# vandenheuvel/rust-lp

Hardware: AMD Instinct MI355X
Metric: simplex iterations/sec (higher is better)
Workload: dtype f64; 1 GPU; dense10k: synthetic dense LP 10000x10000 f64 (+10000 slack columns), SteepestDescent, dense tableau with blocked f64-MFMA updates; m=10000, n=10000, seed=20250002, engine=tableau, update_block=64, parallelism=single GPU, solves=1

## Files before the change

include/relp_engine.h:

```cpp
#ifndef RELP_ENGINE_H
#define RELP_ENGINE_H

#include <stdint.h>

#ifdef __cplusplus
extern "C" {
#endif

typedef struct relp_engine relp_engine_t;

typedef enum {
    RELP_OK = 0,
    RELP_E_ARG = -1,
    RELP_E_HIP = -2,
    RELP_E_ZERO_PIVOT = -3,
    RELP_E_SINGULAR = -4,
    RELP_E_STATE = -5,
    RELP_E_UNSUPPORTED = -6,
    RELP_E_ALLOC = -7
} relp_status_t;

typedef enum {
    RELP_RUNNING = 0,
    RELP_OPTIMAL = 1,
    RELP_UNBOUNDED = 2,
    RELP_INFEASIBLE = 3,
    RELP_PHASE_ONE_DONE = 4,
    RELP_NO_ROW_PHASE_ONE = 5
} relp_outcome_t;

typedef enum {
    RELP_RULE_FIRST_PROFITABLE = 0,
    RELP_RULE_FIRST_PROFITABLE_WITH_MEMORY = 1,
    RELP_RULE_STEEPEST_DESCENT = 2
} relp_pivot_rule_t;

typedef enum { RELP_FORMAT_CSC = 0, RELP_FORMAT_DENSE = 1 } relp_format_t;
typedef enum { RELP_MEM_HOST = 0, RELP_MEM_DEVICE = 1 } relp_memory_t;

typedef struct {
    int32_t nr_normal;
    int32_t nr_eq, nr_range, nr_le, nr_ge;
    int32_t format;
    int32_t matrix_memory;
    const int64_t *col_ptr;
    const int32_t *row_idx;
    const double  *values;
    const double  *dense;
    int64_t        dense_ld;
    const double  *b;
    const double  *ranges;
    const double  *cost;
    const double  *upper_bound;
} relp_matrix_data_t;

typedef struct {
    int32_t device;
    int32_t phase_one_rule;
    int32_t phase_two_rule;
    double  tol_cost;
    double  tol_pivot;
    double  tol_zero;
    double  tol_tie;
    double  tol_feas;
    int32_t poll_interval;
    int32_t trace_capacity;
    int32_t shard_rank, shard_count;
    int32_t update_block;
    int32_t engine;
    int32_t ratio_rule;
    int32_t artificial_removal;
    int32_t pivot_rescue;
    int32_t auto_reinversion;
} relp_config_t;

typedef enum { RELP_RATIO_REFERENCE = 0, RELP_RATIO_LARGEST_PIVOT = 1 } relp_ratio_rule_t;
typedef enum { RELP_ARTIFICIAL_REFERENCE = 0, RELP_ARTIFICIAL_TEXTBOOK = 1 } relp_artificial_removal_t;

typedef enum {
    RELP_ENGINE_REVISED = 0,
    RELP_ENGINE_TABLEAU = 1,
    RELP_ENGINE_LU = 2,
    RELP_ENGINE_AUTO = 3
} relp_engine_kind_t;

void relp_default_config(relp_config_t *cfg);
void relp_robust_config(relp_config_t *cfg);
int32_t relp_engine_kind(const relp_engine_t *h);
relp_status_t relp_robust_stats(const relp_engine_t *h, int64_t *out4);
const char *relp_last_error(const relp_engine_t *h);
const char *relp_version(void);

relp_status_t relp_engine_create(const relp_matrix_data_t *md, const relp_config_t *cfg, relp_engine_t **out);
void          relp_engine_destroy(relp_engine_t *h);
relp_status_t relp_set_stream(relp_engine_t *h, void *hip_stream);

relp_status_t relp_select_primal_pivot_column(relp_engine_t *h, int32_t rule, int32_t *found,
                                              int32_t *column, double *relative_cost);
relp_status_t relp_relative_costs(relp_engine_t *h, double *out_n);
relp_status_t relp_generate_column(relp_engine_t *h, int32_t column, double *out_m);
relp_status_t relp_generate_element(relp_engine_t *h, int32_t row, int32_t column, double *out);
relp_status_t relp_select_primal_pivot_row(relp_engine_t *h, int32_t *found, int32_t *row);
relp_status_t relp_select_primal_pivot_row_of(relp_engine_t *h, const double *column_m, int32_t *found, int32_t *row);
relp_status_t relp_bring_into_basis(relp_engine_t *h, int32_t column, int32_t row, double relative_cost,
                                    int32_t *leaving_column);

relp_status_t relp_run(relp_engine_t *h, int64_t max_iters, int64_t *iterations_done, int32_t *outcome);
relp_status_t relp_solve_relaxation(relp_engine_t *h, int64_t max_iters, int32_t *outcome);
relp_status_t relp_from_basis(relp_engine_t *h, const int32_t *basis_columns_m);
relp_status_t relp_set_reinversion_interval(relp_engine_t *h, int64_t pivots);
int64_t       relp_reinversions(const relp_engine_t *h);
relp_status_t relp_flush(relp_engine_t *h);
relp_status_t relp_tab_flush_stats(relp_engine_t *h, int64_t *out2);
int32_t       relp_tab_load_batch(const relp_engine_t *h);
int32_t       relp_update_block(const relp_engine_t *h);
relp_status_t relp_lu_stats(const relp_engine_t *h, int64_t *out8);
relp_status_t relp_lu_lookahead_stats(const relp_engine_t *h, int64_t *out4);
relp_status_t relp_lu_kernel_layout(const relp_engine_t *h, int32_t *out4);
relp_status_t relp_lu_set_device_factorisation(relp_engine_t *h, int32_t on);
relp_status_t relp_lu_device_factorisation_stats(const relp_engine_t *h, int64_t *out6);
relp_status_t relp_lu_factor_residual(relp_engine_t *h, double *out);

relp_status_t relp_lu_phase_cycles(relp_engine_t *h, int64_t *out16);

relp_status_t relp_basis_inverse_row(relp_engine_t *h, int32_t row, double *out_m);
relp_status_t relp_should_refactor(relp_engine_t *h, int32_t *out);
relp_status_t relp_generate_column_of(relp_engine_t *h, const int32_t *row_idx, const double *values, int32_t nnz, double *out_m);
relp_status_t relp_cost_difference_of(relp_engine_t *h, const int32_t *row_idx, const double *values, int32_t nnz, double *out);
relp_status_t relp_lu_change_basis(relp_engine_t *h, int32_t pivot_row_index);
relp_status_t relp_lu_set_factors(relp_engine_t *h, const int64_t *l_col_ptr, const int32_t *l_row_idx, const double *l_values,
                                  const int64_t *u_col_ptr, const int32_t *u_row_idx, const double *u_values);
relp_status_t relp_lu_updates(relp_engine_t *h, int32_t *count);
relp_status_t relp_lu_get_update(relp_engine_t *h, int32_t k, int32_t *pivot, int32_t *idx, double *values, int32_t cap, int32_t *nnz);
relp_status_t relp_lu_get_upper(relp_engine_t *h, int64_t *col_ptr_m1, int32_t *row_idx, double *values, int64_t cap, int64_t *nnz);

int32_t relp_nr_rows(const relp_engine_t *h);
int32_t relp_nr_columns(const relp_engine_t *h);
int32_t relp_phase(const relp_engine_t *h);
int32_t relp_nr_artificial(const relp_engine_t *h);
relp_status_t relp_get_objective(relp_engine_t *h, double *out);
relp_status_t relp_get_b(relp_engine_t *h, double *out_m);
relp_status_t relp_get_minus_pi(relp_engine_t *h, double *out_m);
relp_status_t relp_get_basis_indices(relp_engine_t *h, int32_t *out_m);
relp_status_t relp_get_basis_inverse(relp_engine_t *h, double *out_mm);
relp_status_t relp_current_bfs(relp_engine_t *h, int32_t *cols, double *vals, int32_t cap, int32_t *count);
relp_status_t relp_get_iterations(relp_engine_t *h, int64_t *out);
relp_status_t relp_get_degenerate_pivots(relp_engine_t *h, int64_t *out);
relp_status_t relp_get_trace(relp_engine_t *h, int32_t *phase, int32_t *entering, int32_t *row,
                             int32_t *leaving, int64_t cap, int64_t *count);
relp_status_t relp_check_basis(relp_engine_t *h, double *max_identity_error, double *max_basic_cost,
                               double *min_b);

typedef enum {
    RELP_K_PRICE = 0, RELP_K_SELECT_COLUMN = 1, RELP_K_BUILD_COLUMN = 2, RELP_K_FTRAN = 3,
    RELP_K_RATIO = 4, RELP_K_UPDATE_VECTORS = 5, RELP_K_UPDATE_INVERSE = 6,
    RELP_K_APPLY_W = 7,
    RELP_K_UPDATE_W = 8,
    RELP_K_FLUSH = 9,
    RELP_K_FT_RUN = 10,
    RELP_K_COUNT = 11
} relp_kernel_id_t;
relp_status_t relp_profile_enable(relp_engine_t *h, int32_t enable, int64_t max_launches, int32_t sample_every);
relp_status_t relp_profile_read(relp_engine_t *h, int32_t kernel_id, int64_t *launches, double *total_ms);

relp_status_t relp_synth_fill_dense(double *device_a, int64_t ld, int32_t m, int32_t n, uint64_t seed,
                                    int64_t first_column, void *hip_stream);
relp_status_t relp_device_alloc(void **out, int64_t bytes);
relp_status_t relp_device_free(void *p);

relp_status_t relp_shard_ranges(const relp_engine_t *h, int32_t *col_lo, int32_t *col_hi,
                                int32_t *row_lo, int32_t *row_hi, int32_t *row_slice_stride);
void          relp_shard_column_range(int32_t nr_normal, int32_t rank, int32_t count, int32_t *lo, int32_t *hi);
int64_t       relp_shard_candidate_len(const relp_engine_t *h);
int64_t       relp_shard_rho_len(const relp_engine_t *h);
relp_status_t relp_shard_price(relp_engine_t *h, double *dev_candidate);
relp_status_t relp_shard_select_column(relp_engine_t *h, const double *dev_candidates, int32_t count);
relp_status_t relp_shard_ftran(relp_engine_t *h, double *dev_alpha_slice);
relp_status_t relp_shard_ratio(relp_engine_t *h, const double *dev_alpha_slices, int32_t count, double *dev_rho);
relp_status_t relp_shard_update(relp_engine_t *h, const double *dev_rho);
relp_status_t relp_shard_plan(const relp_matrix_data_t *md, const relp_config_t *cfg, int32_t *col_lo, int32_t *col_hi);
relp_status_t relp_shard_pivot(relp_engine_t *h);
relp_status_t relp_shard_flush_begin(relp_engine_t *h, double **dev_snapshot, int64_t *len_doubles);
relp_status_t relp_shard_flush_end(relp_engine_t *h);
relp_status_t relp_poll(relp_engine_t *h, int32_t *outcome, int64_t *iterations);

typedef int (*relp_allgather_fn)(void *ctx, const void *dev_send, void *dev_recv, int64_t bytes_per_rank, void *hip_stream);
typedef int (*relp_allreduce_sum_fn)(void *ctx, double *dev_buf, int64_t count, void *hip_stream);
relp_status_t relp_shard_set_collectives(relp_engine_t *h, relp_allgather_fn allgather, relp_allreduce_sum_fn allreduce_sum,
                                         void *ctx);
relp_status_t relp_shard_run(relp_engine_t *h, int64_t max_iters, int64_t *done, int32_t *outcome);
relp_status_t relp_shard_inject_failure(relp_engine_t *h, int64_t after_pivots);
#define RELP_RCCL_ID_BYTES 128
relp_status_t relp_rccl_unique_id(uint8_t id[RELP_RCCL_ID_BYTES]);
relp_status_t relp_rccl_attach(relp_engine_t *h, const uint8_t id[RELP_RCCL_ID_BYTES]);

#ifdef __cplusplus
}
#endif
#endif
```

rust-lp_amd/csrc/relp_abi.cpp:

```cpp
#include <cstring>
#include <new>

#include "relp_engine.hpp"

using relp::Engine;

struct relp_engine { Engine impl; };

#define H(h) ((h)->impl)

extern "C" {

void relp_default_config(relp_config_t* cfg) {
    std::memset(cfg, 0, sizeof(*cfg));
    cfg->device = -1;
    cfg->phase_one_rule = RELP_RULE_FIRST_PROFITABLE_WITH_MEMORY;
    cfg->phase_two_rule = RELP_RULE_STEEPEST_DESCENT;
    cfg->tol_cost = 1e-7; cfg->tol_pivot = 1e-5; cfg->tol_zero = 1e-11; cfg->tol_tie = 1e-9; cfg->tol_feas = 1e-7;
    cfg->poll_interval = 64;
    cfg->trace_capacity = 0;
    cfg->shard_rank = 0; cfg->shard_count = 1;
    cfg->update_block = -1;
    cfg->engine = RELP_ENGINE_REVISED;
}

void relp_robust_config(relp_config_t* cfg) {
    relp_default_config(cfg);
    cfg->ratio_rule = RELP_RATIO_LARGEST_PIVOT;
    cfg->artificial_removal = RELP_ARTIFICIAL_TEXTBOOK;
    cfg->pivot_rescue = 1;
    cfg->auto_reinversion = 1;
    cfg->engine = RELP_ENGINE_AUTO;
}
int32_t relp_engine_kind(const relp_engine_t* h) { return h ? H(h).engine_kind() : -1; }
relp_status_t relp_robust_stats(const relp_engine_t* h, int64_t* out4) { return (h && out4) ? H(h).robust_stats(out4) : RELP_E_ARG; }

const char* relp_last_error(const relp_engine_t* h) { return h ? H(h).last_error() : "null handle"; }
const char* relp_version(void) { return "relp-mi355x 0.2 (gfx950; engines: explicit inverse, dense tableau, sparse LU + Forrest-Tomlin)"; }

relp_status_t relp_engine_create(const relp_matrix_data_t* md, const relp_config_t* cfg, relp_engine_t** out) {
    if (!md || !cfg || !out) return RELP_E_ARG;
    relp_engine_t* h = new (std::nothrow) relp_engine_t();
    if (!h) return RELP_E_ALLOC;
    relp_status_t st = H(h).create(*md, *cfg);
    *out = h;
    return st;
}

void relp_engine_destroy(relp_engine_t* h) { delete h; }
relp_status_t relp_set_stream(relp_engine_t* h, void* s) { return h ? H(h).set_stream((hipStream_t)s) : RELP_E_ARG; }

relp_status_t relp_select_primal_pivot_column(relp_engine_t* h, int32_t rule, int32_t* found, int32_t* column, double* cost) {
    return h ? H(h).select_primal_pivot_column(rule, found, column, cost) : RELP_E_ARG;
}
relp_status_t relp_relative_costs(relp_engine_t* h, double* out) { return (h && out) ? H(h).relative_costs(out) : RELP_E_ARG; }
relp_status_t relp_generate_column(relp_engine_t* h, int32_t column, double* out) { return h ? H(h).generate_column(column, out) : RELP_E_ARG; }
relp_status_t relp_generate_element(relp_engine_t* h, int32_t row, int32_t column, double* out) {
    return h ? H(h).generate_element(row, column, out) : RELP_E_ARG;
}
relp_status_t relp_select_primal_pivot_row(relp_engine_t* h, int32_t* found, int32_t* row) {
    return h ? H(h).select_primal_pivot_row(found, row) : RELP_E_ARG;
}
relp_status_t relp_select_primal_pivot_row_of(relp_engine_t* h, const double* column, int32_t* found, int32_t* row) {
    return (h && column) ? H(h).select_primal_pivot_row_of(column, found, row) : RELP_E_ARG;
}
relp_status_t relp_bring_into_basis(relp_engine_t* h, int32_t column, int32_t row, double cost, int32_t* leaving) {
    return h ? H(h).bring_into_basis(column, row, cost, leaving) : RELP_E_ARG;
}

relp_status_t relp_run(relp_engine_t* h, int64_t max_iters, int64_t* done, int32_t* outcome) {
    return h ? H(h).run(max_iters, done, outcome) : RELP_E_ARG;
}
relp_status_t relp_solve_relaxation(relp_engine_t* h, int64_t max_iters, int32_t* outcome) {
    return h ? H(h).solve_relaxation(max_iters, outcome) : RELP_E_ARG;
}
relp_status_t relp_from_basis(relp_engine_t* h, const int32_t* basis) { return (h && basis) ? H(h).from_basis(basis) : RELP_E_ARG; }

relp_status_t relp_flush(relp_engine_t* h) { return h ? H(h).flush() : RELP_E_ARG; }
relp_status_t relp_set_reinversion_interval(relp_engine_t* h, int64_t pivots) { return h ? H(h).set_reinversion_interval(pivots) : RELP_E_ARG; }
int64_t relp_reinversions(const relp_engine_t* h) { return h ? H(h).reinversions() : -1; }
int32_t relp_update_block(const relp_engine_t* h) { return h ? H(h).update_block() : -1; }
int32_t relp_tab_load_batch(const relp_engine_t* h) { return h ? H(h).tab_load_batch_size() : -1; }
relp_status_t relp_lu_stats(const relp_engine_t* h, int64_t* out8) { return (h && out8) ? H(h).lu_stats(out8) : RELP_E_ARG; }
relp_status_t relp_lu_lookahead_stats(const relp_engine_t* h, int64_t* out4) { return (h && out4) ? H(h).lu_lookahead_stats(out4) : RELP_E_ARG; }
relp_status_t relp_lu_kernel_layout(const relp_engine_t* h, int32_t* out4) { return (h && out4) ? H(h).lu_kernel_layout(out4) : RELP_E_ARG; }
relp_status_t relp_lu_set_device_factorisation(relp_engine_t* h, int32_t on) { return h ? H(h).lu_set_device_factorisation(on != 0) : RELP_E_ARG; }
relp_status_t relp_lu_factor_residual(relp_engine_t* h, double* out) { return (h && out) ? H(h).lu_factor_residual(out) : RELP_E_ARG; }
relp_status_t relp_lu_device_factorisation_stats(const relp_engine_t* h, int64_t* out6) { return (h && out6) ? H(h).luf_stats(out6) : RELP_E_ARG; }
relp_status_t relp_shard_inject_failure(relp_engine_t* h, int64_t after_pivots) { if (!h) return RELP_E_ARG; H(h).shard_inject_failure(after_pivots); return RELP_OK; }
relp_status_t relp_lu_phase_cycles(relp_engine_t* h, int64_t* out16) { return (h && out16) ? H(h).lu_phase_cycles(out16) : RELP_E_ARG; }
relp_status_t relp_basis_inverse_row(relp_engine_t* h, int32_t row, double* out_m) { return (h && out_m) ? H(h).basis_inverse_row(row, out_m) : RELP_E_ARG; }
relp_status_t relp_should_refactor(relp_engine_t* h, int32_t* out) { return (h && out) ? H(h).should_refactor(out) : RELP_E_ARG; }
relp_status_t relp_generate_column_of(relp_engine_t* h, const int32_t* idx, const double* val, int32_t nnz, double* out_m) {
    return h ? H(h).generate_column_of(idx, val, nnz, out_m) : RELP_E_ARG;
}
relp_status_t relp_cost_difference_of(relp_engine_t* h, const int32_t* idx, const double* val, int32_t nnz, double* out) {
    return h ? H(h).cost_difference_of(idx, val, nnz, out) : RELP_E_ARG;
}
relp_status_t relp_lu_change_basis(relp_engine_t* h, int32_t row) { return h ? H(h).lu_change_basis(row) : RELP_E_ARG; }
relp_status_t relp_lu_set_factors(relp_engine_t* h, const int64_t* l_ptr, const int32_t* l_idx, const double* l_val,
                                  const int64_t* u_ptr, const int32_t* u_idx, const double* u_val) {
    return h ? H(h).lu_set_factors(l_ptr, l_idx, l_val, u_ptr, u_idx, u_val) : RELP_E_ARG;
}
relp_status_t relp_lu_updates(relp_engine_t* h, int32_t* count) { return (h && count) ? H(h).lu_updates(count) : RELP_E_ARG; }
relp_status_t relp_lu_get_update(relp_engine_t* h, int32_t k, int32_t* pivot, int32_t* idx, double* val, int32_t cap, int32_t* nnz) {
    return h ? H(h).lu_get_update(k, pivot, idx, val, cap, nnz) : RELP_E_ARG;
}
relp_status_t relp_lu_get_upper(relp_engine_t* h, int64_t* col_ptr, int32_t* row_idx, double* values, int64_t cap, int64_t* nnz) {
    return h ? H(h).lu_get_upper(col_ptr, row_idx, values, cap, nnz) : RELP_E_ARG;
}
relp_status_t relp_shard_flush_begin(relp_engine_t* h, double** snap, int64_t* len) {
    return h ? H(h).shard_flush_begin(snap, len) : RELP_E_ARG;
}
relp_status_t relp_shard_flush_end(relp_engine_t* h) { return h ? H(h).shard_flush_end() : RELP_E_ARG; }
relp_status_t relp_shard_set_collectives(relp_engine_t* h, relp_allgather_fn ag, relp_allreduce_sum_fn ar, void* ctx) {
    return h ? H(h).shard_set_collectives(ag, ar, ctx) : RELP_E_ARG;
}
relp_status_t relp_shard_run(relp_engine_t* h, int64_t max_iters, int64_t* done, int32_t* outcome) {
    return h ? H(h).shard_run(max_iters, done, outcome) : RELP_E_ARG;
}
relp_status_t relp_rccl_attach(relp_engine_t* h, const uint8_t* id) { return (h && id) ? H(h).rccl_attach(id) : RELP_E_ARG; }

int32_t relp_nr_rows(const relp_engine_t* h) { return h ? H(h).nr_rows() : -1; }
int32_t relp_nr_columns(const relp_engine_t* h) { return h ? H(h).nr_columns() : -1; }
int32_t relp_phase(const relp_engine_t* h) { return h ? H(h).phase() : -1; }
int32_t relp_nr_artificial(const relp_engine_t* h) { return h ? H(h).nr_artificial() : -1; }
relp_status_t relp_get_objective(relp_engine_t* h, double* out) { return (h && out) ? H(h).get_objective(out) : RELP_E_ARG; }
relp_status_t relp_get_b(relp_engine_t* h, double* out) { return (h && out) ? H(h).get_vector(0, out) : RELP_E_ARG; }
relp_status_t relp_get_minus_pi(relp_engine_t* h, double* out) { return (h && out) ? H(h).get_vector(1, out) : RELP_E_ARG; }
relp_status_t relp_get_basis_indices(relp_engine_t* h, int32_t* out) { return (h && out) ? H(h).get_basis_indices(out) : RELP_E_ARG; }
relp_status_t relp_get_basis_inverse(relp_engine_t* h, double* out) { return (h && out) ? H(h).get_basis_inverse(out) : RELP_E_ARG; }
relp_status_t relp_current_bfs(relp_engine_t* h, int32_t* cols, double* vals, int32_t cap, int32_t* count) {
    return h ? H(h).current_bfs(cols, vals, cap, count) : RELP_E_ARG;
}
relp_status_t relp_get_iterations(relp_engine_t* h, int64_t* out) { return (h && out) ? H(h).get_iterations(out) : RELP_E_ARG; }
relp_status_t relp_get_degenerate_pivots(relp_engine_t* h, int64_t* out) { return (h && out) ? H(h).get_degenerate_pivots(out) : RELP_E_ARG; }
relp_status_t relp_tab_flush_stats(relp_engine_t* h, int64_t* out2) { return (h && out2) ? H(h).tab_flush_stats(out2) : RELP_E_ARG; }
relp_status_t relp_get_trace(relp_engine_t* h, int32_t* phase, int32_t* entering, int32_t* row, int32_t* leaving,
                             int64_t cap, int64_t* count) {
    return h ? H(h).get_trace(phase, entering, row, leaving, cap, count) : RELP_E_ARG;
}
relp_status_t relp_check_basis(relp_engine_t* h, double* e1, double* e2, double* mb) { return h ? H(h).check_basis(e1, e2, mb) : RELP_E_ARG; }

relp_status_t relp_profile_enable(relp_engine_t* h, int32_t enable, int64_t max_launches, int32_t sample_every) {
    return h ? H(h).profile_enable(enable != 0, max_launches, sample_every) : RELP_E_ARG;
}
relp_status_t relp_profile_read(relp_engine_t* h, int32_t kid, int64_t* launches, double* total_ms) {
    return h ? H(h).profile_read(kid, launches, total_ms) : RELP_E_ARG;
}

relp_status_t relp_synth_fill_dense(double* device_a, int64_t ld, int32_t m, int32_t n, uint64_t seed,
                                    int64_t first_column, void* hip_stream) {
    if (!device_a || ld < m || m < 0 || n < 0) return RELP_E_ARG;
    relp::launch_fill_dense(device_a, ld, m, n, seed, first_column, (hipStream_t)hip_stream);
    if (hipStreamSynchronize((hipStream_t)hip_stream) != hipSuccess) return RELP_E_HIP;
    return hipGetLastError() == hipSuccess ? RELP_OK : RELP_E_HIP;
}
relp_status_t relp_device_alloc(void** out, int64_t bytes) {
    if (!out || bytes < 0) return RELP_E_ARG;
    return hipMalloc(out, (size_t)(bytes ? bytes : 1)) == hipSuccess ? RELP_OK : RELP_E_ALLOC;
}
relp_status_t relp_device_free(void* p) { return hipFree(p) == hipSuccess ? RELP_OK : RELP_E_HIP; }

relp_status_t relp_shard_ranges(const relp_engine_t* h, int32_t* col_lo, int32_t* col_hi, int32_t* row_lo,
                                int32_t* row_hi, int32_t* stride) {
    if (!h) return RELP_E_ARG;
    H(h).shard_ranges(col_lo, col_hi, row_lo, row_hi, stride);
    return RELP_OK;
}
void relp_shard_column_range(int32_t nr_normal, int32_t rank, int32_t count, int32_t* lo, int32_t* hi) {
    relp::shard_column_range(nr_normal, rank, count, lo, hi);
}
int64_t relp_shard_candidate_len(const relp_engine_t* h) { return h ? H(h).candidate_len() : -1; }
int64_t relp_shard_rho_len(const relp_engine_t* h) { return h ? H(h).rho_len() : -1; }
relp_status_t relp_shard_price(relp_engine_t* h, double* c) { return (h && c) ? H(h).shard_price(c) : RELP_E_ARG; }
relp_status_t relp_shard_select_column(relp_engine_t* h, const double* c, int32_t count) {
    return (h && c) ? H(h).shard_select_column(c, count) : RELP_E_ARG;
}
relp_status_t relp_shard_ftran(relp_engine_t* h, double* a) { return (h && a) ? H(h).shard_ftran(a) : RELP_E_ARG; }
relp_status_t relp_shard_ratio(relp_engine_t* h, const double* a, int32_t count, double* rho) {
    return (h && a && rho) ? H(h).shard_ratio(a, count, rho) : RELP_E_ARG;
}
relp_status_t relp_shard_update(relp_engine_t* h, const double* rho) { return (h && rho) ? H(h).shard_update(rho) : RELP_E_ARG; }
relp_status_t relp_shard_pivot(relp_engine_t* h) { return h ? H(h).shard_pivot() : RELP_E_ARG; }
relp_status_t relp_shard_plan(const relp_matrix_data_t* md, const relp_config_t* cfg, int32_t* col_lo, int32_t* col_hi) {
    if (!md || !cfg) return RELP_E_ARG;
    relp::Layout layout;
    const relp_status_t st = layout.plan(*md, *cfg, nullptr);
    if (st) return st;
    if (col_lo) *col_lo = layout.col_lo;
    if (col_hi) *col_hi = layout.col_hi;
    return RELP_OK;
}
relp_status_t relp_poll(relp_engine_t* h, int32_t* outcome, int64_t* iterations) { return h ? H(h).poll(outcome, iterations) : RELP_E_ARG; }

}
```

rust-lp_amd/csrc/relp_device_common.h:

```cpp
#pragma once
#include <algorithm>
#include "relp_kernels.h"

#include <math.h>

namespace relp {

static constexpr int kThreads = 256;
static constexpr int kVecPerBlock = 8;
static constexpr int kSingleBlock = 1024;

__device__ __forceinline__ double wave_sum(double v) {
#pragma unroll
    for (int off = 32; off > 0; off >>= 1) v += __shfl_down(v, off, 64);
    return v;
}

__device__ __forceinline__ void block_multi_dot(const double* __restrict__ M, int64_t ld, int len,
                                                int v0, int v_hi, const double* __restrict__ x,
                                                double* s_partial ,
                                                double& result) {
    const int t = threadIdx.x;
    double acc[kVecPerBlock];
    const double* base[kVecPerBlock];
#pragma unroll
    for (int v = 0; v < kVecPerBlock; ++v) {
        acc[v] = 0.0;
        int vi = v0 + v;
        if (vi >= v_hi) vi = v_hi - 1;
        base[v] = M + (int64_t)vi * ld;
    }
    const int len2 = len & ~1;
    for (int k = 2 * t; k < len2; k += 2 * kThreads) {
        const double2 xv = *reinterpret_cast<const double2*>(x + k);
#pragma unroll
        for (int v = 0; v < kVecPerBlock; ++v) {
            const double2 a = *reinterpret_cast<const double2*>(base[v] + k);
            acc[v] = fma(a.x, xv.x, acc[v]);
            acc[v] = fma(a.y, xv.y, acc[v]);
        }
    }
    if ((len & 1) && t == 0) {
        const double xl = x[len - 1];
#pragma unroll
        for (int v = 0; v < kVecPerBlock; ++v) acc[v] = fma(base[v][len - 1], xl, acc[v]);
    }
    const int lane = t & 63, wave = t >> 6;
#pragma unroll
    for (int v = 0; v < kVecPerBlock; ++v) {
        const double w = wave_sum(acc[v]);
        if (lane == 0) s_partial[wave * kVecPerBlock + v] = w;
    }
    __syncthreads();
    if (t < kVecPerBlock) {
        result = (s_partial[0 * kVecPerBlock + t] + s_partial[1 * kVecPerBlock + t]) +
                 (s_partial[2 * kVecPerBlock + t] + s_partial[3 * kVecPerBlock + t]);
    }
}

__device__ __forceinline__ double select_key(int rule, int n, const PivotRecord* rec, int j, double d_j) {
    if (rule == 2) return d_j;
    const int last = (rule == 1 && rec) ? rec->last_selected : -1;
    if (last >= 0) return (double)(j >= last ? j - last : j - last + n);
    return (double)j;
}

template <int BS>
__device__ __forceinline__ void block_min_key(double& key, int& kj) {
    __shared__ double s_k[BS / 64];
    __shared__ int s_j[BS / 64];
#pragma unroll
    for (int off = 32; off > 0; off >>= 1) {
        const double ok = __shfl_down(key, off, 64);
        const int oj = __shfl_down(kj, off, 64);
        if (ok < key || (ok == key && oj < kj)) { key = ok; kj = oj; }
    }
    const int lane = threadIdx.x & 63, wave = threadIdx.x >> 6;
    if (lane == 0) { s_k[wave] = key; s_j[wave] = kj; }
    __syncthreads();
    key = s_k[0]; kj = s_j[0];
#pragma unroll
    for (int w = 1; w < BS / 64; ++w)
        if (s_k[w] < key || (s_k[w] == key && s_j[w] < kj)) { key = s_k[w]; kj = s_j[w]; }
}

__device__ __forceinline__ void block_partial_min(double key, int kj, SelectPartials sp, int slot) {
    block_min_key<kThreads>(key, kj);
    if (threadIdx.x == 0) { sp.k1[slot] = key; sp.j[slot] = kj; }
}

__device__ __forceinline__ void price_virtual_body(const ColumnTable& ct, const double* __restrict__ minus_pi,
                                                   double* __restrict__ d, int cost_mode, const SelectPartials& sp,
                                                   const PivotRecord* rec, int block) {
    const int t = block * kThreads + threadIdx.x;
    int j = -1;
    double val = 0.0;
    if (t < ct.nr_artificial) {
        j = t;
        val = (cost_mode == 1 ? 1.0 : 0.0) + minus_pi[ct.column_to_row[t]];
    } else {
        const int v = t - ct.nr_artificial;
        if (v < ct.nr_virtual) {
            const int r0 = ct.vrow0[v];
            double s = r0 >= 0 ? (double)ct.vsign[v] * minus_pi[r0] : 0.0;
            const int r1 = ct.vrow1[v];
            if (r1 >= 0) s += minus_pi[r1];
            j = ct.nr_artificial + ct.nr_normal + v;
            val = s;
        }
    }
    if (j >= 0) d[j] = val;
    if (!sp.k1) return;
    double key = INFINITY;
    int kj = 0x7fffffff;
    if (j >= 0 && !sp.in_basis[j] && val < -sp.tol_cost) { key = select_key(sp.rule, sp.n, rec, j, val); kj = j; }
    block_partial_min(key, kj, sp, sp.offset + block);
}

template <int BS>
__device__ __forceinline__ void tab_select_entering(const TableauView& tv, const SelectPartials& sp, int count, double& k1,
                                                    int& bj) {
    constexpr int kListMax = 32, kGroups = BS / kThreads;
    __shared__ int s_list[kListMax];
    __shared__ int s_cnt;
    __shared__ int s_low[BS / 64];
    for (int t = threadIdx.x + BS; t < count; t += BS) {
        const double key = sp.k1[t];
        const int j = sp.j[t];
        if (key < k1 || (key == k1 && j < bj)) { k1 = key; bj = j; }
    }
    if (threadIdx.x == 0) s_cnt = 0;
    block_min_key<BS>(k1, bj);
    if (!(bj != 0x7fffffff && sp.rule == 2 && sp.tol_tie > 0.0)) return;
    const double bound = k1 + sp.tol_tie * fmax(1.0, fabs(k1));
    for (int t = threadIdx.x; t < count; t += BS) {
        if (!(sp.k1[t] <= bound)) continue;
        const int pos = atomicAdd(&s_cnt, 1);
        if (pos < kListMax) s_list[pos] = t;
    }
    __syncthreads();
    const int listed = s_cnt;
    const int grp = threadIdx.x / kThreads, u = threadIdx.x % kThreads;
    int lowest = 0x7fffffff;
    auto scan_slot = [&](int t) {
        const int c = tv.c_lo + t * kThreads + u;
        const int j = c - tv.col_off;
        if (c < tv.c_hi && j >= 0 && j < tv.n) {
            const double v = tv.d[c];
            if (!sp.in_basis[j] && v < -sp.tol_cost && v <= bound && j < lowest) lowest = j;
        }
    };
    if (listed <= kListMax) {
        for (int i = grp; i < listed; i += kGroups) scan_slot(s_list[i]);
    } else {
        for (int t = grp; t < count; t += kGroups)
            if (sp.k1[t] <= bound) scan_slot(t);
    }
#pragma unroll
    for (int off = 32; off > 0; off >>= 1) lowest = min(lowest, __shfl_down(lowest, off, 64));
    if ((threadIdx.x & 63) == 0) s_low[threadIdx.x >> 6] = lowest;
    __syncthreads();
    bj = s_low[0];
#pragma unroll
    for (int w = 1; w < BS / 64; ++w) bj = min(bj, s_low[w]);
}

__device__ __forceinline__ int candidate_winner(const double* key, const double* idx, int64_t stride, int count, int rule,
                                                double tol_tie) {
    int win = -1; double k1 = INFINITY; double kj = 0.0;
    for (int g = 0; g < count; ++g) {
        const double a = key[g * stride], j = idx[g * stride];
        if (a < k1 || (a == k1 && win >= 0 && j < kj)) { k1 = a; kj = j; win = g; }
    }
    if (win >= 0 && rule == 2 && tol_tie > 0.0) {
        const double bound = k1 + tol_tie * fmax(1.0, fabs(k1));
        for (int g = 0; g < count; ++g)
            if (key[g * stride] <= bound && idx[g * stride] < kj) { kj = idx[g * stride]; win = g; }
    }
    return win;
}

static constexpr int kMaxRanks = 64;
__device__ __forceinline__ int candidate_winner_staged(const double* __restrict__ msgs, int count, int64_t msg_len, int rule,
                                                       double tol_tie, int* q, double* d_q) {
    __shared__ double s_key[kMaxRanks], s_idx[kMaxRanks], s_dq[kMaxRanks];
    __shared__ int s_win;
    for (int g = threadIdx.x; g < count && g < kMaxRanks; g += blockDim.x) {
        s_key[g] = msgs[g * msg_len + 0]; s_idx[g] = msgs[g * msg_len + 1]; s_dq[g] = msgs[g * msg_len + 2];
    }
    __syncthreads();
    if (threadIdx.x == 0) s_win = candidate_winner(s_key, s_idx, 1, count, rule, tol_tie);
    __syncthreads();
    const int win = s_win;
    if (win >= 0) { *q = (int)s_idx[win]; *d_q = s_dq[win]; }
    return win;
}

__device__ __forceinline__ void record_candidate(PivotRecord* rec, int rule, int win, int q, double d_q) {
    if (win < 0) {
        rec->outcome = DEV_NO_CANDIDATE;
        if (rule == 1) rec->last_selected = -1;
    } else {
        rec->q = q;
        rec->d_q = d_q;
        if (rule == 1) rec->last_selected = q;
    }
}

__device__ __forceinline__ double pivot_b(double a, double b_i, double br, bool is_r) {
    return is_r ? br : (a != 0.0 ? fma(-a, br, b_i) : b_i);
}

__device__ __forceinline__ void pivot_bookkeeping(int phase, long long iterations, double minus_objective, double d_q, double br,
                                                  int q, int r, int leaving, uint8_t* in_basis, int32_t* trace, int64_t trace_cap,
                                                  PivotRecord* rec) {
    rec->minus_objective = fma(-d_q, br, minus_objective);
    if (leaving < kWrappedArtificialBase) in_basis[leaving] = 0;
    in_basis[q] = 1;
    if (trace && iterations < trace_cap) {
        trace[0 * trace_cap + iterations] = phase;
        trace[1 * trace_cap + iterations] = q;
        trace[2 * trace_cap + iterations] = r;
        trace[3 * trace_cap + iterations] = leaving;
    }
    if (br == 0.0) rec->degenerate += 1;
    rec->iterations = iterations + 1;
}

static constexpr int kMaxEta = 128;

typedef unsigned long long tie_key_t;
static constexpr tie_key_t kNoTieKey = ~0ull;
__device__ __forceinline__ tie_key_t tie_key(double a, int leave, int ratio_rule) {
    const unsigned size = ratio_rule ? 0x7fffffffu - __float_as_uint((float)a) : 0u;
    return ((tie_key_t)size << 32) | (unsigned)leave;
}
__device__ __forceinline__ int tie_key_leaving(tie_key_t k) { return (int)(unsigned)(k & 0xffffffffull); }

template <int BS>
__device__ __forceinline__ void tie_reduce(tie_key_t& key, int& row, tie_key_t* s_k, int* s_r, bool wide) {
    const int lane = threadIdx.x & 63, wave = threadIdx.x >> 6;
    if (wide) {
#pragma unroll
        for (int off = 32; off > 0; off >>= 1) {
            const tie_key_t ok = __shfl_down(key, off, 64);
            const int orow = __shfl_down(row, off, 64);
            if (ok < key) { key = ok; row = orow; }
        }
    } else {
        int lv = (int)(unsigned)key;
        if (key == kNoTieKey) lv = 0x7fffffff;
#pragma unroll
        for (int off = 32; off > 0; off >>= 1) {
            const int ol = __shfl_down(lv, off, 64);
            const int orow = __shfl_down(row, off, 64);
            if (ol < lv) { lv = ol; row = orow; }
        }
        key = (unsigned)lv;
    }
    if (lane == 0) { s_k[wave] = key; s_r[wave] = row; }
    __syncthreads();
    key = s_k[0]; row = s_r[0];
#pragma unroll
    for (int w = 1; w < BS / 64; ++w)
        if (s_k[w] < key) { key = s_k[w]; row = s_r[w]; }
}

template <int BS>
__device__ __forceinline__ void ratio_commit_row(int r, int leaving, const double* alpha, const double* b, const DeferredUpdate& du,
                                                 int p, PivotRecord* rec, int guard_m = 0, double guard_rel = 0.0) {
    if (guard_m > 0) {
        __shared__ double s_gm[BS / 64];
        double mx = 0.0;
        for (int i = threadIdx.x; i < guard_m; i += BS) mx = fmax(mx, fabs(alpha[i]));
#pragma unroll
        for (int off = 32; off > 0; off >>= 1) mx = fmax(mx, __shfl_down(mx, off, 64));
        __syncthreads();
        if ((threadIdx.x & 63) == 0) s_gm[threadIdx.x >> 6] = mx;
        __syncthreads();
        double amax = s_gm[0];
#pragma unroll
        for (int w = 1; w < BS / 64; ++w) amax = fmax(amax, s_gm[w]);
        if (alpha[r] < guard_rel * amax) {
            if (threadIdx.x == 0) rec->outcome = DEV_NO_ROW;
            return;
        }
    }
    const bool deferred = du.kmax > 0;
    double a_r = 0.0, b_r = 0.0;
    int jt = 0;
    if (threadIdx.x == 0) {
        a_r = alpha[r];
        b_r = b[r];
        if (deferred) jt = du.pos_of_row[r];
    }
    if (deferred)
        for (int j = threadIdx.x; j < p; j += BS) du.wr[j] = du.W[(int64_t)j * du.ld + r];
    if (threadIdx.x == 0) {
        rec->r = r;
        rec->leaving = leaving;
        rec->alpha_r = a_r;
        rec->b_r = b_r;
        if (deferred) {
            rec->n_eta_old = p;
            if (jt < 0) { jt = p; du.S[p] = r; du.pos_of_row[r] = p; rec->n_eta = p + 1; }
            rec->eta_target = jt;
        }
    }
}

template <int BS, int ITEMS>
__device__ __forceinline__ void ratio_body(const double* alpha, const double* b, const int32_t* basis_indices, int m,
                                           const Tolerances& tol, const DeferredUpdate& du, int p, PivotRecord* rec) {
    __shared__ double s_min[BS / 64];
    __shared__ double s_bcast;
    const int lane = threadIdx.x & 63, wave = threadIdx.x >> 6;

    constexpr int kItems = ITEMS;
    const bool cached = m <= kItems * BS;
    double ratio_r[kItems], alpha_r[kItems];
    int leave_r[kItems];
    double mn = INFINITY;
    if (cached) {
#pragma unroll
        for (int k = 0; k < kItems; ++k) {
            const int i = threadIdx.x + k * BS;
            const bool in = i < m;
            const double a = in ? alpha[i] : 0.0;
            double bi = in ? b[i] : 0.0;
            leave_r[k] = in ? basis_indices[i] : 0x7fffffff;
            alpha_r[k] = a;
            if (bi <= tol.zero) bi = 0.0;
            ratio_r[k] = (in && a > tol.pivot) ? bi / a : INFINITY;
            mn = fmin(mn, ratio_r[k]);
        }
    } else {
#pragma unroll 4
        for (int i = threadIdx.x; i < m; i += BS) {
            const double a = alpha[i];
            double bi = b[i];
            if (bi <= tol.zero) bi = 0.0;
            const double ratio = (a > tol.pivot) ? bi / a : INFINITY;
            mn = fmin(mn, ratio);
        }
    }
#pragma unroll
    for (int off = 32; off > 0; off >>= 1) mn = fmin(mn, __shfl_down(mn, off, 64));
    if (lane == 0) s_min[wave] = mn;
    __syncthreads();
    if (threadIdx.x == 0) {
        double g = s_min[0];
        for (int w = 1; w < BS / 64; ++w) g = fmin(g, s_min[w]);
        s_bcast = g;
    }
    __syncthreads();
    const double gmin = s_bcast;
    if (gmin == INFINITY) {
        if (threadIdx.x == 0) rec->outcome = DEV_NO_ROW;
        return;
    }
    const double bound = gmin + tol.tie * fmax(1.0, fabs(gmin));
    tie_key_t best_key = kNoTieKey;
    int best_row = -1;
    if (cached) {
#pragma unroll
        for (int k = 0; k < kItems; ++k) {
            if (ratio_r[k] <= bound) {
                const tie_key_t key = tie_key(alpha_r[k], leave_r[k], tol.ratio_rule);
                if (key < best_key) { best_key = key; best_row = threadIdx.x + k * BS; }
            }
        }
    } else {
#pragma unroll 4
        for (int i = threadIdx.x; i < m; i += BS) {
            const double a = alpha[i];
            double bi = b[i];
            const int lv = basis_indices[i];
            if (bi <= tol.zero) bi = 0.0;
            if (a > tol.pivot && bi / a <= bound) {
                const tie_key_t key = tie_key(a, lv, tol.ratio_rule);
                if (key < best_key) { best_key = key; best_row = i; }
            }
        }
    }
    __shared__ tie_key_t s_cl[BS / 64];
    __shared__ int s_cr[BS / 64];
    tie_reduce<BS>(best_key, best_row, s_cl, s_cr, tol.ratio_rule != 0);
    ratio_commit_row<BS>(best_row, tie_key_leaving(best_key), alpha, b, du, p, rec, tol.pivot_guard ? m : 0, tol.guard_rel);
}

__device__ __forceinline__ double row_ratio(double a, double bi, const Tolerances& tol) {
    if (bi <= tol.zero) bi = 0.0;
    return a > tol.pivot ? bi / a : INFINITY;
}

template <int BS>
__device__ __forceinline__ void ratio_blocks_pick(const double* alpha, const double* b, const int32_t* basis_indices, int m,
                                                  const Tolerances& tol, const double* rmin, int nblk, int* row_out, int* leave_out,
                                                  double first = INFINITY, bool have_first = false, int rpb = kThreads) {
    __shared__ double s_min[BS / 64];
    __shared__ double s_bcast;
    constexpr int kListMax = 64;
    __shared__ int s_list[kListMax];
    __shared__ int s_cnt;
    __shared__ tie_key_t s_cl[BS / 64];
    __shared__ int s_cr[BS / 64];
    const int lane = threadIdx.x & 63, wave = threadIdx.x >> 6;
    double mn = have_first ? first : INFINITY;
    for (int t = threadIdx.x + (have_first ? BS : 0); t < nblk; t += BS) mn = fmin(mn, rmin[t]);
#pragma unroll
    for (int off = 32; off > 0; off >>= 1) mn = fmin(mn, __shfl_down(mn, off, 64));
    if (lane == 0) s_min[wave] = mn;
    if (threadIdx.x == 0) s_cnt = 0;
    __syncthreads();
    if (threadIdx.x == 0) {
        double g = s_min[0];
        for (int w = 1; w < BS / 64; ++w) g = fmin(g, s_min[w]);
        s_bcast = g;
    }
    __syncthreads();
    const double gmin = s_bcast;
    if (gmin == INFINITY) { *row_out = -1; *leave_out = 0x7fffffff; return; }
    const double bound = gmin + tol.tie * fmax(1.0, fabs(gmin));
    for (int t = threadIdx.x; t < nblk; t += BS) {
        if (!(rmin[t] <= bound)) continue;
        const int pos = atomicAdd(&s_cnt, 1);
        if (pos < kListMax) s_list[pos] = t;
    }
    __syncthreads();
    const int listed = s_cnt;
    const bool use_list = listed <= kListMax;
    const int total = (use_list ? listed : nblk) * rpb;
    tie_key_t best_key = kNoTieKey;
    int best_row = -1;
    for (int idx = threadIdx.x; idx < total; idx += BS) {
        const int t = use_list ? s_list[idx / rpb] : idx / rpb;
        const int i = t * rpb + idx % rpb;
        if (i >= m) continue;
        const double a = alpha[i];
        double bi = b[i];
        int lv = basis_indices[i];
        asm volatile("" : "+v"(lv));
        if (bi <= tol.zero) bi = 0.0;
        if (a > tol.pivot && bi / a <= bound) {
            const tie_key_t key = tie_key(a, lv, tol.ratio_rule);
            if (key < best_key) { best_key = key; best_row = i; }
        }
    }
    tie_reduce<BS>(best_key, best_row, s_cl, s_cr, tol.ratio_rule != 0);
    *row_out = best_row; *leave_out = tie_key_leaving(best_key);
}

template <int BS>
__device__ __forceinline__ void ratio_blocks_body(const double* alpha, const double* b, const int32_t* basis_indices, int m,
                                                  const Tolerances& tol, const DeferredUpdate& du, const double* rmin, int nblk,
                                                  int p, PivotRecord* rec, double first = INFINITY, bool have_first = false,
                                                  int rpb = kThreads) {
    int r, leaving;
    ratio_blocks_pick<BS>(alpha, b, basis_indices, m, tol, rmin, nblk, &r, &leaving, first, have_first, rpb);
    if (r < 0) {
        if (threadIdx.x == 0) rec->outcome = DEV_NO_ROW;
        return;
    }
    ratio_commit_row<BS>(r, leaving, alpha, b, du, p, rec, tol.pivot_guard ? m : 0, tol.guard_rel);
}

static inline int cdiv(int64_t a, int64_t b) { return (int)((a + b - 1) / b); }
static inline int element_blocks(int64_t total) { return (int)std::min<int64_t>((total + 255) / 256, int64_t(1) << 22); }

}
```

rust-lp_amd/csrc/relp_engine.cpp:

```cpp
#include "relp_engine_internal.hpp"

#include <algorithm>
#include <chrono>
#include <cmath>
#include <cstdio>
#include <cstdlib>
#include <cstring>
#include <limits>

namespace relp {

bool Engine::hip_ok(hipError_t e, const char* what) {
    if (e == hipSuccess) return true;
    err_ = std::string(what) + ": " + hipGetErrorString(e);
    return false;
}

void Engine::free_all() {
    luf_release();
    auto fr = [](auto*& p) { if (p) { (void)hipFree(p); p = nullptr; } };
    if (owns_A_) fr(dA_);
    dA_ = nullptr;
    fr(dBinv_); fr(d_minus_pi_); fr(d_b_); fr(d_alpha_); fr(d_aq_); fr(d_rho_); fr(d_d_); fr(d_w_); fr(d_cost_);
    fr(d_basis_); fr(d_column_to_row_); fr(d_bound_row_); fr(d_vrow0_); fr(d_vrow1_); fr(d_vsign_); fr(d_trace_);
    fr(d_in_basis_); fr(d_rec_);
    fr(d_part_k1_); fr(d_part_j_);
    fr(d_fcols_); fr(d_fcount_); fr(d_fmask_); fr(d_fstats_); fr(d_R0c_);
    fr(dT0_); fr(dR0_); fr(d_b_alt_); fr(d_basis_alt_); fr(d_shadow_); fr(d_shadow_meta_);
    if (h_lu_buf_) { (void)hipHostFree(h_lu_buf_); h_lu_buf_ = nullptr; h_lu_cap_ = 0; }
    if (h_basis_) { (void)hipHostFree(h_basis_); h_basis_ = nullptr; }
    if (h_mirror_) { (void)hipHostFree(h_mirror_); h_mirror_ = nullptr; d_mirror_ = nullptr; }
    fr(d_cost_store_); fr(d_idcol_); fr(d_rmin_);
    fr(d_msg_cand_); fr(d_msg_cands_); fr(d_msg_slice_); fr(d_msg_slices_); fr(d_msg_rho_); fr(d_msg_status_); fr(d_msg_statuses_);
    fr(d_v_); fr(d_W_); fr(d_wr_); fr(d_R_); fr(d_S_); fr(d_pos_of_row_);
    fr(d_cptr_); fr(d_cidx_); fr(d_cval_); fr(d_lu_buf_); fr(d_lu_buf_alt_); fr(d_lu_scratch_); fr(d_ft_buf_); fr(d_pe_buf_);
    if (h_ft_hdr_) { (void)hipHostFree(h_ft_hdr_); h_ft_hdr_ = nullptr; }
    if (h_rec_) { (void)hipHostFree(h_rec_); h_rec_ = nullptr; }
    for (auto e : prof_ev_) (void)hipEventDestroy(e);
    prof_ev_.clear();
    if (owns_stream_ && stream_) { (void)hipStreamDestroy(stream_); }
    stream_ = nullptr;
}

Engine::~Engine() { rccl_release(); free_all(); }

ColumnTable Engine::table() const {
    ColumnTable ct;
    ct.nr_artificial = lay_.nr_artificial;
    ct.nr_normal = lay_.nr_normal;
    ct.nr_virtual = lay_.nr_virtual;
    ct.nr_constraints = lay_.mc;
    ct.column_to_row = d_column_to_row_;
    ct.bound_row = d_bound_row_;
    ct.vrow0 = d_vrow0_;
    ct.vrow1 = d_vrow1_;
    ct.vsign = d_vsign_;
    ct.cost = d_cost_;
    return ct;
}

Tolerances Engine::tolerances() const { return Tolerances{cfg_.tol_cost, cfg_.tol_pivot, cfg_.tol_zero, cfg_.tol_tie, cfg_.ratio_rule, (pivot_guard_on_ && guard_rel_ > 0.0) ? 1 : 0, guard_rel_}; }

TableauView Engine::tview() const {
    TableauView tv;
    tv.T0 = dT0_ - (int64_t)lay_.sc_lo * ld_t_; tv.ld_t = ld_t_;
    tv.R0 = dR0_ - (int64_t)lay_.sc_lo; tv.ld_r = ld_r_;
    tv.d = d_d_; tv.m = lay_.m; tv.n_store = n_store_;
    tv.col_off = phase_ == 1 ? 0 : tab_na_;
    tv.n = nr_columns();
    tv.c_lo = lay_.sc_lo; tv.c_hi = lay_.sc_hi;
    return tv;
}

FlushList Engine::flush_list() const {
    FlushList fl;
    fl.cols = d_fcols_; fl.count = d_fcount_; fl.mask = d_fmask_; fl.R0c = d_R0c_; fl.ld = ld_r_; fl.stats = d_fstats_;
    return fl;
}

SelectPartials Engine::tab_partials(int rule) const {
    SelectPartials sp;
    sp.k1 = d_part_k1_; sp.j = d_part_j_; sp.in_basis = d_in_basis_; sp.tol_cost = cfg_.tol_cost; sp.rule = rule;
    sp.n = nr_columns(); sp.offset = 0; sp.nb_struct = 0; sp.tol_tie = cfg_.tol_tie; sp.p_lo = 0; sp.cols_per_slot = 8;
    return sp;
}

DeferredUpdate Engine::deferred() const {
    DeferredUpdate du;
    du.W = d_W_; du.ld = ld_b_; du.kmax = block_; du.S = d_S_; du.pos_of_row = d_pos_of_row_; du.wr = d_wr_; du.R = d_R_;
    du.batch = load_batch_; du.w_split = w_split_;
    return du;
}

relp_status_t Engine::download_rec() {
    HIP_TRY(hipMemcpyAsync(h_rec_, d_rec_, sizeof(PivotRecord), hipMemcpyDeviceToHost, stream_));
    HIP_TRY(hipStreamSynchronize(stream_));
    return RELP_OK;
}

relp_status_t Engine::upload_rec() {
    HIP_TRY(hipMemcpyAsync(d_rec_, h_rec_, sizeof(PivotRecord), hipMemcpyHostToDevice, stream_));
    HIP_TRY(hipStreamSynchronize(stream_));
    return RELP_OK;
}

relp_status_t Engine::set_stream(hipStream_t s) {
    if (stream_) HIP_TRY(hipStreamSynchronize(stream_));
    if (owns_stream_ && stream_) HIP_TRY(hipStreamDestroy(stream_));
    stream_ = s;
    owns_stream_ = false;
    return RELP_OK;
}

relp_status_t Engine::create(const relp_matrix_data_t& md, const relp_config_t& cfg) {
    (void)hipGetLastError();
    cfg_ = cfg;
    if (cfg_.shard_count < 1) cfg_.shard_count = 1;
    if (cfg_.poll_interval < 1) cfg_.poll_interval = 64;
    if (const relp_status_t lst = lay_.build(md, cfg_, &err_)) return lst;
    if (cfg_.device >= 0) HIP_TRY(hipSetDevice(cfg_.device));
    phase_ = 1;
    n_alloc_ = lay_.nr_columns();

    HIP_TRY(hipStreamCreateWithFlags(&stream_, hipStreamNonBlocking));
    owns_stream_ = true;
    const int32_t n_local = lay_.col_hi - lay_.col_lo;
    lu_ = lay_.engine == RELP_ENGINE_LU;
    tableau_ = lay_.engine == RELP_ENGINE_TABLEAU;
    if (lu_) {
        if (cfg_.shard_count > 1) return fail(RELP_E_UNSUPPORTED, "the LU engine is not sharded");
        relp_status_t lst = lu_load_matrix(md);
        if (lst) return lst;
    } else if (md.format == RELP_FORMAT_DENSE) {
        if (lay_.nr_normal > 0 && lay_.mc > 0 && !md.dense) return fail(RELP_E_ARG, "dense matrix missing");
        const int64_t src_ld = md.dense_ld > 0 ? md.dense_ld : lay_.mc;
        if (src_ld < lay_.mc) return fail(RELP_E_ARG, "dense_ld < nr_constraints");
        if (md.matrix_memory == RELP_MEM_DEVICE && (src_ld % 2) == 0) {
            dA_ = const_cast<double*>(md.dense); ld_a_ = src_ld; owns_A_ = false;
        } else {
            ld_a_ = round_up(std::max<int64_t>(lay_.mc, 1), 2);
            HIP_TRY(dev_alloc(&dA_, ld_a_ * std::max(n_local, 1)));
            owns_A_ = true;
            if (n_local > 0 && lay_.mc > 0)
                HIP_TRY(hipMemcpy2D(dA_, ld_a_ * sizeof(double), md.dense, src_ld * sizeof(double), lay_.mc * sizeof(double),
                                    n_local, md.matrix_memory == RELP_MEM_DEVICE ? hipMemcpyDeviceToDevice : hipMemcpyHostToDevice));
        }
    } else if (md.format == RELP_FORMAT_CSC) {
        if (md.matrix_memory != RELP_MEM_HOST) return fail(RELP_E_UNSUPPORTED, "CSC input must be in host memory");
        if (!md.col_ptr) return fail(RELP_E_ARG, "col_ptr missing");
        ld_a_ = round_up(std::max<int64_t>(lay_.mc, 1), 2);
        const int64_t e0 = n_local > 0 ? md.col_ptr[lay_.col_lo] : 0, e1 = n_local > 0 ? md.col_ptr[lay_.col_hi] : 0;
        for (int64_t p = e0; p < e1; ++p)
            if (md.row_idx[p] < 0 || md.row_idx[p] >= lay_.mc) return fail(RELP_E_ARG, "row index out of range");
        const int64_t cells = ld_a_ * std::max(n_local, 1);
        HIP_TRY(dev_alloc(&dA_, cells));
        owns_A_ = true;
        HIP_TRY(hipMemset(dA_, 0, (size_t)cells * sizeof(double)));
        if (e1 > e0) {
            int64_t* t_ptr = nullptr; int32_t* t_idx = nullptr; double* t_val = nullptr;
            auto drop = [&]() { if (t_ptr) (void)hipFree(t_ptr); if (t_idx) (void)hipFree(t_idx); if (t_val) (void)hipFree(t_val); };
            if (hipMalloc(reinterpret_cast<void**>(&t_ptr), sizeof(int64_t) * (size_t)(n_local + 1)) != hipSuccess ||
                hipMalloc(reinterpret_cast<void**>(&t_idx), sizeof(int32_t) * (size_t)(e1 - e0)) != hipSuccess ||
                hipMalloc(reinterpret_cast<void**>(&t_val), sizeof(double) * (size_t)(e1 - e0)) != hipSuccess) {
                drop();
                return fail(RELP_E_ALLOC, "staging the CSC arrays");
            }
            hipError_t err = hipMemcpy(t_ptr, md.col_ptr + lay_.col_lo, sizeof(int64_t) * (size_t)(n_local + 1), hipMemcpyHostToDevice);
            if (err == hipSuccess) err = hipMemcpy(t_idx, md.row_idx + e0, sizeof(int32_t) * (size_t)(e1 - e0), hipMemcpyHostToDevice);
            if (err == hipSuccess) err = hipMemcpy(t_val, md.values + e0, sizeof(double) * (size_t)(e1 - e0), hipMemcpyHostToDevice);
            if (err == hipSuccess) {
                launch_csc_to_dense(t_ptr, t_idx, t_val, n_local, dA_, ld_a_, nullptr);
                err = hipDeviceSynchronize();
            }
            drop();
            if (err != hipSuccess) return fail(RELP_E_HIP, "dense copy of the CSC input");
        }
    } else {
        return fail(RELP_E_ARG, "unknown matrix format");
    }

    ld_b_ = round_up(lay_.m, 16);
    const int64_t rows_local = std::max(lay_.row_hi - lay_.row_lo, 1);
    HIP_TRY(dev_alloc(&dBinv_, (tableau_ || lu_) ? 16 : rows_local * ld_b_));
    HIP_TRY(dev_alloc(&d_minus_pi_, ld_b_));
    HIP_TRY(dev_alloc(&d_b_, ld_b_));
    HIP_TRY(dev_alloc(&d_alpha_, ld_b_));
    HIP_TRY(dev_alloc(&d_aq_, ld_b_));
    HIP_TRY(dev_alloc(&d_rho_, ld_b_));
    HIP_TRY(dev_alloc(&d_w_, ld_b_));
    HIP_TRY(dev_alloc(&d_d_, n_alloc_));
    HIP_TRY(dev_alloc(&d_cost_, lay_.nr_normal));
    HIP_TRY(dev_alloc(&d_basis_, lay_.m));
    HIP_TRY(dev_alloc(&d_column_to_row_, lay_.nr_artificial));
    HIP_TRY(dev_alloc(&d_bound_row_, lay_.nr_normal));
    HIP_TRY(dev_alloc(&d_vrow0_, lay_.nr_virtual));
    HIP_TRY(dev_alloc(&d_vrow1_, lay_.nr_virtual));
    HIP_TRY(dev_alloc(&d_vsign_, lay_.nr_virtual));
    HIP_TRY(dev_alloc(&d_in_basis_, n_alloc_));
    HIP_TRY(dev_alloc(&d_rec_, 1));
    {
        const int64_t slots = price_structural_blocks(lay_.col_lo, lay_.col_hi) + (lay_.nr_artificial + lay_.nr_virtual + 255) / 256 + 8 +
                              tab_scan_blocks(n_alloc_) + price_csc_blocks(0, lay_.nr_normal);
        HIP_TRY(dev_alloc(&d_part_k1_, slots));
        HIP_TRY(dev_alloc(&d_part_j_, slots));
    }
    block_ = cfg_.update_block < 0 ? (lay_.m >= 4096 ? 64 : 0) : std::min(cfg_.update_block, 128);
    if (lu_) {
        block_ = cfg_.update_block < 0 ? 128 : std::max(1, std::min(cfg_.update_block, 128));
        HIP_TRY(dev_alloc(&d_lu_scratch_, ld_b_));
        {
            const char* la = std::getenv("RELP_LU_LOOKAHEAD");
            const char* fl = std::getenv("RELP_FUSE_LANES");
            const char* df = std::getenv("RELP_LU_DEVICE_FACTOR");
            luf_enabled_ = df && std::atoi(df) != 0;
            luf_download_ = df && std::atoi(df) == 2;
            lu_lookahead_env_ = la ? std::atoi(la) : 8;
            lu_lookahead_set_ = la != nullptr;
            lu_fuse_lanes_env_ = fl ? std::atoi(fl) : 256;
        }
        relp_status_t fst = ft_plan_and_alloc();
        if (fst) return fst;
    }
    if (tableau_) {
        if (block_ == 0) block_ = 64;
        if (cfg_.update_block < 0 && lay_.m >= 4096 && n_alloc_ >= 40000) block_ = 96;
        n_store_ = n_alloc_;
        tab_na_ = lay_.nr_artificial;
        const int64_t n_owned = std::max(lay_.sc_hi - lay_.sc_lo, 1);
        ld_t_ = round_up(lay_.m, 2);
        ld_r_ = round_up(n_owned, 2);
        HIP_TRY(dev_alloc(&dT0_, ld_t_ * n_owned));
        HIP_TRY(dev_alloc(&dR0_, ld_r_ * (block_ + 1)));
        {
            const char* e = std::getenv("RELP_TAB_FLUSH_ALL");
            flush_all_ = e && std::atoi(e) != 0;
            HIP_TRY(dev_alloc(&d_fstats_, 2));
            if (!flush_all_) {
                HIP_TRY(dev_alloc(&d_fcols_, n_owned));
                HIP_TRY(dev_alloc(&d_fcount_, 1));
                HIP_TRY(dev_alloc(&d_fmask_, (n_owned + 63) / 64));
                HIP_TRY(dev_alloc(&d_R0c_, ld_r_ * block_));
            }
        }
        {
            const char* e = std::getenv("RELP_TAB_LOAD_BATCH");
            load_batch_ = tab_load_batch(e ? std::atoi(e) : 0);
            const char* w = std::getenv("RELP_TAB_W_SPLIT");
            w_split_ = w && std::atoi(w) >= 1 ? std::min(std::atoi(w), 16) : kTabSplitDefault;
        }
        {
            const char* e = std::getenv("RELP_FUSED_UPDATE");
            fused_update_ = !(e && std::atoi(e) == 0);
            if (cfg_.pivot_rescue && cfg_.shard_count == 1) fused_update_ = false;
            if (fused_update_) {
                HIP_TRY(dev_alloc(&d_b_alt_, ld_b_));
                HIP_TRY(dev_alloc(&d_basis_alt_, lay_.m));
                HIP_TRY(dev_alloc(&d_shadow_, std::max(block_, 1) + 1));
                HIP_TRY(hipMalloc(reinterpret_cast<void**>(&d_shadow_meta_), 2 * sizeof(int32_t)));
                const int32_t none[2] = {-1, 0};
                HIP_TRY(hipMemcpy(d_shadow_meta_, none, sizeof none, hipMemcpyHostToDevice));
            }
        }
        HIP_TRY(dev_alloc(&d_cost_store_, n_store_));
        HIP_TRY(dev_alloc(&d_idcol_, lay_.m));
    }
    if (block_ > 0 && ft_) {
        HIP_TRY(dev_alloc(&d_v_, ld_b_));
    } else if (block_ > 0) {
        HIP_TRY(dev_alloc(&d_v_, ld_b_));
        HIP_TRY(dev_alloc(&d_W_, ld_b_ * block_));
        if (!tableau_) HIP_TRY(dev_alloc(&d_R_, ld_b_ * block_));
        HIP_TRY(dev_alloc(&d_wr_, block_));
        HIP_TRY(dev_alloc(&d_S_, block_));
        HIP_TRY(dev_alloc(&d_pos_of_row_, lay_.m));
        HIP_TRY(hipMemset(d_pos_of_row_, 0xFF, sizeof(int32_t) * lay_.m));
    }
    HIP_TRY(dev_alloc(&d_rmin_, lay_.m / 8 + 2));
    HIP_TRY(hipHostMalloc(reinterpret_cast<void**>(&h_rec_), sizeof(PivotRecord), hipHostMallocDefault));
    trace_cap_ = std::max(cfg_.trace_capacity, 0);
    if (trace_cap_ > 0) HIP_TRY(dev_alloc(&d_trace_, 4 * trace_cap_));

    auto up = [&](void* dst, const void* src, size_t bytes) -> hipError_t {
        return bytes ? hipMemcpy(dst, src, bytes, hipMemcpyHostToDevice) : hipSuccess;
    };
    HIP_TRY(up(d_cost_, lay_.cost.data(), sizeof(double) * lay_.nr_normal));
    HIP_TRY(up(d_bound_row_, lay_.bound_row.data(), sizeof(int32_t) * lay_.nr_normal));
    HIP_TRY(up(d_vrow0_, lay_.vrow0.data(), sizeof(int32_t) * lay_.nr_virtual));
    HIP_TRY(up(d_vrow1_, lay_.vrow1.data(), sizeof(int32_t) * lay_.nr_virtual));
    HIP_TRY(up(d_vsign_, lay_.vsign.data(), sizeof(int32_t) * lay_.nr_virtual));
    HIP_TRY(up(d_column_to_row_, lay_.column_to_row.data(), sizeof(int32_t) * lay_.nr_artificial));
    HIP_TRY(up(d_basis_, lay_.basis.data(), sizeof(int32_t) * lay_.m));
    HIP_TRY(up(d_b_, lay_.rhs.data(), sizeof(double) * lay_.m));
    HIP_TRY(up(d_minus_pi_, lay_.minus_pi.data(), sizeof(double) * lay_.m));
    std::vector<uint8_t> flags(n_alloc_, 0);
    for (int32_t r = 0; r < lay_.m; ++r) flags[lay_.basis[r]] = 1;
    HIP_TRY(up(d_in_basis_, flags.data(), flags.size()));
    if (lay_.row_hi > lay_.row_lo && !tableau_ && !lu_) launch_set_identity(dBinv_, ld_b_, lay_.row_lo, lay_.row_hi, stream_);
    if (tableau_) {
        idcol_h_ = lay_.basis;
        HIP_TRY(up(d_idcol_, idcol_h_.data(), sizeof(int32_t) * lay_.m));
        const double* A = dA_ - (int64_t)lay_.col_lo * ld_a_;
        launch_tab_build(tview(), A, ld_a_, table(), stream_);
        cost_store_h_.assign(n_store_, 0.0);
        for (int32_t k = 0; k < lay_.nr_artificial; ++k) cost_store_h_[k] = 1.0;
        std::vector<double> w(ld_b_, 0.0);
        for (int32_t k = 0; k < lay_.nr_artificial; ++k) w[lay_.column_to_row[k]] = 1.0;
        HIP_TRY(up(d_cost_store_, cost_store_h_.data(), sizeof(double) * n_store_));
        HIP_TRY(up(d_w_, w.data(), sizeof(double) * ld_b_));
        launch_tab_price_init(tview(), d_w_, d_cost_store_, stream_);
    }
    {
        bool sparse_input = false;
        if (md.format == RELP_FORMAT_CSC && md.col_ptr && lay_.nr_normal > 0 && lay_.mc > 0)
            sparse_input = (double)md.col_ptr[lay_.nr_normal] <= 0.10 * (double)lay_.nr_normal * (double)lay_.mc;
        reinvert_interval_ = (!lu_ && cfg_.shard_count == 1 && lay_.m <= 4096 && sparse_input) ? 1000 : 0;
        if (cfg_.auto_reinversion && !lu_ && cfg_.shard_count == 1) reinvert_interval_ = 256;
    }
    std::memset(h_rec_, 0, sizeof(PivotRecord));
    h_rec_->outcome = DEV_RUNNING;
    h_rec_->minus_objective = -lay_.phase1_objective;
    h_rec_->last_selected = -1;
    h_rec_->phase = 1;
    relp_status_t st = upload_rec();
    if (st) return st;
    HIP_TRY(hipDeviceSynchronize());
    if (hipGetLastError() != hipSuccess) return fail(RELP_E_HIP, "a kernel launch of the set-up failed");
    if (lu_ && (st = lu_refactor())) return st;
    return RELP_OK;
}

relp_status_t Engine::profile_enable(bool enable, int64_t max_launches, int32_t sample_every) {
    prof_stride_ = sample_every > 0 ? sample_every : 1;
    prof_tick_ = 0;
    HIP_TRY(hipStreamSynchronize(stream_));
    for (auto e : prof_ev_) (void)hipEventDestroy(e);
    prof_ev_.clear(); prof_kid_.clear(); prof_open_ = false;
    prof_on_ = enable;
    if (enable) {
        prof_ev_.resize((size_t)max_launches * 2);
        for (auto& e : prof_ev_) HIP_TRY(hipEventCreate(&e));
        prof_kid_.reserve((size_t)max_launches);
    }
    return RELP_OK;
}

void Engine::prof_begin(int kid, hipStream_t on) {
    prof_open_ = false;
    if (!prof_on_ || (prof_kid_.size() + 1) * 2 > prof_ev_.size()) return;
    if (kid != RELP_K_FLUSH && (prof_tick_ % prof_stride_) != 0) return;
    (void)hipEventRecord(prof_ev_[2 * prof_kid_.size()], on ? on : stream_);
    prof_kid_.push_back(kid);
    prof_open_ = true;
}

void Engine::prof_end(hipStream_t on) {
    if (!prof_open_) return;
    (void)hipEventRecord(prof_ev_[2 * (prof_kid_.size() - 1) + 1], on ? on : stream_);
    prof_open_ = false;
}

relp_status_t Engine::profile_read(int kernel_id, int64_t* launches, double* total_ms) {
    HIP_TRY(hipStreamSynchronize(stream_));
    int64_t n = 0; double ms = 0.0;
    for (size_t k = 0; k < prof_kid_.size(); ++k) {
        if (prof_kid_[k] != kernel_id) continue;
        float t = 0.f;
        if (hipEventElapsedTime(&t, prof_ev_[2 * k], prof_ev_[2 * k + 1]) == hipSuccess) { ms += t; ++n; }
    }
    if (launches) *launches = n;
    if (total_ms) *total_ms = ms;
    return RELP_OK;
}

void Engine::enqueue_price(int cost_mode, const double* vec, const PivotRecord* rec, int32_t p_lo, int32_t p_hi) {
    const ColumnTable ct = table();
    if (lu_) {
        launch_price_csc(csc(), ct, vec, d_d_, 0, lay_.nr_normal, cost_mode, SelectPartials{}, rec, stream_);
        launch_price_virtual(ct, vec, d_d_, cost_mode, rec, stream_);
        return;
    }
    const double* A = dA_ - (int64_t)lay_.col_lo * ld_a_;
    launch_price_structural(A, ld_a_, ct, vec, d_d_, p_lo, p_hi, cost_mode, rec, stream_);
    if (p_lo > 0 || p_hi < lay_.nr_normal) launch_price_mask_unowned(ct, d_d_, p_lo, p_hi, rec, stream_);
    launch_price_virtual(ct, vec, d_d_, cost_mode, rec, stream_);
}

void Engine::enqueue_iteration_tableau(int rule) {
    const TableauView tv = tview();
    const DeferredUpdate du = deferred();
    const SelectPartials sp = tab_partials(rule);
    if (fused_update_ && in_loop_) {
        prof_begin(RELP_K_FTRAN);
        launch_tab_select_column_rmin(tv, du, sp, tab_scan_blocks(lay_.sc_hi - lay_.sc_lo), d_alpha_, d_b_, tolerances(), d_rmin_,
                                      d_rec_, stream_, d_shadow_, d_shadow_meta_);
        prof_end();
        prof_begin(RELP_K_PRICE);
        launch_tab_ratio_update_all(tv, du, sp, lay_.m, d_alpha_, d_b_, d_b_alt_, d_basis_, d_basis_alt_, d_in_basis_, d_trace_,
                                    trace_cap_, tolerances(), d_rmin_, d_shadow_, d_shadow_meta_, d_rec_, stream_);
        prof_end();
        std::swap(d_b_, d_b_alt_);
        std::swap(d_basis_, d_basis_alt_);
        shadow_pending_ = true;
        if (++since_flush_ >= block_) enqueue_flush();
        return;
    }
    tab_settle();
    prof_begin(RELP_K_FTRAN);
    launch_tab_select_column_rmin(tv, du, sp, tab_scan_blocks(lay_.sc_hi - lay_.sc_lo), d_alpha_, d_b_, tolerances(), d_rmin_,
                                  d_rec_, stream_);
    prof_end();
    prof_begin(RELP_K_RATIO);
    launch_ratio_blocks(d_alpha_, d_b_, d_basis_, lay_.m, tolerances(), du, d_rmin_, d_rec_, stream_);
    prof_end();
    prof_begin(RELP_K_PRICE);
    launch_tab_update_all(tv, du, sp, lay_.m, d_alpha_, d_b_, d_basis_, d_in_basis_, d_trace_, trace_cap_, d_rec_, stream_);
    prof_end();
    if (++since_flush_ >= block_) enqueue_flush();
}

void Engine::enqueue_iteration(int rule) {
    struct Tick { int64_t& t; ~Tick() { ++t; } } tick{prof_tick_};
    if (tableau_) { enqueue_iteration_tableau(rule); return; }
    if (lu_) { enqueue_iteration_lu(rule); return; }
    const ColumnTable ct = table();
    const double* A = dA_ - (int64_t)lay_.col_lo * ld_a_;
    double* Binv = dBinv_ - (int64_t)lay_.row_lo * ld_b_;
    const int n = nr_columns();
    SelectPartials sp;
    sp.k1 = d_part_k1_; sp.j = d_part_j_; sp.in_basis = d_in_basis_; sp.tol_cost = cfg_.tol_cost; sp.rule = rule;
    const int nb_struct = price_structural_blocks(lay_.col_lo, lay_.col_hi);
    sp.n = n; sp.offset = 0; sp.nb_struct = nb_struct; sp.tol_tie = cfg_.tol_tie; sp.p_lo = lay_.col_lo; sp.cols_per_slot = 8;
    const int nb_virt = price_virtual_blocks(ct);
    prof_begin(RELP_K_PRICE);
    if (lay_.col_lo > 0 || lay_.col_hi < lay_.nr_normal) {
        launch_price_structural_sel(A, ld_a_, ct, d_minus_pi_, d_d_, lay_.col_lo, lay_.col_hi, phase_, sp, d_rec_, stream_);
        launch_price_mask_unowned(ct, d_d_, lay_.col_lo, lay_.col_hi, d_rec_, stream_);
        SelectPartials spv = sp;
        spv.offset = nb_struct;
        launch_price_virtual_sel(ct, d_minus_pi_, d_d_, phase_, spv, d_rec_, stream_);
    } else {
        launch_price_all_sel(A, ld_a_, ct, d_minus_pi_, d_d_, lay_.col_lo, lay_.col_hi, phase_, sp, d_rec_, stream_);
    }
    prof_end();
    prof_begin(RELP_K_SELECT_COLUMN);
    launch_select_partials(sp, nb_struct + nb_virt, d_d_, A, ld_a_, ct, lay_.m, d_aq_, d_rec_, stream_);
    prof_end();
    if (block_ == 0) {
        prof_begin(RELP_K_FTRAN);
        launch_ftran_rmin(Binv, ld_b_, lay_.m, d_aq_, d_alpha_, d_b_, tolerances(), d_rmin_, d_rec_, stream_);
        prof_end();
        prof_begin(RELP_K_RATIO);
        launch_ratio_rows(d_alpha_, d_b_, d_basis_, lay_.m, tolerances(), DeferredUpdate{}, d_rmin_, ftran_rows_per_block(), d_rec_,
                          stream_);
        prof_end();
        prof_begin(RELP_K_UPDATE_VECTORS);
        launch_compute_rho(Binv, ld_b_, lay_.m, lay_.row_lo, lay_.row_hi, d_rho_, d_rec_, stream_);
        prof_end();
        prof_begin(RELP_K_UPDATE_INVERSE);
        launch_update_inverse_vectors(Binv, ld_b_, lay_.m, d_alpha_, d_rho_, d_b_, d_minus_pi_, d_basis_, d_in_basis_, d_trace_,
                                      trace_cap_, d_rec_, stream_);
        prof_end();
        return;
    }
    const DeferredUpdate du = deferred();
    prof_begin(RELP_K_FTRAN);
    launch_ftran(Binv, ld_b_, lay_.m, lay_.row_lo, lay_.row_hi, d_aq_, d_v_, 0, d_rec_, stream_);
    prof_end();
    prof_begin(RELP_K_APPLY_W);
    launch_apply_w_rmin(du, lay_.m, d_v_, d_alpha_, d_b_, tolerances(), d_rmin_, d_rec_, stream_);
    prof_end();
    prof_begin(RELP_K_RATIO);
    launch_ratio_rows(d_alpha_, d_b_, d_basis_, lay_.m, tolerances(), du, d_rmin_, 256, d_rec_, stream_);
    prof_end();
    prof_begin(RELP_K_UPDATE_W);
    launch_update_w(du, lay_.m, d_alpha_, d_rec_, stream_);
    launch_rho_deferred(du, Binv, ld_b_, lay_.m, lay_.row_lo, lay_.row_hi, d_rho_, d_rec_, stream_);
    prof_end();
    prof_begin(RELP_K_UPDATE_VECTORS);
    launch_update_vectors(lay_.m, d_alpha_, d_rho_, d_b_, d_minus_pi_, d_basis_, d_in_basis_, d_trace_, trace_cap_, d_rec_,
                          stream_);
    prof_end();
    if (++since_flush_ >= block_) enqueue_flush();
}

void Engine::tab_settle() {
    if (shadow_pending_) {
        launch_tab_apply_shadow(deferred(), d_shadow_, d_shadow_meta_, stream_);
        shadow_pending_ = false;
    }
}

void Engine::enqueue_flush() {
    if (block_ == 0) return;
    if (lu_) {
        if (since_flush_ == 0 && !ft_need_refactor_) return;
        prof_begin(RELP_K_FLUSH);
        const relp_status_t st = lu_refactor();
        prof_end();
        if (st && !lu_status_) lu_status_ = st;
        return;
    }
    if (tableau_) {
        tab_settle();
        const DeferredUpdate dut = deferred();
        prof_begin(RELP_K_FLUSH);
        launch_tab_flush(tview(), dut, d_rec_, flush_list(), stream_);
        launch_flush_reset(dut, d_rec_, stream_);
        prof_end();
        since_flush_ = 0;
        if (++flushes_since_reprice_ >= kRepriceEveryFlushes) {
            flushes_since_reprice_ = 0;
            const TableauView tv = tview();
            const int rule = phase_ == 1 ? cfg_.phase_one_rule : cfg_.phase_two_rule;
            launch_tab_basis_costs(tv, d_basis_, d_cost_store_, d_w_, stream_);
            launch_tab_price_init(tv, d_w_, d_cost_store_, stream_);
            launch_tab_scan(tv, tab_partials(rule), d_rec_, stream_);
        }
        return;
    }
    const DeferredUpdate du = deferred();
    double* Binv = dBinv_ - (int64_t)lay_.row_lo * ld_b_;
    prof_begin(RELP_K_FLUSH);
    launch_flush_snapshot(du, Binv, ld_b_, lay_.row_lo, lay_.row_hi, d_rec_, stream_);
    launch_flush_apply(du, Binv, ld_b_, lay_.m, lay_.row_lo, lay_.row_hi, d_rec_, stream_);
    launch_flush_reset(du, d_rec_, stream_);
    prof_end();
    since_flush_ = 0;
}

relp_status_t Engine::flush() {
    tab_settle();
    if (cfg_.shard_count > 1 && block_ > 0 && !tableau_) {
        if (!coll_allreduce_) return fail(RELP_E_STATE, "sharded flush needs relp_shard_flush_begin/end (or the collective hooks)");
        if (since_flush_ == 0) return RELP_OK;
        double* snap = nullptr; int64_t len = 0;
        relp_status_t st = shard_flush_begin(&snap, &len);
        if (st) return st;
        if (len > 0) {
            if (coll_allreduce_(coll_ctx_, snap, len, stream_)) return fail(RELP_E_HIP, "all-reduce of the flush snapshot failed");
            if ((st = shard_flush_end())) return st;
        }
        since_flush_ = 0;
        return RELP_OK;
    }
    enqueue_flush();
    return RELP_OK;
}

relp_status_t Engine::select_primal_pivot_column(int rule, int32_t* found, int32_t* column, double* cost) {
    relp_status_t st = download_rec();
    if (st) return st;
// ... 954 lines not shown
```

rust-lp_amd/csrc/relp_engine.hpp:

```cpp
#pragma once
#include <hip/hip_runtime.h>

#include <cstdint>
#include <chrono>
#include <condition_variable>
#include <functional>
#include <mutex>
#include <string>
#include <thread>
#include <vector>

#include "../../include/relp_engine.h"
#include "relp_kernels.h"
#include "relp_layout.hpp"
#include "relp_lu.hpp"

namespace relp {

class Engine {
  public:
    Engine() = default;
    ~Engine();

    relp_status_t create(const relp_matrix_data_t& md, const relp_config_t& cfg);
    relp_status_t set_stream(hipStream_t s);

    relp_status_t select_primal_pivot_column(int rule, int32_t* found, int32_t* column, double* cost);
    relp_status_t relative_costs(double* out_n);
    relp_status_t generate_column(int32_t column, double* out_m);
    relp_status_t generate_element(int32_t row, int32_t column, double* out);
    relp_status_t select_primal_pivot_row(int32_t* found, int32_t* row);
    relp_status_t select_primal_pivot_row_of(const double* column, int32_t* found, int32_t* row);
    relp_status_t bring_into_basis(int32_t column, int32_t row, double cost, int32_t* leaving);

    relp_status_t run(int64_t max_iters, int64_t* done, int32_t* outcome);
    int32_t engine_kind() const { return lay_.engine; }
    relp_status_t robust_stats(int64_t* out4) const;
    relp_status_t solve_relaxation(int64_t max_iters, int32_t* outcome);
    relp_status_t from_basis(const int32_t* basis_columns);
    relp_status_t set_reinversion_interval(int64_t pivots);
    int64_t reinversions() const { return reinversions_; }
    relp_status_t flush();
    int32_t update_block() const { return block_; }
    relp_status_t lu_stats(int64_t* out8) const;
    relp_status_t lu_lookahead_stats(int64_t* out4) const;
    relp_status_t lu_kernel_layout(int32_t* out4) const;
    relp_status_t luf_stats(int64_t* out6) const;
    relp_status_t lu_set_device_factorisation(bool on);
    relp_status_t lu_factor_residual(double* out);
    relp_status_t lu_basis_columns(std::vector<std::vector<std::pair<int32_t, double>>>& cols);
    relp_status_t lu_basis_flat(std::vector<int64_t>& ptr, std::vector<int32_t>& idx, std::vector<double>& val);
    relp_status_t lu_phase_cycles(int64_t* out16);
    relp_status_t lu_download_basis();
    relp_status_t lu_factor_downloaded_basis();
    relp_status_t lu_refactor_lookahead(int rule, int64_t budget, bool have_basis);
    relp_status_t ft_read_report(bool* have_basis);
    void lu_refactor_clock(std::chrono::steady_clock::time_point tb, std::chrono::steady_clock::time_point t0,
                           std::chrono::steady_clock::time_point t1, std::chrono::steady_clock::time_point t2);
    relp_status_t basis_inverse_row(int32_t row, double* out_m);
    relp_status_t should_refactor(int32_t* out);
    relp_status_t generate_column_of(const int32_t* idx, const double* val, int32_t nnz, double* out_m);
    relp_status_t cost_difference_of(const int32_t* idx, const double* val, int32_t nnz, double* out);
    relp_status_t lu_change_basis(int32_t row);
    relp_status_t lu_updates(int32_t* count);
    relp_status_t lu_get_update(int32_t k, int32_t* pivot, int32_t* idx, double* val, int32_t cap, int32_t* nnz);
    relp_status_t lu_get_upper(int64_t* col_ptr, int32_t* row_idx, double* values, int64_t cap, int64_t* nnz);
    relp_status_t lu_set_factors(const int64_t* l_ptr, const int32_t* l_idx, const double* l_val, const int64_t* u_ptr,
                                 const int32_t* u_idx, const double* u_val);
    relp_status_t shard_flush_begin(double** dev_snapshot, int64_t* len);
    relp_status_t shard_flush_end();

    int32_t nr_rows() const { return lay_.m; }
    int32_t nr_columns() const { return lay_.nr_columns(); }
    int32_t phase() const { return phase_; }
    int32_t nr_artificial() const { return lay_.nr_artificial; }
    relp_status_t get_objective(double* out);
    relp_status_t get_vector(int which, double* out);
    relp_status_t get_basis_indices(int32_t* out);
    relp_status_t get_basis_inverse(double* out);
    relp_status_t current_bfs(int32_t* cols, double* vals, int32_t cap, int32_t* count);
    relp_status_t get_iterations(int64_t* out);
    relp_status_t get_degenerate_pivots(int64_t* out);
    relp_status_t tab_flush_stats(int64_t* out2);
    int32_t tab_load_batch_size() const { return tableau_ ? load_batch_ : 0; }
    relp_status_t get_trace(int32_t* phase, int32_t* entering, int32_t* row, int32_t* leaving, int64_t cap,
                            int64_t* count);
    relp_status_t check_basis(double* max_identity_error, double* max_basic_cost, double* min_b);

    relp_status_t profile_enable(bool enable, int64_t max_launches, int32_t sample_every);
    relp_status_t profile_read(int kernel_id, int64_t* launches, double* total_ms);

    void shard_ranges(int32_t* col_lo, int32_t* col_hi, int32_t* row_lo, int32_t* row_hi, int32_t* stride) const;
    int64_t candidate_len() const { return lay_.candidate_len; }
    int64_t rho_len() const { return ld_b_; }
    relp_status_t shard_price(double* dev_candidate);
    relp_status_t shard_select_column(const double* dev_candidates, int32_t count);
    relp_status_t shard_ftran(double* dev_alpha_slice);
    relp_status_t shard_ratio(const double* dev_alpha_slices, int32_t count, double* dev_rho);
    relp_status_t shard_update(const double* dev_rho);
    relp_status_t shard_pivot();
    relp_status_t shard_set_collectives(relp_allgather_fn ag, relp_allreduce_sum_fn ar, void* ctx);
    relp_status_t shard_run(int64_t max_iters, int64_t* done, int32_t* outcome);
    void shard_inject_failure(int64_t after_pivots) { inject_failure_after_ = after_pivots; }
    relp_status_t rccl_attach(const uint8_t* id);
    relp_status_t poll(int32_t* outcome, int64_t* iterations);

    const char* last_error() const { return err_.c_str(); }

  private:
    Layout lay_;
    relp_config_t cfg_{};
    int32_t phase_ = 1;

    double* dA_ = nullptr; int64_t ld_a_ = 0; bool owns_A_ = false;
    double* dBinv_ = nullptr; int64_t ld_b_ = 0;
    double *d_minus_pi_ = nullptr, *d_b_ = nullptr, *d_alpha_ = nullptr, *d_aq_ = nullptr, *d_rho_ = nullptr,
           *d_d_ = nullptr, *d_w_ = nullptr, *d_cost_ = nullptr;
    int32_t *d_basis_ = nullptr, *d_column_to_row_ = nullptr, *d_bound_row_ = nullptr, *d_vrow0_ = nullptr,
            *d_vrow1_ = nullptr, *d_vsign_ = nullptr, *d_trace_ = nullptr;
    uint8_t* d_in_basis_ = nullptr;
    PivotRecord* d_rec_ = nullptr;
    PivotRecord* h_rec_ = nullptr;
    hipStream_t stream_ = nullptr; bool owns_stream_ = false;
    int64_t trace_cap_ = 0;
    int32_t block_ = 0;
    int64_t since_flush_ = 0;
    double* d_v_ = nullptr;
    double *d_W_ = nullptr, *d_wr_ = nullptr, *d_R_ = nullptr;
    int32_t *d_S_ = nullptr, *d_pos_of_row_ = nullptr;
    double* d_part_k1_ = nullptr;
    int32_t* d_part_j_ = nullptr;
    bool tableau_ = false;
    double* dT0_ = nullptr; int64_t ld_t_ = 0;
    double* dR0_ = nullptr; int64_t ld_r_ = 0;
    bool flush_all_ = false;
    int32_t *d_fcols_ = nullptr, *d_fcount_ = nullptr;
    unsigned long long *d_fmask_ = nullptr, *d_fstats_ = nullptr;
    double* d_R0c_ = nullptr;
    FlushList flush_list() const;
    int32_t load_batch_ = 0, w_split_ = 0;
    double* d_cost_store_ = nullptr;
    int32_t* d_idcol_ = nullptr;
    bool fused_update_ = false, shadow_pending_ = false;
    double *d_b_alt_ = nullptr, *d_shadow_ = nullptr;
    int32_t *d_basis_alt_ = nullptr, *d_shadow_meta_ = nullptr;
    double* d_rmin_ = nullptr;
    int32_t n_store_ = 0;
    int32_t tab_na_ = 0;
    bool tab_partials_valid_ = false;
    static constexpr int kRepriceEveryFlushes = 8;
    int32_t flushes_since_reprice_ = 0;
    std::vector<int32_t> idcol_h_;
    std::vector<double> cost_store_h_;
    bool in_loop_ = false;
    void tab_settle();
    struct LoopScope {
        Engine& e;
        explicit LoopScope(Engine& en) : e(en) { e.in_loop_ = true; }
        ~LoopScope() { e.in_loop_ = false; e.tab_settle(); }
    };
    struct SettledScope {
        Engine& e; bool was;
        explicit SettledScope(Engine& en) : e(en), was(en.in_loop_) { e.in_loop_ = false; e.tab_settle(); }
        ~SettledScope() { e.in_loop_ = was; }
    };
    TableauView tview() const;
    double* d_aq_big() { return dR0_ + (int64_t)block_ * ld_r_; }
    SelectPartials tab_partials(int rule) const;
    void enqueue_iteration_tableau(int rule);
    relp_status_t tableau_reprice();
    bool lu_ = false;
    std::vector<int64_t> hc_ptr_; std::vector<int32_t> hc_idx_; std::vector<double> hc_val_;
    int64_t* d_cptr_ = nullptr; int32_t* d_cidx_ = nullptr; double* d_cval_ = nullptr;
    LUFactors hlu_;
    char* d_lu_buf_ = nullptr; int64_t lu_cap_ = 0;
    std::vector<std::vector<std::pair<int32_t, double>>> basis_cols_;
    std::vector<int64_t> basis_ptr_; std::vector<int32_t> basis_idx_; std::vector<double> basis_val_;
    struct HostPool {
        struct Slot { std::thread th; std::mutex mu; std::condition_variable cv; std::function<void()> job; bool busy = false, stop = false; };
        Slot slot[2];
        void run(int i, std::function<void()> f) {
            Slot& s = slot[i];
            if (!s.th.joinable())
                s.th = std::thread([&s] {
                    std::unique_lock<std::mutex> lk(s.mu);
                    for (;;) {
                        s.cv.wait(lk, [&s] { return s.busy || s.stop; });
                        if (s.stop) return;
                        lk.unlock(); s.job(); lk.lock();
                        s.busy = false;
                        s.cv.notify_all();
                    }
                });
            { std::lock_guard<std::mutex> lk(s.mu); s.job = std::move(f); s.busy = true; }
            s.cv.notify_all();
        }
        void wait() {
            for (Slot& s : slot) { std::unique_lock<std::mutex> lk(s.mu); s.cv.wait(lk, [&s] { return !s.busy; }); }
        }
        ~HostPool() {
            for (Slot& s : slot) {
                if (!s.th.joinable()) continue;
                { std::lock_guard<std::mutex> lk(s.mu); s.stop = true; }
                s.cv.notify_all();
                s.th.join();
            }
        }
    } host_pool_;
    char* h_lu_buf_ = nullptr; size_t h_lu_cap_ = 0;
    char* d_lu_buf_alt_ = nullptr; int64_t lu_cap_alt_ = 0;
    int32_t* h_basis_ = nullptr; int32_t m_alloc_rows_ = 0;
    FtMirror* h_mirror_ = nullptr; FtMirror* d_mirror_ = nullptr;
    double* d_lu_scratch_ = nullptr;
    DeviceLU dlu_{};
    relp_status_t lu_status_ = RELP_OK;
    int64_t lu_refactors_ = 0;
    int64_t lu_lookahead_installs_ = 0, lu_replayed_changes_ = 0;
    int32_t lu_lookahead_env_ = 8, lu_fuse_lanes_env_ = 256;
    bool lu_lookahead_set_ = false;
    int32_t lu_pipeline_cap_ = 0;
    double refactor_us_[3] = {0.0, 0.0, 0.0};
    int64_t reinvert_interval_ = 0, since_reinvert_ = 0, reinversions_ = 0;
    DeviceCSC csc() const { return DeviceCSC{d_cptr_, d_cidx_, d_cval_}; }
    auto csc_column() const {
        return [this](int32_t p, auto&& put) { for (int64_t e = hc_ptr_[p]; e < hc_ptr_[p + 1]; ++e) put(hc_idx_[e], hc_val_[e]); };
    }
    relp_status_t lu_load_matrix(const relp_matrix_data_t& md);
    relp_status_t lu_refactor();
    relp_status_t lu_upload_factors();
    relp_status_t reinvert();
    relp_status_t retabulate();
    bool retab_done_ = false;
    relp_status_t build_basis_columns(const std::vector<int32_t>& basis, std::vector<std::vector<std::pair<int32_t, double>>>* cols);
    void enqueue_iteration_lu(int rule);
    bool ft_ = false;
    FtState fts_{};
    char* d_ft_buf_ = nullptr;
    int32_t* h_ft_hdr_ = nullptr;
    int32_t ft_tcap_ = 0, ft_eta_cap_ = 0;
    struct LufState;
    LufState* luf_ = nullptr;
    bool luf_enabled_ = false;
    int64_t luf_runs_ = 0, luf_fallbacks_ = 0, luf_lds_retries_ = 0; double luf_kernel_us_ = 0.0; int32_t luf_last_bump_ = 0, luf_last_peeled_ = 0;
    relp_status_t luf_prepare();
    relp_status_t lu_factor_on_device(int32_t* device_status);
    relp_status_t luf_download_factors();
    relp_status_t lu_host_factors();
    bool luf_is_resident() const;
    bool luf_download_ = false;
    void luf_release();
    void luf_mark_dirty();
    bool hyper_forced_ = false; int32_t hyper_probe_in_[4] = {0, 0, 0, 0};
    bool ft_big_ = false; int32_t ft_rhs_cap_ = 0;
    bool ft_grid_price_ = false;
    int32_t ft_tier_ = 0;
    int64_t ft_zero_bytes_ = 0, ft_ones_bytes_ = 0;
    bool ft_need_refactor_ = false;
    relp_status_t ft_plan_and_alloc();
    relp_status_t ft_reset();
    relp_status_t ft_read_hdr();
    FtProblem ft_problem(int rule) const;
    void ft_enqueue_pivots(const FtState& go, int rule, int64_t left);
    char* d_pe_buf_ = nullptr; PriceEll pe_{};
    relp_status_t ft_build_price_ell();
    relp_status_t run_ft(int64_t max_iters, int64_t* done, int32_t* outcome);
    DeferredUpdate deferred() const;
    void enqueue_flush();
    int32_t n_alloc_ = 0;

    relp_allgather_fn coll_allgather_ = nullptr;
    relp_allreduce_sum_fn coll_allreduce_ = nullptr;
    void* coll_ctx_ = nullptr;
    void* rccl_comm_ = nullptr;
    double* d_msg_cand_ = nullptr;
    double* d_msg_cands_ = nullptr;
    double* d_msg_slice_ = nullptr;
    double* d_msg_slices_ = nullptr;
    double* d_msg_rho_ = nullptr;
    relp_status_t shard_iteration();
    relp_status_t shard_iteration_comm_only(int from_step);
    int coll_step_ = 0;
    int64_t shadow_flush_ = 0;
    relp_status_t shard_agree_on_status(relp_status_t local);
    double* d_msg_status_ = nullptr;
    double* d_msg_statuses_ = nullptr;
    int64_t inject_failure_after_ = -1;
    bool coll_broken_ = false;
    relp_status_t remove_artificial_basis_variables_sharded(std::vector<int32_t>& rows_to_remove);
    void rccl_release();

    bool prof_on_ = false;
    std::vector<hipEvent_t> prof_ev_;
    std::vector<int> prof_kid_;
    bool prof_open_ = false;
    int32_t prof_stride_ = 1;
    int64_t prof_tick_ = 0;

    std::string err_;

    ColumnTable table() const;
    Tolerances tolerances() const;
    bool hip_ok(hipError_t e, const char* what);
    relp_status_t fail(relp_status_t code, const std::string& msg) { err_ = msg; return code; }
    relp_status_t download_rec();
    relp_status_t upload_rec();
    void prof_begin(int kid, hipStream_t on = nullptr);
    void prof_end(hipStream_t on = nullptr);
    void enqueue_price(int cost_mode, const double* vec, const PivotRecord* rec, int32_t p_lo, int32_t p_hi);
    void enqueue_iteration(int rule);
    relp_status_t finish_phase_one(int32_t* outcome);
    relp_status_t remove_artificial_basis_variables(std::vector<int32_t>& rows_to_remove);
    relp_status_t switch_to_phase_two(const std::vector<int32_t>& rows_to_remove);
    std::vector<int32_t> stuck_artificials_;
    relp_status_t run_loop(int64_t max_iters, int64_t* done, int32_t* outcome);
    relp_status_t rescue_unbar_all();
    void auto_reinversion_adapt(const std::vector<double>& before, const std::vector<double>& after);
    std::vector<int32_t> barred_;
    double guard_rel_ = 0.0;
    bool pivot_guard_on_ = false;
    bool hold_phase_end_ = false;
    int64_t rescue_small_pivots_ = 0, rescue_barred_ = 0, rescue_confirmations_ = 0;
    double last_reinvert_drift_ = -1.0;
    relp_status_t remove_rows(const std::vector<int32_t>& rows);
    void free_all();
};

}
```

rust-lp_amd/csrc/relp_kernels.h:

```cpp
#pragma once
#include <hip/hip_runtime.h>
#include <stdint.h>

#include "relp_layout.hpp"

namespace relp {

enum DeviceOutcome : int32_t { DEV_RUNNING = 0, DEV_NO_CANDIDATE = 1, DEV_NO_ROW = 2 };

struct PivotRecord {
    int32_t outcome;
    int32_t q;
    double  d_q;
    int32_t r;
    int32_t leaving;
    double  alpha_r;
    double  b_r;
    double  minus_objective;
    long long iterations;
    int32_t last_selected;
    int32_t phase;
    int32_t owner_has_row;
    int32_t pad_;
    double  key1;
    int32_t n_eta;
    int32_t eta_target;
    int32_t n_eta_old;
    int32_t degenerate;
    int32_t p_now;
    int32_t pad2_;
};

struct DeferredUpdate {
    double*  W;
    int64_t  ld;
    int32_t  kmax;
    int32_t* S;
    int32_t* pos_of_row;
    double*  wr;
    double*  R;
    int32_t  batch;
    int32_t  w_split;
};

struct ColumnTable {
    int32_t nr_artificial;
    int32_t nr_normal;
    int32_t nr_virtual;
    int32_t nr_constraints;
    const int32_t* column_to_row;
    const int32_t* bound_row;
    const int32_t* vrow0;
    const int32_t* vrow1;
    const int32_t* vsign;
    const double*  cost;
};

struct Tolerances { double cost, pivot, zero, tie; int32_t ratio_rule, pivot_guard; double guard_rel; };

struct SelectPartials {
    double*        k1;
    int32_t*       j;
    const uint8_t* in_basis;
    double         tol_cost;
    int32_t        rule;
    int32_t        n;
    int32_t        offset;
    int32_t        nb_struct;
    double         tol_tie;
    int32_t        p_lo;
    int32_t        cols_per_slot;
};

struct LuRow { int32_t k, e0, e1, pad_; double diag; };
struct DeviceSchedule {
    const LuRow* rows;
    const int32_t* idx; const double* val;
    const int32_t* level_ptr;
    int32_t n_levels; int32_t nnz;
    const int32_t* seg; int32_t n_seg; int32_t pad_;
};
struct DeviceLU {
    int32_t m; int32_t pad_;
    const int32_t* rowperm;
    const int32_t* colperm;
    DeviceSchedule Lf, Uf, Ub, Lb;
};
static constexpr int kEllLg = 13;
static constexpr int kEllLgWide = 24;
static constexpr int kEllPadHeaders = 4;
struct EllPass { int32_t lane0, lanes, info, level; };
struct EllSchedule {
    const EllPass*  passes;
    const int32_t*  lvl_pass;
    double*         rdiag;
    double*         sval;
    const double*   oval;
    const int32_t*  rovf;
    const uint16_t* sidx;
    const uint16_t* oidx;
    const int32_t*  via_ptr;
    const int32_t*  via_pos;
    int32_t n_passes, n_levels, m, n_lanes, n_ovf;
    int32_t bytes;
    int32_t rhs_base;
    int32_t n_triv;
    const int32_t* triv;
    const int32_t* reach;
    const int32_t* rhs_src;
    int32_t n_rhs, pad_;
    const int32_t* rhs_pos;
    const uint32_t* triv_bits;
};

struct DeviceCSC { const int64_t* col_ptr; const int32_t* row_idx; const double* values; };

static constexpr int kFtThreads = 512;
static constexpr int kFtWaves = kFtThreads / 64;
static constexpr int kFtMaxSlots = 64;
static constexpr int kFtMaxRows = 1 << 20;
static constexpr int kFtLdsBudget = 156 * 1024;
static constexpr int kFtBitmapBytes = 40 * 1024;
static inline __host__ __device__ int ft_bitmap_shift(int m, int rhs_cap) {
    int s = 0;
    while (((((long long)m + 1 + rhs_cap) >> s) + 64 + (((long long)m) >> s) + 64) / 8 > kFtBitmapBytes) ++s;
    return s;
}
struct FtPivotInfo {
    int32_t u_e0, u_e1;
    int32_t via_u0, via_u1;
    int32_t via_t0, via_t1;
    int32_t lev_ub, pad_;
};
struct FtState {
    int32_t  m, tcap, ldt, eta_cap;
    int32_t* hdr;
    int32_t* slot_pivot;
    int32_t* slot_prev;
    int32_t* slot_live;
    int32_t* tslot;
    double*  TC;
    int32_t* eta_off;
    int32_t* eta_idx; double* eta_val;
    int32_t* spk_off;
    int32_t* spk_idx; double* spk_val;
    const int32_t* inv_rowperm;
    const int32_t* inv_colperm;
    const int32_t* task_uf;
    const int32_t* task_ub;
    EllSchedule ell[4];
    const int32_t* lev_ub;
    const struct FtPivotInfo* pinfo;
    int32_t* journal;
    double*  spike;
    double*  sp_work;
    int32_t  hyper;
    int32_t  pad2_;
    double*  x_work;
    unsigned long long* chunk_mask;
    int32_t* nz_idx; double* nz_val;
    int32_t* rho_idx;
    int32_t* nzc;
    uint32_t* bits_save;
    int32_t  big;
    int32_t  rhs_cap;
    int32_t  stage[4];
    int32_t  stage_bytes;
    int32_t  lds_bytes;
    int32_t  max_updates;
    int32_t  pad_;
    long long* prof;
};
static constexpr int kPriceSlots = 8;
static constexpr int kPriceLongSlots = 24;
static constexpr int kPriceLongFlag = 0x8000;
static constexpr uint32_t kPriceLongFlag32 = 0x80000000u;
struct PriceEll {
    const uint16_t* idx; const double* val;
    const uint16_t* lidx; const double* lval;
    const uint32_t* idx32; const uint32_t* lidx32;
    const int32_t* long_cols;
    const int32_t* very_long;
    const uint16_t* long_of;
    int32_t n_long, n_very_long;
};
struct FtMirror {
    PivotRecord rec;
    int32_t hdr[4];
    int32_t walked[4], whole[4];
    int32_t sweeps[4];
    int32_t basis[1];
};
struct FtProblem {
    DeviceCSC csc; ColumnTable ct; PriceEll pe;
    double *minus_pi, *b, *alpha, *rho, *d;
    int32_t* basis; uint8_t* in_basis; int32_t* trace; int64_t trace_cap;
    PivotRecord* rec;
    FtMirror* mirror;
    Tolerances tol;
    int32_t rule, n, phase;
    int32_t external_price;
};

void launch_price_structural(const double* A, int64_t ld_a, const ColumnTable& ct, const double* minus_pi,
                             double* d, int32_t p_lo, int32_t p_hi, int32_t cost_mode, const PivotRecord* rec,
                             hipStream_t s);
void launch_price_mask_unowned(const ColumnTable& ct, double* d, int32_t p_lo, int32_t p_hi,
                               const PivotRecord* rec, hipStream_t s);
void launch_price_structural_sel(const double* A, int64_t ld_a, const ColumnTable& ct, const double* minus_pi,
                                 double* d, int32_t p_lo, int32_t p_hi, int32_t cost_mode, SelectPartials sp,
                                 const PivotRecord* rec, hipStream_t s);
void launch_price_virtual_sel(const ColumnTable& ct, const double* minus_pi, double* d, int32_t cost_mode,
                              SelectPartials sp, const PivotRecord* rec, hipStream_t s);
void launch_price_all_sel(const double* A, int64_t ld_a, const ColumnTable& ct, const double* minus_pi, double* d,
                          int32_t p_lo, int32_t p_hi, int32_t cost_mode, SelectPartials sp, const PivotRecord* rec,
                          hipStream_t s);
int32_t price_structural_blocks(int32_t p_lo, int32_t p_hi);
int32_t price_virtual_blocks(const ColumnTable& ct);
void launch_select_partials(SelectPartials sp, int32_t count, const double* d, const double* A, int64_t ld_a,
                            const ColumnTable& ct, int32_t m, double* aq, PivotRecord* rec, hipStream_t s);
void launch_price_virtual(const ColumnTable& ct, const double* minus_pi, double* d, int32_t cost_mode,
                          const PivotRecord* rec, hipStream_t s);
void launch_select_column(const double* d, const uint8_t* in_basis, int32_t n, int32_t rule, double tol_cost,
                          double tol_tie, PivotRecord* rec, hipStream_t s);
void launch_build_column(const double* A, int64_t ld_a, const ColumnTable& ct, int32_t m, double* aq,
                         const PivotRecord* rec, hipStream_t s);
void launch_ftran(const double* Binv, int64_t ld_b, int32_t m, int32_t row_lo, int32_t row_hi,
                  const double* aq, double* out, int32_t out_offset, const PivotRecord* rec, hipStream_t s);
void launch_ratio(const double* alpha, const double* b, const int32_t* basis_indices, int32_t m,
                  Tolerances tol, PivotRecord* rec, hipStream_t s);
void launch_compute_rho(const double* Binv, int64_t ld_b, int32_t m, int32_t row_lo, int32_t row_hi,
                        double* rho, PivotRecord* rec, hipStream_t s);
void launch_update_vectors(int32_t m, const double* alpha, const double* rho, double* b, double* minus_pi,
                           int32_t* basis_indices, uint8_t* in_basis, int32_t* trace, int64_t trace_cap,
                           PivotRecord* rec, hipStream_t s);
void launch_update_inverse(double* Binv, int64_t ld_b, int32_t m, int32_t row_lo, int32_t row_hi,
                           const double* alpha, const double* rho, const PivotRecord* rec, hipStream_t s);
void launch_update_inverse_vectors(double* Binv, int64_t ld_b, int32_t m, const double* alpha, const double* rho, double* b,
                                   double* minus_pi, int32_t* basis_indices, uint8_t* in_basis, int32_t* trace,
                                   int64_t trace_cap, PivotRecord* rec, hipStream_t s);

void launch_weighted_column_sums(const double* Binv, int64_t ld_b, int32_t m, const double* w,
                                 double* minus_pi, hipStream_t s);
void launch_set_identity(double* Binv_local, int64_t ld_b, int32_t row_lo, int32_t row_hi, hipStream_t s);
void launch_fill_dense(double* A, int64_t ld, int32_t m, int32_t n, uint64_t seed, int64_t first_column,
                       hipStream_t s);
void launch_csc_to_dense(const int64_t* col_ptr, const int32_t* row_idx, const double* values, int32_t n_cols, double* A,
                         int64_t ld, hipStream_t s);

void launch_apply_w(const DeferredUpdate& du, int32_t m, const double* v, double* alpha, const PivotRecord* rec,
                    hipStream_t s);
int32_t ftran_rows_per_block();
void launch_ftran_rmin(const double* Binv, int64_t ld_b, int32_t m, const double* aq, double* out, const double* b,
                       Tolerances tol, double* rmin, const PivotRecord* rec, hipStream_t s);
void launch_apply_w_rmin(const DeferredUpdate& du, int32_t m, const double* v, double* alpha, const double* b, Tolerances tol,
                         double* rmin, const PivotRecord* rec, hipStream_t s);
void launch_ratio_rows(const double* alpha, const double* b, const int32_t* basis_indices, int32_t m, Tolerances tol,
                       const DeferredUpdate& du, const double* rmin, int32_t rows_per_block, PivotRecord* rec, hipStream_t s);
void launch_eta_prepare(const DeferredUpdate& du, PivotRecord* rec, hipStream_t s);
void launch_update_w(const DeferredUpdate& du, int32_t m, const double* alpha, const PivotRecord* rec, hipStream_t s);
void launch_rho_deferred(const DeferredUpdate& du, const double* Binv, int64_t ld_b, int32_t m, int32_t row_lo,
                         int32_t row_hi, double* rho, PivotRecord* rec, hipStream_t s);
void launch_flush_snapshot(const DeferredUpdate& du, const double* Binv, int64_t ld_b, int32_t row_lo, int32_t row_hi,
                           const PivotRecord* rec, hipStream_t s);
void launch_flush_apply(const DeferredUpdate& du, double* Binv, int64_t ld_b, int32_t m, int32_t row_lo,
                        int32_t row_hi, const PivotRecord* rec, hipStream_t s);
void launch_flush_reset(const DeferredUpdate& du, PivotRecord* rec, hipStream_t s);

struct TableauView {
    double*  T0;      int64_t ld_t;
    double*  R0;      int64_t ld_r;
    double*  d;
    int32_t  m;
    int32_t  n_store;
    int32_t  col_off;
    int32_t  n;
    int32_t  c_lo, c_hi;
};
void launch_tab_build(const TableauView& tv, const double* A, int64_t ld_a, const ColumnTable& ct, hipStream_t s);
void launch_tab_price_init(const TableauView& tv, const double* w, const double* cost_store, hipStream_t s);
void launch_tab_basis_costs(const TableauView& tv, const int32_t* basis_indices, const double* cost_store, double* w,
                            hipStream_t s);
void launch_tab_scan(const TableauView& tv, SelectPartials sp, const PivotRecord* rec, hipStream_t s);
int32_t tab_scan_blocks(int32_t n_owned_columns);
bool launch_lu_ftran_cols(const DeviceLU& lu, const TableauView& tv, const double* A, int64_t ld_a, const ColumnTable& ct,
                          int32_t c_first, int32_t c_count, hipStream_t s);
void launch_tab_select(const TableauView& tv, SelectPartials sp, int32_t count, PivotRecord* rec, hipStream_t s);
void launch_tab_column(const TableauView& tv, const DeferredUpdate& du, double* alpha, const PivotRecord* rec,
                       hipStream_t s);
void launch_tab_row_update(const TableauView& tv, const DeferredUpdate& du, SelectPartials sp, PivotRecord* rec,
                           hipStream_t s);
void launch_tab_update_vectors(int32_t m, const double* alpha, double* b, int32_t* basis_indices, uint8_t* in_basis,
                               int32_t* trace, int64_t trace_cap, PivotRecord* rec, hipStream_t s);
void launch_tab_select_column_rmin(const TableauView& tv, const DeferredUpdate& du, SelectPartials sp, int32_t count,
                                   double* alpha, const double* b, Tolerances tol, double* rmin, PivotRecord* rec,
                                   hipStream_t s, const double* shadow = nullptr, int32_t* shadow_meta = nullptr);
void launch_ratio_blocks(const double* alpha, const double* b, const int32_t* basis_indices, int32_t m, Tolerances tol,
                         const DeferredUpdate& du, const double* rmin, PivotRecord* rec, hipStream_t s);
void launch_tab_select_column_msg(const TableauView& tv, const DeferredUpdate& du, SelectPartials sp, int32_t count,
                                  double* msg, const double* b, Tolerances tol, PivotRecord* rec, hipStream_t s,
                                  const double* shadow = nullptr, int32_t* shadow_meta = nullptr);
void launch_tab_select_candidate_ratio(const double* msgs, int32_t count, int64_t msg_len, int32_t m, double* alpha,
                                       const double* b, const int32_t* basis_indices, int32_t rule, Tolerances tol,
                                       const DeferredUpdate& du, int32_t forced_row, PivotRecord* rec, hipStream_t s);
void launch_tab_zero_level_scan(const TableauView& tv, const DeferredUpdate& du, SelectPartials sp, int32_t row,
                                int32_t nr_artificial, Tolerances tol, const PivotRecord* rec, hipStream_t s);
void launch_tab_update_all(const TableauView& tv, const DeferredUpdate& du, SelectPartials sp, int32_t m,
                           const double* alpha, double* b, int32_t* basis_indices, uint8_t* in_basis, int32_t* trace,
                           int64_t trace_cap, PivotRecord* rec, hipStream_t s);
struct FlushList {
    int32_t*            cols;
    int32_t*            count;
    unsigned long long* mask;
    double*             R0c;
    int64_t             ld;
    unsigned long long* stats;
};
static constexpr int32_t kTabLoadBatchDefault = 8;
static constexpr int32_t kTabSplitDefault = 2;
static constexpr int32_t kTabSplitCUs = 256;
int32_t tab_load_batch(int32_t wanted);
void launch_tab_flush(const TableauView& tv, const DeferredUpdate& du, const PivotRecord* rec, const FlushList& fl,
                      hipStream_t s);
void launch_tab_ratio_update_all(const TableauView& tv, const DeferredUpdate& du, SelectPartials sp, int32_t m,
                                 const double* alpha, const double* b_in, double* b_out, const int32_t* basis_in,
                                 int32_t* basis_out, uint8_t* in_basis, int32_t* trace, int64_t trace_cap, Tolerances tol,
                                 const double* rmin, double* shadow, int32_t* shadow_meta, PivotRecord* rec, hipStream_t s,
                                 const double* msgs = nullptr, int32_t count = 0, int64_t msg_len = 0, int32_t rule = 0);
void launch_tab_apply_shadow(const DeferredUpdate& du, double* shadow, int32_t* shadow_meta, hipStream_t s);
void launch_tab_gather_columns(const TableauView& tv, const int32_t* cols, double* out, hipStream_t s);
void launch_tab_row(const TableauView& tv, const DeferredUpdate& du, int32_t row, double* out, const PivotRecord* rec,
                    hipStream_t s);

void launch_price_csc(const DeviceCSC& csc, const ColumnTable& ct, const double* vec, double* d, int32_t p_lo,
                      int32_t p_hi, int32_t cost_mode, SelectPartials sp, const PivotRecord* rec, hipStream_t s);
void launch_price_csc_all(const DeviceCSC& csc, const ColumnTable& ct, const double* vec, double* d, int32_t nr_normal,
                          int32_t cost_mode, SelectPartials sp, int32_t nb_virtual, const PivotRecord* rec, hipStream_t s);
int32_t price_csc_blocks(int32_t p_lo, int32_t p_hi);
void launch_select_partials_csc(SelectPartials sp, int32_t count, const double* d, const DeviceCSC& csc,
                                const ColumnTable& ct, int32_t m, double* aq, PivotRecord* rec, hipStream_t s);
void launch_build_column_csc(const DeviceCSC& csc, const ColumnTable& ct, int32_t m, double* aq, const PivotRecord* rec,
                             hipStream_t s);
void launch_lu_ftran(const DeviceLU& lu, const double* aq, double* v, double* scratch, const PivotRecord* rec,
                     hipStream_t s);
void launch_lu_btran(const DeviceLU& lu, const DeferredUpdate& du, const double* rhs, int32_t row, double* rho,
// ... 23 lines not shown
```

rust-lp_amd/csrc/relp_kernels_tableau.hip:

```cpp
#include "relp_device_common.h"
#include <type_traits>

namespace relp {

typedef double double4_t __attribute__((ext_vector_type(4)));

template <int B, class Use>
__device__ __forceinline__ void for_pending(const double* base, int64_t stride, int64_t x, int n, Use&& use) {
    int j0 = 0;
    for (; j0 + B <= n; j0 += B) {
        double v[B];
#pragma unroll
        for (int t = 0; t < B; ++t) v[t] = base[(int64_t)(j0 + t) * stride + x];
#pragma unroll
        for (int t = 0; t < B; ++t) use(j0 + t, v[t]);
    }
    if (B > 1 && j0 < n) {
        double v[B];
#pragma unroll
        for (int t = 0; t < B; ++t) v[t] = j0 + t < n ? base[(int64_t)(j0 + t) * stride + x] : 0.0;
#pragma unroll
        for (int t = 0; t < B; ++t)
            if (j0 + t < n) use(j0 + t, v[t]);
    }
}

template <int B>
__device__ __forceinline__ void tab_update_w_row(const DeferredUpdate& du, int i, double u, const double* s_wr, int j0, int j1) {
    if (u == 0.0 || j1 <= j0) return;
    double* col = du.W + (int64_t)j0 * du.ld;
    for_pending<B>(col, du.ld, i, j1 - j0, [&](int j, double old) {
        const double w = s_wr[j0 + j];
        if (w != 0.0) col[(int64_t)j * du.ld + i] = fma(u, w, old);
    });
}

__global__ void k_tab_build(TableauView tv, const double* __restrict__ A, int64_t ld_a, ColumnTable ct) {
    const int64_t total = (int64_t)tv.m * (tv.c_hi - tv.c_lo);
    for (int64_t idx = (int64_t)blockIdx.x * blockDim.x + threadIdx.x; idx < total; idx += (int64_t)gridDim.x * blockDim.x) {
        const int c = tv.c_lo + (int)(idx / tv.m), i = (int)(idx % tv.m);
        double v = 0.0;
        if (c < ct.nr_artificial) {
            v = (i == ct.column_to_row[c]) ? 1.0 : 0.0;
        } else {
            const int p = c - ct.nr_artificial;
            if (p < ct.nr_normal) {
                if (i < ct.nr_constraints) v = A[(int64_t)p * ld_a + i];
                else v = (i == ct.bound_row[p]) ? 1.0 : 0.0;
            } else {
                const int vv = p - ct.nr_normal;
                if (i == ct.vrow0[vv]) v = (double)ct.vsign[vv];
                else if (i == ct.vrow1[vv]) v = 1.0;
            }
        }
        tv.T0[(int64_t)c * tv.ld_t + i] = v;
    }
}

__global__ __launch_bounds__(kThreads) void k_tab_price_init(TableauView tv, const double* __restrict__ w,
                                                             const double* __restrict__ cost_store) {
    __shared__ double s_partial[4 * kVecPerBlock];
    const int v0 = tv.c_lo + blockIdx.x * kVecPerBlock;
    double dot = 0.0;
    block_multi_dot(tv.T0, tv.ld_t, tv.m, v0, tv.c_hi, w, s_partial, dot);
    const int c = v0 + threadIdx.x;
    if (threadIdx.x < kVecPerBlock && c < tv.c_hi) tv.d[c] = cost_store[c] - dot;
}

__global__ void k_tab_basis_costs(const int32_t* __restrict__ basis_indices, const double* __restrict__ cost_store,
                                  int col_off, int n_store, int m, double* __restrict__ w) {
    const int i = blockIdx.x * blockDim.x + threadIdx.x;
    if (i >= m) return;
    const int j = basis_indices[i];
    const int c = j + col_off;
    w[i] = (j < kWrappedArtificialBase && c >= 0 && c < n_store) ? cost_store[c] : 0.0;
}

__global__ __launch_bounds__(kThreads) void k_tab_scan(TableauView tv, SelectPartials sp, const PivotRecord* rec) {
    if (rec->outcome != DEV_RUNNING) return;
    const int c = tv.c_lo + blockIdx.x * kThreads + threadIdx.x;
    const int j = c - tv.col_off;
    double key = INFINITY;
    int kj = 0x7fffffff;
    if (c < tv.c_hi && j >= 0 && j < tv.n) {
        const double v = tv.d[c];
        if (!sp.in_basis[j] && v < -sp.tol_cost) { key = select_key(sp.rule, sp.n, rec, j, v); kj = j; }
    }
    block_partial_min(key, kj, sp, blockIdx.x);
}

__global__ __launch_bounds__(kSingleBlock) void k_tab_select(TableauView tv, SelectPartials sp, int count,
                                                             PivotRecord* rec) {
    if (rec->outcome != DEV_RUNNING) return;
    double k1 = INFINITY;
    int bj = 0x7fffffff;
    if ((int)threadIdx.x < count) { k1 = sp.k1[threadIdx.x]; bj = sp.j[threadIdx.x]; }
    tab_select_entering<kSingleBlock>(tv, sp, count, k1, bj);
    if (threadIdx.x == 0) {
        if (bj == 0x7fffffff) {
            rec->outcome = DEV_NO_CANDIDATE;
            if (sp.rule == 1) rec->last_selected = -1;
        } else {
            rec->q = bj;
            rec->d_q = tv.d[bj + tv.col_off];
            rec->key1 = k1;
            if (sp.rule == 1) rec->last_selected = bj;
        }
    }
}

template <int B>
__global__ __launch_bounds__(kThreads) void k_tab_column(TableauView tv, DeferredUpdate du, double* __restrict__ alpha,
                                                         const PivotRecord* rec) {
    if (rec->outcome != DEV_RUNNING) return;
    __shared__ double s_vs[kMaxEta];
    const int p = rec->n_eta;
    const int cq = rec->q + tv.col_off;
    if ((int)threadIdx.x < p) s_vs[threadIdx.x] = tv.R0[(int64_t)threadIdx.x * tv.ld_r + cq];
    __syncthreads();
    const int i = blockIdx.x * kThreads + threadIdx.x;
    if (i >= tv.m) return;
    double a = tv.T0[(int64_t)cq * tv.ld_t + i];
    for_pending<B>(du.W, du.ld, i, p, [&](int j, double w) { a = fma(w, s_vs[j], a); });
    alpha[i] = a;
}

template <int B>
__device__ __forceinline__ void tab_row_update_core(const TableauView& tv, const DeferredUpdate& du, const SelectPartials& sp,
                                                    const PivotRecord& R, int block, const double* s_wr, int p_old, int jt, int r,
                                                    int q, int leaving, double d_q, double alpha_r) {
    const PivotRecord* rec = &R;
    const int c = tv.c_lo + block * kThreads + threadIdx.x;
    const double d_old = c < tv.c_hi ? tv.d[c] : 0.0;
    __syncthreads();
    double key = INFINITY;
    int kj = 0x7fffffff;
    if (c < tv.c_hi) {
        double base;
        if (jt < p_old) base = tv.R0[(int64_t)jt * tv.ld_r + c];
        else {
            base = tv.T0[(int64_t)c * tv.ld_t + r];
            tv.R0[(int64_t)jt * tv.ld_r + c] = base;
        }
        double row = base;
        for_pending<B>(tv.R0, tv.ld_r, c, p_old, [&](int j, double r0) { row = fma(s_wr[j], r0, row); });
        const double theta = d_q / alpha_r;
        const int j = c - tv.col_off;
        double dn = fma(-theta, row, d_old);
        if (j == q) dn = 0.0;
        tv.d[c] = dn;
        if (j >= 0 && j < tv.n) {
            const bool basic = (j == q) || (sp.in_basis[j] && j != leaving);
            if (!basic && dn < -sp.tol_cost) { key = select_key(sp.rule, sp.n, rec, j, dn); kj = j; }
        }
    }
    block_partial_min(key, kj, sp, block);
}

template <int B>
__device__ __forceinline__ void tab_row_update_body(const TableauView& tv, const DeferredUpdate& du,
                                                    const SelectPartials& sp, const PivotRecord& R, int block) {
    __shared__ double s_wr[kMaxEta];
    if ((int)threadIdx.x < du.kmax) s_wr[threadIdx.x] = du.wr[threadIdx.x];
    tab_row_update_core<B>(tv, du, sp, R, block, s_wr, R.n_eta_old, R.eta_target, R.r, R.q, R.leaving, R.d_q, R.alpha_r);
}

template <int B>
__global__ __launch_bounds__(kThreads) void k_tab_row_update(TableauView tv, DeferredUpdate du, SelectPartials sp,
                                                             PivotRecord* rec) {
    const PivotRecord R = *rec;
    if (R.outcome != DEV_RUNNING) return;
    tab_row_update_body<B>(tv, du, sp, R, blockIdx.x);
}

template <int B>
__device__ __forceinline__ void tab_update_w_vectors_body(const DeferredUpdate& du, int m, const double* __restrict__ alpha,
                                                          double* __restrict__ b, int32_t* __restrict__ basis_indices,
                                                          uint8_t* __restrict__ in_basis, int32_t* __restrict__ trace,
                                                          int64_t trace_cap, const PivotRecord& R, PivotRecord* rec,
                                                          int block) {
    __shared__ double s_wr2[kMaxEta];
    const int p_old = R.n_eta_old, jt = R.eta_target, r = R.r;
    if ((int)threadIdx.x < du.kmax) s_wr2[threadIdx.x] = du.wr[threadIdx.x];
    const int i = block * kThreads + threadIdx.x;
    const double a_i = i < m ? alpha[i] : 0.0;
    const double b_i = i < m ? b[i] : 0.0;
    __syncthreads();
    const double ar = R.alpha_r;
    const double br = R.b_r / ar;
    if (i < m) {
        const double a = a_i;
        const double u = (i == r) ? (1.0 / ar - 1.0) : (-a / ar);
        tab_update_w_row<B>(du, i, u, s_wr2, 0, p_old);
        double* tgt = du.W + (int64_t)jt * du.ld + i;
        if (jt < p_old) *tgt += u; else *tgt = u;
        b[i] = pivot_b(a, b_i, br, i == r);
    }
    if (i == 0) {
        basis_indices[r] = R.q;
        pivot_bookkeeping(R.phase, R.iterations, R.minus_objective, R.d_q, br, R.q, r, R.leaving, in_basis, trace, trace_cap, rec);
    }
}

template <int B>
__global__ __launch_bounds__(kThreads) void k_tab_update_all(TableauView tv, DeferredUpdate du, SelectPartials sp,
                                                             int nb_row, int m, const double* __restrict__ alpha,
                                                             double* __restrict__ b, int32_t* __restrict__ basis_indices,
                                                             uint8_t* __restrict__ in_basis, int32_t* __restrict__ trace,
                                                             int64_t trace_cap, PivotRecord* rec) {
    const PivotRecord R = *rec;
    if (R.outcome != DEV_RUNNING) return;
    if ((int)blockIdx.x < nb_row) tab_row_update_body<B>(tv, du, sp, R, blockIdx.x);
    else tab_update_w_vectors_body<B>(du, m, alpha, b, basis_indices, in_basis, trace, trace_cap, R, rec, blockIdx.x - nb_row);
}

template <int B>
__global__ __launch_bounds__(kThreads) void k_tab_ratio_update_all(TableauView tv, DeferredUpdate du, SelectPartials sp, int nb_row,
                                                                   int m, const double* alpha,
                                                                   const double* __restrict__ b_in, double* __restrict__ b_out,
                                                                   const int32_t* __restrict__ basis_in,
                                                                   int32_t* __restrict__ basis_out, uint8_t* in_basis,
                                                                   int32_t* __restrict__ trace, int64_t trace_cap, Tolerances tol,
                                                                   const double* rmin, int nblk,
                                                                   double* __restrict__ shadow, int32_t* __restrict__ shadow_meta,
                                                                   PivotRecord* rec, const double* __restrict__ msgs, int count,
                                                                   int64_t msg_len, int rule, int split) {
    const double first = (!msgs && (int)threadIdx.x < nblk) ? rmin[threadIdx.x] : INFINITY;
    PivotRecord R = *rec;
    const bool w_half = (int)blockIdx.x >= nb_row;
    const int part = w_half ? ((int)blockIdx.x - nb_row) / nblk : 0;
    const int wblock = (int)blockIdx.x - nb_row - part * nblk;
    const int i = wblock * kThreads + threadIdx.x;
    const bool lead = w_half && part == 0;
    const bool mine = lead && i < m;
    if (R.outcome != DEV_RUNNING) {
        if (mine) { b_out[i] = b_in[i]; basis_out[i] = basis_in[i]; }
        return;
    }
    if (msgs) {
        int q_win = 0;
        double d_win = 0.0;
        const int win = candidate_winner_staged(msgs, count, msg_len, rule, tol.tie, &q_win, &d_win);
        if (win < 0) {
            if (mine) { b_out[i] = b_in[i]; basis_out[i] = basis_in[i]; }
            if (lead && wblock == 0 && threadIdx.x == 0) record_candidate(rec, rule, -1, 0, 0.0);
            return;
        }
        R.q = q_win;
        R.d_q = d_win;
        if (rule == 1) R.last_selected = R.q;
        alpha = msgs + win * msg_len + 3;
        rmin = alpha + m;
    }
    int r, leaving;
    ratio_blocks_pick<kThreads>(alpha, b_in, basis_in, m, tol, rmin, nblk, &r, &leaving, first, !msgs);
    if (r < 0) {
        if (mine) { b_out[i] = b_in[i]; basis_out[i] = basis_in[i]; }
        if (lead && wblock == 0 && threadIdx.x == 0) rec->outcome = DEV_NO_ROW;
        return;
    }
    __shared__ double s_wr[kMaxEta];
    __shared__ double s_ab[2];
    __shared__ int s_jt;
    const int p_old = R.p_now;
    if ((int)threadIdx.x < p_old) s_wr[threadIdx.x] = du.W[(int64_t)threadIdx.x * du.ld + r];
    if (threadIdx.x == 0) {
        s_ab[0] = alpha[r]; s_ab[1] = b_in[r];
        const int slot = du.pos_of_row[r];
        s_jt = slot < 0 ? p_old : slot;
    }
    __syncthreads();
    const double alpha_r = s_ab[0], b_r = s_ab[1];
    const int jt = s_jt, q = R.q;
    if (!w_half) {
        tab_row_update_core<B>(tv, du, sp, R, blockIdx.x, s_wr, p_old, jt, r, q, leaving, R.d_q, alpha_r);
        return;
    }
    const double br = b_r / alpha_r;
    const int share = (p_old + split - 1) / split;
    const int j_lo = min(part * share, p_old), j_hi = min(j_lo + share, p_old);
    if (!lead) {
        if (i < m && i != r) {
            const double u = -alpha[i] / alpha_r;
            tab_update_w_row<B>(du, i, u, s_wr, j_lo, j_hi);
            if (jt >= j_lo && jt < j_hi) du.W[(int64_t)jt * du.ld + i] += u;
        }
        return;
    }
    if (i < m) {
        const double a = alpha[i], b_i = b_in[i];
        const double u = (i == r) ? (1.0 / alpha_r - 1.0) : (-a / alpha_r);
        if (i != r) {
            tab_update_w_row<B>(du, i, u, s_wr, j_lo, j_hi);
            double* tgt = du.W + (int64_t)jt * du.ld + i;
            if (jt >= p_old) *tgt = u;
            else if (jt < j_hi) *tgt += u;
        } else {
            for (int j = 0; j < p_old; ++j) {
                const double w = s_wr[j];
                shadow[j] = (u != 0.0 && w != 0.0) ? fma(u, w, w) : w;
            }
            if (jt < p_old) shadow[jt] += u; else shadow[jt] = u;
            shadow_meta[0] = r;
            shadow_meta[1] = jt < p_old ? p_old : p_old + 1;
        }
        b_out[i] = pivot_b(a, b_i, br, i == r);
        basis_out[i] = (i == r) ? q : basis_in[i];
    }
    if (i == 0) {
        if (msgs) record_candidate(rec, rule, 0, q, R.d_q);
        rec->r = r; rec->leaving = leaving; rec->alpha_r = alpha_r; rec->b_r = b_r;
        rec->n_eta_old = p_old; rec->eta_target = jt;
        if (jt >= p_old) { du.S[p_old] = r; du.pos_of_row[r] = p_old; rec->n_eta = p_old + 1; }
        pivot_bookkeeping(R.phase, R.iterations, R.minus_objective, R.d_q, br, q, r, leaving, in_basis, trace, trace_cap, rec);
    }
}

__global__ void k_tab_apply_shadow(DeferredUpdate du, double* __restrict__ shadow, int32_t* __restrict__ shadow_meta) {
    const int row = shadow_meta[0], len = shadow_meta[1];
    if (row < 0) return;
    for (int j = threadIdx.x; j < len; j += blockDim.x) du.W[(int64_t)j * du.ld + row] = shadow[j];
    __syncthreads();
    if (threadIdx.x == 0) shadow_meta[0] = -1;
}

template <int B>
__global__ __launch_bounds__(kThreads) void k_tab_select_column(TableauView tv, DeferredUpdate du, SelectPartials sp,
                                                                int count, double* alpha, double* msg,
                                                                const double* b, Tolerances tol,
                                                                double* rmin, PivotRecord* rec,
                                                                const double* shadow, int32_t* shadow_meta) {
    const int outcome = rec->outcome, p = rec->n_eta;
    if (shadow_meta) {
        const int srow = shadow_meta[0], slen = shadow_meta[1];
        if (srow >= 0 && srow / kThreads == (int)blockIdx.x) {
            if ((int)threadIdx.x < slen) du.W[(int64_t)threadIdx.x * du.ld + srow] = shadow[threadIdx.x];
            __syncthreads();
            if (threadIdx.x == 0) shadow_meta[0] = -1;
        }
        if (blockIdx.x == 0 && threadIdx.x == 0) rec->p_now = p;
    }
    double k1 = INFINITY;
    int bj = 0x7fffffff;
    if ((int)threadIdx.x < count) { k1 = sp.k1[threadIdx.x]; bj = sp.j[threadIdx.x]; }
    const int i = blockIdx.x * kThreads + threadIdx.x;
    const double b_i = (rmin && i < tv.m) ? b[i] : 0.0;
    if (outcome != DEV_RUNNING) return;
    __shared__ double s_vs[kMaxEta];
    __shared__ double s_min[kThreads / 64];
    tab_select_entering<kThreads>(tv, sp, count, k1, bj);
    if (bj == 0x7fffffff) {
        if (msg) {
            if (i < tv.m) alpha[i] = 0.0;
            if (i == 0) { msg[0] = INFINITY; msg[1] = 0.0; msg[2] = 0.0; }
        } else if (blockIdx.x == 0 && threadIdx.x == 0) {
            rec->outcome = DEV_NO_CANDIDATE;
            if (sp.rule == 1) rec->last_selected = -1;
        }
        return;
    }
    const int cq = bj + tv.col_off;
    if (blockIdx.x == 0 && threadIdx.x == 0) {
        if (msg) { msg[0] = k1; msg[1] = (double)bj; msg[2] = tv.d[cq]; }
        else {
            rec->q = bj;
            rec->d_q = tv.d[cq];
            rec->key1 = k1;
            if (sp.rule == 1) rec->last_selected = bj;
        }
    }
    if ((int)threadIdx.x < p) s_vs[threadIdx.x] = tv.R0[(int64_t)threadIdx.x * tv.ld_r + cq];
    const double t0 = i < tv.m ? tv.T0[(int64_t)cq * tv.ld_t + i] : 0.0;
    __syncthreads();
    double ratio = INFINITY;
    if (i < tv.m) {
        double a = t0;
        for_pending<B>(du.W, du.ld, i, p, [&](int j, double w) { a = fma(w, s_vs[j], a); });
        alpha[i] = a;
        const double bz = b_i <= tol.zero ? 0.0 : b_i;
        if (a > tol.pivot) ratio = bz / a;
    }
    if (!rmin) return;
#pragma unroll
    for (int off = 32; off > 0; off >>= 1) ratio = fmin(ratio, __shfl_down(ratio, off, 64));
    if ((threadIdx.x & 63) == 0) s_min[threadIdx.x >> 6] = ratio;
    __syncthreads();
    if (threadIdx.x == 0) rmin[blockIdx.x] = fmin(fmin(s_min[0], s_min[1]), fmin(s_min[2], s_min[3]));
}

__global__ __launch_bounds__(kSingleBlock) void k_ratio_blocks(const double* __restrict__ alpha, const double* __restrict__ b,
                                                               const int32_t* __restrict__ basis_indices, int m,
                                                               Tolerances tol, DeferredUpdate du,
                                                               const double* __restrict__ rmin, int nblk, PivotRecord* rec) {
    const int outcome = rec->outcome, p = rec->n_eta;
    const double first = (int)threadIdx.x < nblk ? rmin[threadIdx.x] : INFINITY;
    if (outcome != DEV_RUNNING) return;
    ratio_blocks_body<kSingleBlock>(alpha, b, basis_indices, m, tol, du, rmin, nblk, p, rec, first, true);
}

__global__ __launch_bounds__(kSingleBlock) void k_tab_select_candidate_ratio(const double* __restrict__ msgs, int count,
                                                                             int64_t msg_len, int m, double* __restrict__ alpha,
                                                                             const double* __restrict__ b,
                                                                             const int32_t* __restrict__ basis_indices,
                                                                             int rule, Tolerances tol, DeferredUpdate du,
                                                                             int forced_row, PivotRecord* rec) {
    const int outcome = rec->outcome, p = rec->n_eta;
    if (outcome != DEV_RUNNING) return;
    int q = 0;
    double d_q = 0.0;
    const int win = candidate_winner_staged(msgs, count, msg_len, rule, tol.tie, &q, &d_q);
    if (threadIdx.x == 0) record_candidate(rec, rule, win, q, d_q);
    if (win < 0) return;
    const double* __restrict__ col = msgs + win * msg_len + 3;
    const int nblk = (m + kThreads - 1) / kThreads;
    if (forced_row >= 0) {
        for (int i = threadIdx.x; i < m; i += kSingleBlock) alpha[i] = col[i];
        ratio_commit_row<kSingleBlock>(forced_row, basis_indices[forced_row], col, b, du, p, rec);
        return;
    }
    const double first = (int)threadIdx.x < nblk ? col[m + threadIdx.x] : INFINITY;
    constexpr int kCopy = 16;
    double cp[kCopy];
#pragma unroll
    for (int u = 0; u < kCopy; ++u) {
        const int i = threadIdx.x + u * kSingleBlock;
        cp[u] = i < m ? col[i] : 0.0;
    }
    ratio_blocks_body<kSingleBlock>(col, b, basis_indices, m, tol, du, col + m, nblk, p, rec, first, true);
#pragma unroll
    for (int u = 0; u < kCopy; ++u) {
        const int i = threadIdx.x + u * kSingleBlock;
        if (i < m) alpha[i] = cp[u];
    }
    for (int i = threadIdx.x + kCopy * kSingleBlock; i < m; i += kSingleBlock) alpha[i] = col[i];
}

__global__ void k_tab_update_vectors(int m, const double* __restrict__ alpha, double* __restrict__ b,
                                     int32_t* __restrict__ basis_indices, uint8_t* __restrict__ in_basis,
                                     int32_t* __restrict__ trace, int64_t trace_cap, PivotRecord* rec) {
    if (rec->outcome != DEV_RUNNING) return;
    const int i = blockIdx.x * blockDim.x + threadIdx.x;
    const int r = rec->r;
    const double br = rec->b_r / rec->alpha_r;
    if (i < m) b[i] = pivot_b(alpha[i], b[i], br, i == r);
    if (i == 0) {
        basis_indices[r] = rec->q;
        pivot_bookkeeping(rec->phase, rec->iterations, rec->minus_objective, rec->d_q, br, rec->q, r, rec->leaving, in_basis, trace,
                          trace_cap, rec);
    }
}

template <int MT, int NT>
__global__ __launch_bounds__(kThreads) void k_tab_flush(TableauView tv, DeferredUpdate du, const int32_t* p_dev,
                                                        unsigned long long* stats) {
    constexpr int kFlushMT = MT, kFlushNT = NT;
    const int p = *p_dev;
    if (p == 0) return;
    if (stats && blockIdx.x == 0 && blockIdx.y == 0 && threadIdx.x == 0) { stats[0] += 1; stats[1] += tv.c_hi - tv.c_lo; }
    const int lane = threadIdx.x & 63, wave = threadIdx.x >> 6;
    const int c_wave = tv.c_lo + blockIdx.x * (2 * 16 * MT) + (wave & 1) * (16 * MT);
    const int i_wave = blockIdx.y * (2 * 16 * NT) + (wave >> 1) * (16 * NT);
    if (c_wave >= tv.c_hi || i_wave >= tv.m) return;
    const int lm = lane & 15, lk = lane >> 4;
    double4_t acc[kFlushMT][kFlushNT];
#pragma unroll
    for (int a = 0; a < kFlushMT; ++a)
#pragma unroll
        for (int b = 0; b < kFlushNT; ++b)
#pragma unroll
            for (int g = 0; g < 4; ++g) {
                const int c = c_wave + a * 16 + lk + 4 * g;
                const int i = i_wave + b * 16 + lm;
                acc[a][b][g] = (c < tv.c_hi && i < tv.m) ? tv.T0[(int64_t)c * tv.ld_t + i] : 0.0;
            }
    double af[kFlushMT], bf[kFlushNT], afn[kFlushMT], bfn[kFlushNT];
    auto load_frags = [&](int k0, double* fa, double* fb) {
        const int k = k0 + lk;
        const bool kv = k < p;
#pragma unroll
        for (int a = 0; a < kFlushMT; ++a) {
            const int c = c_wave + a * 16 + lm;
            fa[a] = (kv && c < tv.c_hi) ? tv.R0[(int64_t)k * tv.ld_r + c] : 0.0;
        }
#pragma unroll
        for (int b = 0; b < kFlushNT; ++b) {
            const int i = i_wave + b * 16 + lm;
            fb[b] = (kv && i < tv.m) ? du.W[(int64_t)k * du.ld + i] : 0.0;
        }
    };
    load_frags(0, af, bf);
    for (int k0 = 0; k0 < p; k0 += 4) {
        load_frags(k0 + 4, afn, bfn);
#pragma unroll
        for (int a = 0; a < kFlushMT; ++a)
#pragma unroll
            for (int b = 0; b < kFlushNT; ++b)
                acc[a][b] = __builtin_amdgcn_mfma_f64_16x16x4f64(af[a], bf[b], acc[a][b], 0, 0, 0);
#pragma unroll
        for (int a = 0; a < kFlushMT; ++a) af[a] = afn[a];
#pragma unroll
        for (int b = 0; b < kFlushNT; ++b) bf[b] = bfn[b];
    }
#pragma unroll
    for (int a = 0; a < kFlushMT; ++a)
#pragma unroll
        for (int b = 0; b < kFlushNT; ++b)
#pragma unroll
            for (int g = 0; g < 4; ++g) {
                const int c = c_wave + a * 16 + lk + 4 * g;
                const int i = i_wave + b * 16 + lm;
                if (c < tv.c_hi && i < tv.m) tv.T0[(int64_t)c * tv.ld_t + i] = acc[a][b][g];
            }
}

template <int WC, int WR, int KC, bool kList>
__global__ __launch_bounds__(WC * WR * 64) void k_tab_flush_lds(TableauView tv, DeferredUpdate du, const int32_t* p_dev,
                                                                FlushList fl) {
    constexpr int MT = 4, NT = 2;
    constexpr int TC = WC * 16 * MT, TR = WR * 16 * NT, NTHR = WC * WR * 64;
    constexpr int RA = KC * TC / 2 / NTHR, RB = KC * TR / 2 / NTHR;
    static_assert(RA * NTHR * 2 == KC * TC && RB * NTHR * 2 == KC * TR, "staging must divide evenly");
    const int p = *p_dev;
    const int n_cols = kList ? *fl.count : tv.c_hi - tv.c_lo;
    if (p == 0) return;
    if (kList && (int)blockIdx.y * TC >= n_cols) return;
    if (!kList && fl.stats && blockIdx.x == 0 && blockIdx.y == 0 && threadIdx.x == 0) { fl.stats[0] += 1; fl.stats[1] += n_cols; }
    __shared__ __align__(16) double As[2][KC][TC];
    __shared__ __align__(16) double Bs[2][KC][TR];
    const int tid = threadIdx.x, lane = tid & 63, wave = tid >> 6;
    const int wc = wave % WC, wr = wave / WC;
    const int x_blk = blockIdx.y * TC, i_blk = blockIdx.x * TR;
    const int x_wave = x_blk + wc * 16 * MT, i_wave = i_blk + wr * 16 * NT;
    const bool active = x_wave < n_cols && i_wave < tv.m;
    const int lm = lane & 15, lk = lane >> 4;
    const double* a_src = kList ? fl.R0c : tv.R0 + tv.c_lo;
    const int64_t a_ld = kList ? fl.ld : tv.ld_r;
    const int col_lane = kList && active && x_wave + lane < n_cols ? fl.cols[x_wave + lane] : -1;
    auto column = [&](int a, int g) -> int {
        const int x = a * 16 + lk + 4 * g;
        if (kList) return __shfl(col_lane, x, 64);
        return x_wave + x < n_cols ? tv.c_lo + x_wave + x : -1;
    };
    double2 ra[RA], rb[RB];
    auto gload = [&](int kc) {
#pragma unroll
        for (int u = 0; u < RA; ++u) {
            const int idx = tid + NTHR * u, k = idx / (TC / 2), x = x_blk + 2 * (idx % (TC / 2));
            ra[u] = (kc + k < p && x < a_ld) ? *reinterpret_cast<const double2*>(a_src + (int64_t)(kc + k) * a_ld + x)
                                             : make_double2(0.0, 0.0);
        }
#pragma unroll
        for (int u = 0; u < RB; ++u) {
            const int idx = tid + NTHR * u, k = idx / (TR / 2), i = i_blk + 2 * (idx % (TR / 2));
            rb[u] = (kc + k < p && i < (int)du.ld) ? *reinterpret_cast<const double2*>(du.W + (int64_t)(kc + k) * du.ld + i)
                                                   : make_double2(0.0, 0.0);
        }
    };
    auto lstore = [&](int buf) {
#pragma unroll
        for (int u = 0; u < RA; ++u) {
            const int idx = tid + NTHR * u;
            *reinterpret_cast<double2*>(&As[buf][idx / (TC / 2)][2 * (idx % (TC / 2))]) = ra[u];
        }
#pragma unroll
        for (int u = 0; u < RB; ++u) {
            const int idx = tid + NTHR * u;
            *reinterpret_cast<double2*>(&Bs[buf][idx / (TR / 2)][2 * (idx % (TR / 2))]) = rb[u];
        }
    };
    gload(0);
    double4_t acc[MT][NT];
#pragma unroll
    for (int a = 0; a < MT; ++a)
#pragma unroll
        for (int b = 0; b < NT; ++b)
#pragma unroll
            for (int g = 0; g < 4; ++g) {
                const int c = column(a, g);
                const int i = i_wave + b * 16 + lm;
                acc[a][b][g] = (active && c >= 0 && i < tv.m) ? tv.T0[(int64_t)c * tv.ld_t + i] : 0.0;
            }
    lstore(0);
    __syncthreads();
    const int nchunks = (p + KC - 1) / KC;
    for (int ch = 0; ch < nchunks; ++ch) {
        const int buf = ch & 1;
        if (ch + 1 < nchunks) gload((ch + 1) * KC);
        if (active) {
            const int kmax = min(KC, p - ch * KC);
            for (int k0 = 0; k0 < kmax; k0 += 4) {
                double af[MT], bf[NT];
#pragma unroll
                for (int a = 0; a < MT; ++a) af[a] = As[buf][k0 + lk][wc * 16 * MT + a * 16 + lm];
#pragma unroll
                for (int b = 0; b < NT; ++b) bf[b] = Bs[buf][k0 + lk][wr * 16 * NT + b * 16 + lm];
#pragma unroll
                for (int a = 0; a < MT; ++a)
#pragma unroll
                    for (int b = 0; b < NT; ++b)
                        acc[a][b] = __builtin_amdgcn_mfma_f64_16x16x4f64(af[a], bf[b], acc[a][b], 0, 0, 0);
            }
        }
        if (ch + 1 < nchunks) lstore(buf ^ 1);
        __syncthreads();
    }
    if (!active) return;
#pragma unroll
    for (int a = 0; a < MT; ++a)
#pragma unroll
        for (int b = 0; b < NT; ++b)
#pragma unroll
            for (int g = 0; g < 4; ++g) {
                const int c = column(a, g);
                const int i = i_wave + b * 16 + lm;
                if (c >= 0 && i < tv.m) tv.T0[(int64_t)c * tv.ld_t + i] = acc[a][b][g];
            }
}

__global__ __launch_bounds__(kThreads) void k_tab_flush_mark(TableauView tv, FlushList fl, const int32_t* p_dev) {
    const int p = *p_dev;
    if (p == 0) return;
    __shared__ unsigned long long s_mask[kThreads / 64];
    const int lane = threadIdx.x & 63, wave = threadIdx.x >> 6;
    const int c = tv.c_lo + blockIdx.x * 64 + lane;
    bool nz = false;
    if (c < tv.c_hi) {
        for (int j0 = wave; j0 < p; j0 += 4 * 8) {
            double v[8];
#pragma unroll
            for (int u = 0; u < 8; ++u) v[u] = j0 + 4 * u < p ? tv.R0[(int64_t)(j0 + 4 * u) * tv.ld_r + c] : 0.0;
#pragma unroll
            for (int u = 0; u < 8; ++u) nz |= !(v[u] == 0.0);
        }
    }
    const unsigned long long m = __ballot(nz);
    if (lane == 0) s_mask[wave] = m;
    __syncthreads();
    if (threadIdx.x == 0) fl.mask[blockIdx.x] = s_mask[0] | s_mask[1] | s_mask[2] | s_mask[3];
}

__global__ __launch_bounds__(kThreads) void k_tab_flush_compact(TableauView tv, FlushList fl, const int32_t* p_dev, int nb) {
    const int p = *p_dev;
    if (p == 0) return;
    __shared__ int s_before[kThreads / 64];
    const int lane = threadIdx.x & 63, wave = threadIdx.x >> 6;
    int before = 0;
    for (int b = threadIdx.x; b < (int)blockIdx.x; b += kThreads) before += __popcll(fl.mask[b]);
#pragma unroll
    for (int off = 32; off > 0; off >>= 1) before += __shfl_down(before, off, 64);
    if (lane == 0) s_before[wave] = before;
    __syncthreads();
    before = s_before[0] + s_before[1] + s_before[2] + s_before[3];
    const unsigned long long mask = fl.mask[blockIdx.x];
    if ((mask >> lane) & 1ull) {
        const int c = tv.c_lo + blockIdx.x * 64 + lane;
        const int x = before + __popcll(mask & ((1ull << lane) - 1ull));
        if (wave == 0) fl.cols[x] = c;
        for (int j0 = wave; j0 < p; j0 += 4 * 8) {
            double v[8];
#pragma unroll
            for (int u = 0; u < 8; ++u) v[u] = j0 + 4 * u < p ? tv.R0[(int64_t)(j0 + 4 * u) * tv.ld_r + c] : 0.0;
#pragma unroll
            for (int u = 0; u < 8; ++u)
                if (j0 + 4 * u < p) fl.R0c[(int64_t)(j0 + 4 * u) * fl.ld + x] = v[u];
        }
    }
    if ((int)blockIdx.x == nb - 1 && threadIdx.x == 0) {
        const int count = before + __popcll(mask);
        *fl.count = count;
        fl.stats[0] += 1;
        fl.stats[1] += count;
    }
}

__global__ void k_tab_gather_columns(TableauView tv, const int32_t* __restrict__ cols, double* __restrict__ out) {
    const int64_t total = (int64_t)tv.m * tv.m;
    for (int64_t idx = (int64_t)blockIdx.x * blockDim.x + threadIdx.x; idx < total; idx += (int64_t)gridDim.x * blockDim.x) {
        const int k = (int)(idx / tv.m), i = (int)(idx % tv.m);
        out[(int64_t)i * tv.m + k] = tv.T0[(int64_t)cols[k] * tv.ld_t + i];
    }
}

template <int B>
__global__ __launch_bounds__(kThreads) void k_tab_row(TableauView tv, DeferredUpdate du, int row, double* __restrict__ out,
                                                      const PivotRecord* rec) {
    __shared__ double s_w[kMaxEta];
    const int p = rec->n_eta;
    if ((int)threadIdx.x < p) s_w[threadIdx.x] = du.W[(int64_t)threadIdx.x * du.ld + row];
    __syncthreads();
    const int c = tv.c_lo + blockIdx.x * kThreads + threadIdx.x;
    if (c >= tv.c_hi) return;
    double v = tv.T0[(int64_t)c * tv.ld_t + row];
    for_pending<B>(tv.R0, tv.ld_r, c, p, [&](int j, double r0) { v = fma(s_w[j], r0, v); });
    out[c - tv.c_lo] = v;
}

template <int B>
__global__ __launch_bounds__(kThreads) void k_tab_zero_level_scan(TableauView tv, DeferredUpdate du, SelectPartials sp, int row,
                                                                  int nr_artificial, Tolerances tol, const PivotRecord* rec) {
    const int outcome = rec->outcome, p = rec->n_eta;
    if (outcome != DEV_RUNNING) return;
    __shared__ double s_w[kMaxEta];
    if ((int)threadIdx.x < p) s_w[threadIdx.x] = du.W[(int64_t)threadIdx.x * du.ld + row];
    __syncthreads();
    const int c = tv.c_lo + blockIdx.x * kThreads + threadIdx.x;
    const int j = c - tv.col_off;
    double key = INFINITY;
    int kj = 0x7fffffff;
    if (c < tv.c_hi && j >= nr_artificial && j < tv.n && !sp.in_basis[j] && fabs(tv.d[c]) <= tol.cost) {
        double v = tv.T0[(int64_t)c * tv.ld_t + row];
        for_pending<B>(tv.R0, tv.ld_r, c, p, [&](int k, double r0) { v = fma(s_w[k], r0, v); });
        if (fabs(v) > tol.pivot) { key = (double)j; kj = j; }
    }
    block_partial_min(key, kj, sp, blockIdx.x);
}

int32_t tab_scan_blocks(int32_t n_owned_columns) { return cdiv(n_owned_columns, kThreads); }

int32_t tab_load_batch(int32_t wanted) {
    return (wanted == 1 || wanted == 8 || wanted == 16 || wanted == 32) ? wanted : kTabLoadBatchDefault;
}

template <class Launch>
static void with_load_batch(int32_t batch, Launch&& launch) {
    switch (tab_load_batch(batch)) {
    case 1:  launch(std::integral_constant<int, 1>{}); break;
    case 16: launch(std::integral_constant<int, 16>{}); break;
    case 32: launch(std::integral_constant<int, 32>{}); break;
    default: launch(std::integral_constant<int, 8>{}); break;
    }
    static_assert(kTabLoadBatchDefault == 8, "the default of tab_load_batch is the switch's default case");
}

void launch_tab_build(const TableauView& tv, const double* A, int64_t ld_a, const ColumnTable& ct, hipStream_t s) {
    const int64_t total = (int64_t)tv.m * (tv.c_hi - tv.c_lo);
    if (total <= 0) return;
    hipLaunchKernelGGL(k_tab_build, dim3(element_blocks(total)), dim3(256), 0, s, tv, A, ld_a, ct);
}

void launch_tab_price_init(const TableauView& tv, const double* w, const double* cost_store, hipStream_t s) {
    if (tv.c_hi <= tv.c_lo) return;
    hipLaunchKernelGGL(k_tab_price_init, dim3(cdiv(tv.c_hi - tv.c_lo, kVecPerBlock)), dim3(kThreads), 0, s, tv, w,
                       cost_store);
}

void launch_tab_basis_costs(const TableauView& tv, const int32_t* basis_indices, const double* cost_store, double* w,
                            hipStream_t s) {
    hipLaunchKernelGGL(k_tab_basis_costs, dim3(cdiv(tv.m, 256)), dim3(256), 0, s, basis_indices, cost_store, tv.col_off,
                       tv.n_store, tv.m, w);
}

void launch_tab_scan(const TableauView& tv, SelectPartials sp, const PivotRecord* rec, hipStream_t s) {
    if (tv.c_hi <= tv.c_lo) return;
    hipLaunchKernelGGL(k_tab_scan, dim3(tab_scan_blocks(tv.c_hi - tv.c_lo)), dim3(kThreads), 0, s, tv, sp, rec);
}

void launch_tab_select(const TableauView& tv, SelectPartials sp, int32_t count, PivotRecord* rec, hipStream_t s) {
    hipLaunchKernelGGL(k_tab_select, dim3(1), dim3(kSingleBlock), 0, s, tv, sp, count, rec);
}

void launch_tab_column(const TableauView& tv, const DeferredUpdate& du, double* alpha, const PivotRecord* rec,
                       hipStream_t s) {
    with_load_batch(du.batch, [&](auto B) {
        hipLaunchKernelGGL((k_tab_column<decltype(B)::value>), dim3(cdiv(tv.m, kThreads)), dim3(kThreads), 0, s, tv, du, alpha, rec);
    });
}

void launch_tab_row_update(const TableauView& tv, const DeferredUpdate& du, SelectPartials sp, PivotRecord* rec,
                           hipStream_t s) {
    if (tv.c_hi <= tv.c_lo) return;
    with_load_batch(du.batch, [&](auto B) {
        hipLaunchKernelGGL((k_tab_row_update<decltype(B)::value>), dim3(tab_scan_blocks(tv.c_hi - tv.c_lo)), dim3(kThreads), 0, s, tv, du, sp,
                           rec);
    });
}

void launch_tab_update_vectors(int32_t m, const double* alpha, double* b, int32_t* basis_indices, uint8_t* in_basis,
                               int32_t* trace, int64_t trace_cap, PivotRecord* rec, hipStream_t s) {
    hipLaunchKernelGGL(k_tab_update_vectors, dim3(cdiv(m, 256)), dim3(256), 0, s, m, alpha, b, basis_indices, in_basis,
                       trace, trace_cap, rec);
}

void launch_tab_select_column_rmin(const TableauView& tv, const DeferredUpdate& du, SelectPartials sp, int32_t count,
                                   double* alpha, const double* b, Tolerances tol, double* rmin, PivotRecord* rec,
                                   hipStream_t s, const double* shadow, int32_t* shadow_meta) {
    with_load_batch(du.batch, [&](auto B) {
        hipLaunchKernelGGL((k_tab_select_column<decltype(B)::value>), dim3(cdiv(tv.m, kThreads)), dim3(kThreads), 0, s, tv, du, sp, count, alpha,
                           (double*)nullptr, b, tol, rmin, rec, shadow, shadow_meta);
    });
}

void launch_tab_ratio_update_all(const TableauView& tv, const DeferredUpdate& du, SelectPartials sp, int32_t m,
                                 const double* alpha, const double* b_in, double* b_out, const int32_t* basis_in,
                                 int32_t* basis_out, uint8_t* in_basis, int32_t* trace, int64_t trace_cap, Tolerances tol,
                                 const double* rmin, double* shadow, int32_t* shadow_meta, PivotRecord* rec, hipStream_t s,
                                 const double* msgs, int32_t count, int64_t msg_len, int32_t rule) {
    const int nb_row = tv.c_hi > tv.c_lo ? tab_scan_blocks(tv.c_hi - tv.c_lo) : 0;
    const int nb_w = cdiv(m, kThreads);
    int split = tab_load_batch(du.batch) == 1 ? 1 : std::max(1, std::min({(int)du.w_split, (int)du.kmax, (kTabSplitCUs - nb_row) / nb_w}));
    with_load_batch(du.batch, [&](auto B) {
        hipLaunchKernelGGL((k_tab_ratio_update_all<decltype(B)::value>), dim3(nb_row + split * nb_w), dim3(kThreads), 0, s, tv, du, sp, nb_row, m,
                           alpha, b_in, b_out, basis_in, basis_out, in_basis, trace, trace_cap, tol, rmin, nb_w, shadow,
                           shadow_meta, rec, msgs, (int)count, msg_len, (int)rule, split);
    });
}

void launch_tab_apply_shadow(const DeferredUpdate& du, double* shadow, int32_t* shadow_meta, hipStream_t s) {
    hipLaunchKernelGGL(k_tab_apply_shadow, dim3(1), dim3(128), 0, s, du, shadow, shadow_meta);
}

void launch_ratio_blocks(const double* alpha, const double* b, const int32_t* basis_indices, int32_t m, Tolerances tol,
                         const DeferredUpdate& du, const double* rmin, PivotRecord* rec, hipStream_t s) {
    hipLaunchKernelGGL(k_ratio_blocks, dim3(1), dim3(kSingleBlock), 0, s, alpha, b, basis_indices, m, tol, du, rmin,
                       cdiv(m, kThreads), rec);
}

void launch_tab_select_column_msg(const TableauView& tv, const DeferredUpdate& du, SelectPartials sp, int32_t count,
                                  double* msg, const double* b, Tolerances tol, PivotRecord* rec, hipStream_t s,
                                  const double* shadow, int32_t* shadow_meta) {
    with_load_batch(du.batch, [&](auto B) {
        hipLaunchKernelGGL((k_tab_select_column<decltype(B)::value>), dim3(cdiv(tv.m, kThreads)), dim3(kThreads), 0, s, tv, du, sp, count, msg + 3,
                           msg, b, tol, msg + 3 + tv.m, rec, shadow, shadow_meta);
    });
}

void launch_tab_select_candidate_ratio(const double* msgs, int32_t count, int64_t msg_len, int32_t m, double* alpha,
                                       const double* b, const int32_t* basis_indices, int32_t rule, Tolerances tol,
                                       const DeferredUpdate& du, int32_t forced_row, PivotRecord* rec, hipStream_t s) {
    hipLaunchKernelGGL(k_tab_select_candidate_ratio, dim3(1), dim3(kSingleBlock), 0, s, msgs, count, msg_len, m, alpha, b,
                       basis_indices, rule, tol, du, forced_row, rec);
}

void launch_tab_zero_level_scan(const TableauView& tv, const DeferredUpdate& du, SelectPartials sp, int32_t row,
                                int32_t nr_artificial, Tolerances tol, const PivotRecord* rec, hipStream_t s) {
    if (tv.c_hi <= tv.c_lo) return;
    with_load_batch(du.batch, [&](auto B) {
        hipLaunchKernelGGL((k_tab_zero_level_scan<decltype(B)::value>), dim3(tab_scan_blocks(tv.c_hi - tv.c_lo)), dim3(kThreads), 0, s, tv, du, sp,
                           row, nr_artificial, tol, rec);
    });
}

void launch_tab_update_all(const TableauView& tv, const DeferredUpdate& du, SelectPartials sp, int32_t m,
                           const double* alpha, double* b, int32_t* basis_indices, uint8_t* in_basis, int32_t* trace,
                           int64_t trace_cap, PivotRecord* rec, hipStream_t s) {
    const int nb_row = tv.c_hi > tv.c_lo ? tab_scan_blocks(tv.c_hi - tv.c_lo) : 0;
    const int nb_w = cdiv(m, kThreads);
    with_load_batch(du.batch, [&](auto B) {
        hipLaunchKernelGGL((k_tab_update_all<decltype(B)::value>), dim3(nb_row + nb_w), dim3(kThreads), 0, s, tv, du, sp, nb_row, m, alpha, b,
                           basis_indices, in_basis, trace, trace_cap, rec);
    });
}

void launch_tab_flush(const TableauView& tv, const DeferredUpdate& du, const PivotRecord* rec, const FlushList& fl,
                      hipStream_t s) {
    if (tv.c_hi <= tv.c_lo) return;
    const int ncols = tv.c_hi - tv.c_lo;
    const int32_t* p_dev = &rec->n_eta;
    if ((int64_t)ncols * tv.m >= (1 << 16)) {
        constexpr int WC = 2, WR = 4, KC = 16;
        dim3 grid(cdiv(tv.m, WR * 32), cdiv(ncols, WC * 64));
        if (fl.cols) {
            const int nb = cdiv(ncols, 64);
            hipLaunchKernelGGL(k_tab_flush_mark, dim3(nb), dim3(kThreads), 0, s, tv, fl, p_dev);
            hipLaunchKernelGGL(k_tab_flush_compact, dim3(nb), dim3(kThreads), 0, s, tv, fl, p_dev, nb);
            hipLaunchKernelGGL((k_tab_flush_lds<WC, WR, KC, true>), grid, dim3(WC * WR * 64), 0, s, tv, du, p_dev, fl);
        } else {
            hipLaunchKernelGGL((k_tab_flush_lds<WC, WR, KC, false>), grid, dim3(WC * WR * 64), 0, s, tv, du, p_dev, fl);
        }
        return;
    }
    constexpr int MT = 4, NT = 2;
    dim3 grid(cdiv(ncols, 2 * 16 * MT), cdiv(tv.m, 2 * 16 * NT));
    hipLaunchKernelGGL((k_tab_flush<MT, NT>), grid, dim3(kThreads), 0, s, tv, du, p_dev, fl.stats);
}

void launch_tab_gather_columns(const TableauView& tv, const int32_t* cols, double* out, hipStream_t s) {
    const int64_t total = (int64_t)tv.m * tv.m;
    hipLaunchKernelGGL(k_tab_gather_columns, dim3(element_blocks(total)), dim3(256), 0, s, tv, cols, out);
}

void launch_tab_row(const TableauView& tv, const DeferredUpdate& du, int32_t row, double* out, const PivotRecord* rec,
                    hipStream_t s) {
    if (tv.c_hi <= tv.c_lo) return;
    with_load_batch(du.batch, [&](auto B) {
        hipLaunchKernelGGL((k_tab_row<decltype(B)::value>), dim3(tab_scan_blocks(tv.c_hi - tv.c_lo)), dim3(kThreads), 0, s, tv, du, row, out, rec);
    });
}


}
```

rust-lp_amd/engine.py:

```python
from __future__ import annotations

import ctypes as C
import os
from typing import List, Optional, Tuple

import numpy as np

from .matrix_data import MatrixData

_HERE = os.path.dirname(os.path.abspath(__file__))
LIB_PATH = os.path.join(_HERE, "librelp_engine.so")

FIRST_PROFITABLE, FIRST_PROFITABLE_WITH_MEMORY, STEEPEST_DESCENT = 0, 1, 2
RUNNING, OPTIMAL, UNBOUNDED, INFEASIBLE, PHASE_ONE_DONE, NO_ROW_PHASE_ONE = range(6)
OUTCOME_NAMES = {RUNNING: "running", OPTIMAL: "optimal", UNBOUNDED: "unbounded", INFEASIBLE: "infeasible",
                 PHASE_ONE_DONE: "phase_one_done", NO_ROW_PHASE_ONE: "no_row_phase_one"}
(K_PRICE, K_SELECT_COLUMN, K_BUILD_COLUMN, K_FTRAN, K_RATIO, K_UPDATE_VECTORS, K_UPDATE_INVERSE, K_APPLY_W,
 K_UPDATE_W, K_FLUSH, K_FT_RUN) = range(11)
KERNEL_NAMES = ["price", "select_column", "build_column", "ftran", "ratio", "update_vectors", "update_inverse",
                "apply_w", "update_w", "flush", "ft_run"]
ENGINE_REVISED, ENGINE_TABLEAU, ENGINE_LU, ENGINE_AUTO = 0, 1, 2, 3
RATIO_REFERENCE, RATIO_LARGEST_PIVOT = 0, 1
ARTIFICIAL_REFERENCE, ARTIFICIAL_TEXTBOOK = 0, 1
E_ARG, E_HIP, E_ZERO_PIVOT, E_SINGULAR, E_STATE, E_UNSUPPORTED, E_ALLOC = -1, -2, -3, -4, -5, -6, -7
FORMAT_CSC, FORMAT_DENSE = 0, 1
MEM_HOST, MEM_DEVICE = 0, 1


class RelpError(RuntimeError):
    pass


class _MatrixData(C.Structure):
    _fields_ = [("nr_normal", C.c_int32), ("nr_eq", C.c_int32), ("nr_range", C.c_int32), ("nr_le", C.c_int32),
                ("nr_ge", C.c_int32), ("format", C.c_int32), ("matrix_memory", C.c_int32),
                ("col_ptr", C.c_void_p), ("row_idx", C.c_void_p), ("values", C.c_void_p),
                ("dense", C.c_void_p), ("dense_ld", C.c_int64),
                ("b", C.c_void_p), ("ranges", C.c_void_p), ("cost", C.c_void_p), ("upper_bound", C.c_void_p)]


class Config(C.Structure):
    _fields_ = [("device", C.c_int32), ("phase_one_rule", C.c_int32), ("phase_two_rule", C.c_int32),
                ("tol_cost", C.c_double), ("tol_pivot", C.c_double), ("tol_zero", C.c_double),
                ("tol_tie", C.c_double), ("tol_feas", C.c_double),
                ("poll_interval", C.c_int32), ("trace_capacity", C.c_int32),
                ("shard_rank", C.c_int32), ("shard_count", C.c_int32),
                ("update_block", C.c_int32), ("engine", C.c_int32),
                ("ratio_rule", C.c_int32), ("artificial_removal", C.c_int32),
                ("pivot_rescue", C.c_int32), ("auto_reinversion", C.c_int32)]


_SIGNATURES = {
    "relp_default_config": (None, [C.POINTER(Config)]),
    "relp_robust_config": (None, [C.POINTER(Config)]),
    "relp_engine_kind": (C.c_int32, [C.c_void_p]),
    "relp_robust_stats": (C.c_int, [C.c_void_p, C.POINTER(C.c_int64)]),
    "relp_last_error": (C.c_char_p, [C.c_void_p]),
    "relp_version": (C.c_char_p, []),
    "relp_engine_create": (C.c_int, [C.POINTER(_MatrixData), C.POINTER(Config), C.POINTER(C.c_void_p)]),
    "relp_engine_destroy": (None, [C.c_void_p]),
    "relp_set_stream": (C.c_int, [C.c_void_p, C.c_void_p]),
    "relp_select_primal_pivot_column": (C.c_int, [C.c_void_p, C.c_int32, C.POINTER(C.c_int32), C.POINTER(C.c_int32),
                                                  C.POINTER(C.c_double)]),
    "relp_relative_costs": (C.c_int, [C.c_void_p, C.c_void_p]),
    "relp_generate_column": (C.c_int, [C.c_void_p, C.c_int32, C.c_void_p]),
    "relp_generate_element": (C.c_int, [C.c_void_p, C.c_int32, C.c_int32, C.POINTER(C.c_double)]),
    "relp_select_primal_pivot_row": (C.c_int, [C.c_void_p, C.POINTER(C.c_int32), C.POINTER(C.c_int32)]),
    "relp_select_primal_pivot_row_of": (C.c_int, [C.c_void_p, C.POINTER(C.c_double), C.POINTER(C.c_int32), C.POINTER(C.c_int32)]),
    "relp_bring_into_basis": (C.c_int, [C.c_void_p, C.c_int32, C.c_int32, C.c_double, C.POINTER(C.c_int32)]),
    "relp_run": (C.c_int, [C.c_void_p, C.c_int64, C.POINTER(C.c_int64), C.POINTER(C.c_int32)]),
    "relp_solve_relaxation": (C.c_int, [C.c_void_p, C.c_int64, C.POINTER(C.c_int32)]),
    "relp_from_basis": (C.c_int, [C.c_void_p, C.c_void_p]),
    "relp_flush": (C.c_int, [C.c_void_p]),
    "relp_update_block": (C.c_int32, [C.c_void_p]),
    "relp_tab_load_batch": (C.c_int32, [C.c_void_p]),
    "relp_tab_flush_stats": (C.c_int, [C.c_void_p, C.POINTER(C.c_int64)]),
    "relp_lu_stats": (C.c_int, [C.c_void_p, C.POINTER(C.c_int64)]),
    "relp_lu_lookahead_stats": (C.c_int, [C.c_void_p, C.POINTER(C.c_int64)]),
    "relp_lu_kernel_layout": (C.c_int, [C.c_void_p, C.POINTER(C.c_int32)]),
    "relp_lu_set_device_factorisation": (C.c_int, [C.c_void_p, C.c_int32]),
    "relp_lu_device_factorisation_stats": (C.c_int, [C.c_void_p, C.POINTER(C.c_int64)]),
    "relp_lu_factor_residual": (C.c_int, [C.c_void_p, C.POINTER(C.c_double)]),
    "relp_lu_phase_cycles": (C.c_int, [C.c_void_p, C.POINTER(C.c_int64)]),
    "relp_basis_inverse_row": (C.c_int, [C.c_void_p, C.c_int32, C.c_void_p]),
    "relp_should_refactor": (C.c_int, [C.c_void_p, C.POINTER(C.c_int32)]),
    "relp_generate_column_of": (C.c_int, [C.c_void_p, C.c_void_p, C.c_void_p, C.c_int32, C.c_void_p]),
    "relp_cost_difference_of": (C.c_int, [C.c_void_p, C.c_void_p, C.c_void_p, C.c_int32, C.POINTER(C.c_double)]),
    "relp_lu_change_basis": (C.c_int, [C.c_void_p, C.c_int32]),
    "relp_lu_set_factors": (C.c_int, [C.c_void_p] + [C.c_void_p] * 6),
    "relp_lu_updates": (C.c_int, [C.c_void_p, C.POINTER(C.c_int32)]),
    "relp_lu_get_update": (C.c_int, [C.c_void_p, C.c_int32, C.POINTER(C.c_int32), C.c_void_p, C.c_void_p, C.c_int32, C.POINTER(C.c_int32)]),
    "relp_lu_get_upper": (C.c_int, [C.c_void_p, C.c_void_p, C.c_void_p, C.c_void_p, C.c_int64, C.POINTER(C.c_int64)]),
    "relp_shard_flush_begin": (C.c_int, [C.c_void_p, C.POINTER(C.c_void_p), C.POINTER(C.c_int64)]),
    "relp_shard_flush_end": (C.c_int, [C.c_void_p]),
    "relp_nr_rows": (C.c_int32, [C.c_void_p]),
    "relp_nr_columns": (C.c_int32, [C.c_void_p]),
    "relp_phase": (C.c_int32, [C.c_void_p]),
    "relp_nr_artificial": (C.c_int32, [C.c_void_p]),
    "relp_get_objective": (C.c_int, [C.c_void_p, C.POINTER(C.c_double)]),
    "relp_get_b": (C.c_int, [C.c_void_p, C.c_void_p]),
    "relp_get_minus_pi": (C.c_int, [C.c_void_p, C.c_void_p]),
    "relp_get_basis_indices": (C.c_int, [C.c_void_p, C.c_void_p]),
    "relp_get_basis_inverse": (C.c_int, [C.c_void_p, C.c_void_p]),
    "relp_current_bfs": (C.c_int, [C.c_void_p, C.c_void_p, C.c_void_p, C.c_int32, C.POINTER(C.c_int32)]),
    "relp_get_iterations": (C.c_int, [C.c_void_p, C.POINTER(C.c_int64)]),
    "relp_get_degenerate_pivots": (C.c_int, [C.c_void_p, C.POINTER(C.c_int64)]),
    "relp_get_trace": (C.c_int, [C.c_void_p, C.c_void_p, C.c_void_p, C.c_void_p, C.c_void_p, C.c_int64,
                                 C.POINTER(C.c_int64)]),
    "relp_check_basis": (C.c_int, [C.c_void_p, C.POINTER(C.c_double), C.POINTER(C.c_double), C.POINTER(C.c_double)]),
    "relp_profile_enable": (C.c_int, [C.c_void_p, C.c_int32, C.c_int64, C.c_int32]),
    "relp_profile_read": (C.c_int, [C.c_void_p, C.c_int32, C.POINTER(C.c_int64), C.POINTER(C.c_double)]),
    "relp_synth_fill_dense": (C.c_int, [C.c_void_p, C.c_int64, C.c_int32, C.c_int32, C.c_uint64, C.c_int64, C.c_void_p]),
    "relp_device_alloc": (C.c_int, [C.POINTER(C.c_void_p), C.c_int64]),
    "relp_device_free": (C.c_int, [C.c_void_p]),
    "relp_shard_ranges": (C.c_int, [C.c_void_p] + [C.POINTER(C.c_int32)] * 5),
    "relp_shard_column_range": (None, [C.c_int32, C.c_int32, C.c_int32, C.POINTER(C.c_int32), C.POINTER(C.c_int32)]),
    "relp_shard_candidate_len": (C.c_int64, [C.c_void_p]),
    "relp_shard_rho_len": (C.c_int64, [C.c_void_p]),
    "relp_shard_price": (C.c_int, [C.c_void_p, C.c_void_p]),
    "relp_shard_select_column": (C.c_int, [C.c_void_p, C.c_void_p, C.c_int32]),
    "relp_shard_ftran": (C.c_int, [C.c_void_p, C.c_void_p]),
    "relp_shard_ratio": (C.c_int, [C.c_void_p, C.c_void_p, C.c_int32, C.c_void_p]),
    "relp_shard_update": (C.c_int, [C.c_void_p, C.c_void_p]),
    "relp_poll": (C.c_int, [C.c_void_p, C.POINTER(C.c_int32), C.POINTER(C.c_int64)]),
    "relp_shard_pivot": (C.c_int, [C.c_void_p]),
    "relp_set_reinversion_interval": (C.c_int, [C.c_void_p, C.c_int64]),
    "relp_reinversions": (C.c_int64, [C.c_void_p]),
    "relp_shard_set_collectives": (C.c_int, [C.c_void_p, C.c_void_p, C.c_void_p, C.c_void_p]),
    "relp_shard_run": (C.c_int, [C.c_void_p, C.c_int64, C.POINTER(C.c_int64), C.POINTER(C.c_int32)]),
    "relp_shard_inject_failure": (C.c_int, [C.c_void_p, C.c_int64]),
    "relp_rccl_unique_id": (C.c_int, [C.POINTER(C.c_uint8)]),
    "relp_rccl_attach": (C.c_int, [C.c_void_p, C.POINTER(C.c_uint8)]),
    "relp_shard_plan": (C.c_int, [C.POINTER(_MatrixData), C.POINTER(Config), C.POINTER(C.c_int32), C.POINTER(C.c_int32)]),
}

_lib = None


def load_library():
    global _lib
    if _lib is None:
        if not os.path.exists(LIB_PATH):
            raise RelpError(f"{LIB_PATH} is missing: run `python -c 'import __graft_entry__ as g; g.build()'` "
                            "(hipcc --offload-arch=gfx950).  There is no CPU fallback.")
        lib = C.CDLL(LIB_PATH)
        for name, (res, args) in _SIGNATURES.items():
            fn = getattr(lib, name)
            fn.restype = res
            fn.argtypes = args
        _lib = lib
    return _lib


def default_config(**overrides) -> Config:
    cfg = Config()
    load_library().relp_default_config(C.byref(cfg))
    for k, v in overrides.items():
        if not hasattr(cfg, k):
            raise TypeError(f"unknown config field {k}")
        setattr(cfg, k, v)
    return cfg


def robust_config(**overrides) -> Config:
    cfg = Config()
    load_library().relp_robust_config(C.byref(cfg))
    for k, v in overrides.items():
        if not hasattr(cfg, k):
            raise TypeError(f"unknown config field {k}")
        setattr(cfg, k, v)
    return cfg


def shard_column_range(nr_normal: int, rank: int, count: int) -> Tuple[int, int]:
    lo, hi = C.c_int32(), C.c_int32()
    load_library().relp_shard_column_range(nr_normal, rank, count, C.byref(lo), C.byref(hi))
    return lo.value, hi.value


def shard_plan(provider: MatrixData, config: Config) -> Tuple[int, int]:
    md = _MatrixData()
    md.nr_normal, md.nr_eq, md.nr_range = provider.nr_normal, provider.nr_eq, provider.nr_range
    md.nr_le, md.nr_ge = provider.nr_le, provider.nr_ge
    ub = np.ascontiguousarray(provider.upper_bound, dtype=np.float64)
    md.upper_bound = ub.ctypes.data
    lo, hi = C.c_int32(), C.c_int32()
    st = load_library().relp_shard_plan(C.byref(md), C.byref(config), C.byref(lo), C.byref(hi))
    if st != 0:
        raise RelpError(f"relp_shard_plan failed ({st})")
    return lo.value, hi.value


class Tableau:

    def __init__(self, provider: MatrixData, config: Optional[Config] = None, *, device_dense_ptr: Optional[int] = None,
                 device_dense_ld: Optional[int] = None, **config_overrides):
        self._lib = load_library()
        cfg = config if config is not None else default_config()
        for k, v in config_overrides.items():
            setattr(cfg, k, v)
        self.config = cfg
        keep = []

        def ptr(a, dtype):
            arr = np.ascontiguousarray(a, dtype=dtype)
            keep.append(arr)
            return arr.ctypes.data

        md = _MatrixData()
        md.nr_normal, md.nr_eq, md.nr_range = provider.nr_normal, provider.nr_eq, provider.nr_range
        md.nr_le, md.nr_ge = provider.nr_le, provider.nr_ge
        if device_dense_ptr is not None:
            md.format, md.matrix_memory = FORMAT_DENSE, MEM_DEVICE
            md.dense = device_dense_ptr
            md.dense_ld = device_dense_ld or provider.nr_constraints
        elif provider.dense is not None:
            md.format, md.matrix_memory = FORMAT_DENSE, MEM_HOST
            dense = np.asfortranarray(provider.dense, dtype=np.float64)
            keep.append(dense)
            md.dense = dense.ctypes.data
            md.dense_ld = dense.shape[0]
        else:
            md.format, md.matrix_memory = FORMAT_CSC, MEM_HOST
            md.col_ptr = ptr(provider.col_ptr, np.int64)
            md.row_idx = ptr(provider.row_idx, np.int32)
            md.values = ptr(provider.values, np.float64)
        md.b = ptr(provider.b, np.float64)
        md.ranges = ptr(provider.ranges, np.float64)
        md.cost = ptr(provider.cost, np.float64)
        md.upper_bound = ptr(provider.upper_bound, np.float64)
        h = C.c_void_p()
        st = self._lib.relp_engine_create(C.byref(md), C.byref(cfg), C.byref(h))
        self._h = h
        if st != 0:
            msg = self._lib.relp_last_error(h).decode() if h else "allocation failed"
            if h:
                self._lib.relp_engine_destroy(h)
            self._h = None
            raise RelpError(f"relp_engine_create failed ({st}): {msg}")
        self.provider = provider
        del keep

    def close(self):
        if getattr(self, "_h", None):
            self._lib.relp_engine_destroy(self._h)
            self._h = None

    def __del__(self):
        try:
            self.close()
        except Exception:
            pass

    def _ck(self, st):
        if st != 0:
            raise RelpError(f"relp call failed ({st}): {self._lib.relp_last_error(self._h).decode()}")

    @property
    def handle(self):
        return self._h

    def set_stream(self, hip_stream: int):
        self._ck(self._lib.relp_set_stream(self._h, hip_stream))

    def nr_rows(self) -> int:
        return self._lib.relp_nr_rows(self._h)

    def nr_columns(self) -> int:
        return self._lib.relp_nr_columns(self._h)

    def nr_artificial_variables(self) -> int:
        return self._lib.relp_nr_artificial(self._h)

    @property
    def phase(self) -> int:
        return self._lib.relp_phase(self._h)

    def select_primal_pivot_column(self, rule: int) -> Optional[Tuple[int, float]]:
        found, col, cost = C.c_int32(), C.c_int32(), C.c_double()
        self._ck(self._lib.relp_select_primal_pivot_column(self._h, rule, C.byref(found), C.byref(col), C.byref(cost)))
        return (col.value, cost.value) if found.value else None

    def relative_costs(self) -> np.ndarray:
        out = np.zeros(self.nr_columns())
        self._ck(self._lib.relp_relative_costs(self._h, out.ctypes.data))
        return out

    def relative_cost(self, j: int) -> float:
        return float(self.relative_costs()[j])

    def generate_column(self, j: int) -> np.ndarray:
        out = np.zeros(self.nr_rows())
        self._ck(self._lib.relp_generate_column(self._h, j, out.ctypes.data))
        return out

    def generate_element(self, i: int, j: int) -> float:
        v = C.c_double()
        self._ck(self._lib.relp_generate_element(self._h, i, j, C.byref(v)))
        return v.value

    def set_reinversion_interval(self, pivots: int) -> None:
        self._ck(self._lib.relp_set_reinversion_interval(self._h, int(pivots)))

    def reinversions(self) -> int:
        return int(self._lib.relp_reinversions(self._h))

    def select_primal_pivot_row(self, column=None) -> Optional[int]:
        found, row = C.c_int32(), C.c_int32()
        if column is None:
            self._ck(self._lib.relp_select_primal_pivot_row(self._h, C.byref(found), C.byref(row)))
        else:
            col = np.ascontiguousarray(column, dtype=np.float64)
            if col.shape != (self.nr_rows(),):
                raise ValueError("column must have nr_rows() entries")
            self._ck(self._lib.relp_select_primal_pivot_row_of(self._h, col.ctypes.data_as(C.POINTER(C.c_double)),
                                                              C.byref(found), C.byref(row)))
        return row.value if found.value else None

    def bring_into_basis(self, column: int, row: int, cost: float) -> int:
        leaving = C.c_int32()
        self._ck(self._lib.relp_bring_into_basis(self._h, column, row, cost, C.byref(leaving)))
        return leaving.value

    def run(self, max_iters: int) -> Tuple[int, int]:
        done, oc = C.c_int64(), C.c_int32()
        self._ck(self._lib.relp_run(self._h, max_iters, C.byref(done), C.byref(oc)))
        return done.value, oc.value

    def solve_relaxation(self, max_iters: int = 1 << 40) -> int:
        oc = C.c_int32()
        self._ck(self._lib.relp_solve_relaxation(self._h, max_iters, C.byref(oc)))
        return oc.value

    def flush(self) -> None:
        self._ck(self._lib.relp_flush(self._h))

    def update_block(self) -> int:
        return self._lib.relp_update_block(self._h)

    def load_batch(self) -> int:
        return self._lib.relp_tab_load_batch(self._h)

    def flush_stats(self) -> Tuple[int, int]:
        out = (C.c_int64 * 2)()
        self._ck(self._lib.relp_tab_flush_stats(self._h, out))
        return int(out[0]), int(out[1])

    def engine_kind(self) -> int:
        return int(self._lib.relp_engine_kind(self._h))

    def robust_stats(self) -> dict:
        out = (C.c_int64 * 4)()
        self._ck(self._lib.relp_robust_stats(self._h, out))
        return dict(zip(("small_pivots", "columns_barred", "confirmations", "reinversion_interval"), (int(v) for v in out)))

    def lu_stats(self) -> dict:
        out = (C.c_int64 * 8)()
        self._ck(self._lib.relp_lu_stats(self._h, out))
        keys = ("refactorisations", "m", "nnz_l", "nnz_u", "levels_l", "levels_u", "levels_ut", "levels_lt")
        stats = dict(zip(keys, (int(v) for v in out)))
        la = (C.c_int64 * 4)()
        self._ck(self._lib.relp_lu_lookahead_stats(self._h, la))
        stats.update(lookahead_installs=int(la[0]), replayed_changes=int(la[1]), lookahead=int(la[2]), fuse_lanes=int(la[3]))
        return stats

    def lu_kernel_layout(self) -> dict:
        out = (C.c_int32 * 4)()
        self._ck(self._lib.relp_lu_kernel_layout(self._h, out))
        return {"persistent_kernel": bool(out[0]), "layout": int(out[1]), "tail_slots": int(out[2]), "grid_price": bool(out[3])}

    def lu_set_device_factorisation(self, on: bool) -> None:
        self._ck(self._lib.relp_lu_set_device_factorisation(self._h, 1 if on else 0))

    def lu_factor_residual(self) -> float:
        out = C.c_double()
        self._ck(self._lib.relp_lu_factor_residual(self._h, C.byref(out)))
        return out.value

    def lu_device_factorisation_stats(self) -> dict:
        out = (C.c_int64 * 6)()
        self._ck(self._lib.relp_lu_device_factorisation_stats(self._h, out))
        keys = ("enabled", "device_factorisations", "host_fallbacks", "kernel_us", "last_bump", "last_peeled")
        return dict(zip(keys, (int(v) for v in out)))

    def basis_inverse_row(self, row: int) -> np.ndarray:
        out = np.zeros(self.nr_rows())
        self._ck(self._lib.relp_basis_inverse_row(self._h, row, out.ctypes.data))
        return out

    def should_refactor(self) -> bool:
        v = C.c_int32()
        self._ck(self._lib.relp_should_refactor(self._h, C.byref(v)))
        return bool(v.value)

    @staticmethod
    def _sparse(column):
        idx = np.ascontiguousarray([i for i, _ in column], dtype=np.int32)
        val = np.ascontiguousarray([v for _, v in column], dtype=np.float64)
        return idx, val

    def generate_column_of(self, column) -> np.ndarray:
        idx, val = self._sparse(column)
        out = np.zeros(self.nr_rows())
        self._ck(self._lib.relp_generate_column_of(self._h, idx.ctypes.data, val.ctypes.data, len(idx), out.ctypes.data))
        return out

    def cost_difference_of(self, column) -> float:
        idx, val = self._sparse(column)
        v = C.c_double()
        self._ck(self._lib.relp_cost_difference_of(self._h, idx.ctypes.data, val.ctypes.data, len(idx), C.byref(v)))
        return v.value

    def lu_change_basis(self, pivot_row_index: int) -> None:
        self._ck(self._lib.relp_lu_change_basis(self._h, pivot_row_index))

    def lu_set_factors(self, lower_columns, upper_columns) -> None:
        m = self.nr_rows()

        def csc(cols):
            cols = list(cols) + [[] for _ in range(m - len(cols))]
            ptr = np.zeros(m + 1, dtype=np.int64)
            for j, c in enumerate(cols):
                ptr[j + 1] = ptr[j] + len(c)
            idx = np.ascontiguousarray([i for c in cols for i, _ in c] or [0], dtype=np.int32)
            val = np.ascontiguousarray([v for c in cols for _, v in c] or [0.0], dtype=np.float64)
            return ptr, idx, val
        lp, li, lv = csc(lower_columns)
        up, ui, uv = csc(upper_columns)
        self._ck(self._lib.relp_lu_set_factors(self._h, lp.ctypes.data, li.ctypes.data, lv.ctypes.data, up.ctypes.data,
                                               ui.ctypes.data, uv.ctypes.data))

    def lu_updates(self):
        n = C.c_int32()
        self._ck(self._lib.relp_lu_updates(self._h, C.byref(n)))
        m = self.nr_rows()
        out = []
        for k in range(n.value):
            pivot, nnz = C.c_int32(), C.c_int32()
            idx, val = np.zeros(m, dtype=np.int32), np.zeros(m)
            self._ck(self._lib.relp_lu_get_update(self._h, k, C.byref(pivot), idx.ctypes.data, val.ctypes.data, m, C.byref(nnz)))
            out.append((pivot.value, list(zip(idx[:nnz.value].tolist(), val[:nnz.value].tolist()))))
        return out

    def lu_upper(self):
        m = self.nr_rows()
        cap = m * (m + 1) // 2 + m
        ptr, idx, val, nnz = np.zeros(m + 1, dtype=np.int64), np.zeros(cap, dtype=np.int32), np.zeros(cap), C.c_int64()
        self._ck(self._lib.relp_lu_get_upper(self._h, ptr.ctypes.data, idx.ctypes.data, val.ctypes.data, cap, C.byref(nnz)))
        return [list(zip(idx[ptr[j]:ptr[j + 1]].tolist(), val[ptr[j]:ptr[j + 1]].tolist())) for j in range(m)]

    PHASE_NAMES = ("price", "scatter", "l_solve", "eta_forward", "spike_push", "u_solve", "ratio", "b_update", "u_bar",
                   "ut_solve", "compact", "eta_backward", "lt_solve", "vectors", "load_store", "stage_and_level0")

    def lu_phase_cycles(self) -> dict:
        out = (C.c_int64 * 16)()
        self._ck(self._lib.relp_lu_phase_cycles(self._h, out))
        return dict(zip(self.PHASE_NAMES, (int(v) for v in out)))

    def from_basis(self, basis_columns) -> None:
        arr = np.ascontiguousarray(basis_columns, dtype=np.int32)
        self._ck(self._lib.relp_from_basis(self._h, arr.ctypes.data))

    def objective_function_value(self) -> float:
        v = C.c_double()
        self._ck(self._lib.relp_get_objective(self._h, C.byref(v)))
        return v.value

    def b(self) -> np.ndarray:
        out = np.zeros(self.nr_rows())
        self._ck(self._lib.relp_get_b(self._h, out.ctypes.data))
        return out

    def minus_pi(self) -> np.ndarray:
        out = np.zeros(self.nr_rows())
        self._ck(self._lib.relp_get_minus_pi(self._h, out.ctypes.data))
        return out

    def basis_indices(self) -> np.ndarray:
        out = np.zeros(self.nr_rows(), dtype=np.int32)
        self._ck(self._lib.relp_get_basis_indices(self._h, out.ctypes.data))
        return out

    def basis_inverse(self) -> np.ndarray:
        m = self.nr_rows()
        out = np.zeros((m, m))
        self._ck(self._lib.relp_get_basis_inverse(self._h, out.ctypes.data))
        return out

    def current_bfs(self) -> List[Tuple[int, float]]:
        m = self.nr_rows()
        cols, vals, cnt = np.zeros(m, dtype=np.int32), np.zeros(m), C.c_int32()
        self._ck(self._lib.relp_current_bfs(self._h, cols.ctypes.data, vals.ctypes.data, m, C.byref(cnt)))
        return list(zip(cols[:cnt.value].tolist(), vals[:cnt.value].tolist()))

    def degenerate_pivots(self) -> int:
        out = C.c_int64()
        self._ck(self._lib.relp_get_degenerate_pivots(self._h, C.byref(out)))
        return out.value

    def iterations(self) -> int:
        v = C.c_int64()
        self._ck(self._lib.relp_get_iterations(self._h, C.byref(v)))
        return v.value

    def trace(self) -> List[Tuple[int, int, int, int]]:
        cap = int(self.config.trace_capacity)
        arrs = [np.zeros(max(cap, 1), dtype=np.int32) for _ in range(4)]
        cnt = C.c_int64()
        self._ck(self._lib.relp_get_trace(self._h, *[a.ctypes.data for a in arrs], cap, C.byref(cnt)))
        k = min(cnt.value, cap)
        return list(zip(*(a[:k].tolist() for a in arrs)))

    def check_basis(self) -> Tuple[float, float, float]:
        a, b, c = C.c_double(), C.c_double(), C.c_double()
        self._ck(self._lib.relp_check_basis(self._h, C.byref(a), C.byref(b), C.byref(c)))
        return a.value, b.value, c.value

    def profile_enable(self, enable: bool, max_launches: int = 0, sample_every: int = 1):
        self._ck(self._lib.relp_profile_enable(self._h, int(enable), max_launches, sample_every))

    def profile_read(self):
        out = {}
        for kid, name in enumerate(KERNEL_NAMES):
            n, ms = C.c_int64(), C.c_double()
            self._ck(self._lib.relp_profile_read(self._h, kid, C.byref(n), C.byref(ms)))
            out[name] = (n.value, ms.value)
        return out


def phase_one_primal(tableau: Tableau, max_iters: int = 1 << 40) -> int:
    if tableau.phase != 1:
        raise RelpError("tableau is not artificial")
    return tableau.run(max_iters)[1]


def phase_two_primal(tableau: Tableau, max_iters: int = 1 << 40) -> int:
    if tableau.phase != 2:
        raise RelpError("tableau still has artificial variables")
    return tableau.run(max_iters)[1]


def solve_relaxation(provider: MatrixData, **config_overrides):
    t = Tableau(provider, **config_overrides)
    return t.solve_relaxation(), t


VERIFY_IDENTITY, VERIFY_BASIC, VERIFY_MIN_B = 1e-5, 1e-3, -1e-6
VERIFIED_LEGS = (("read", "robust", ENGINE_LU), ("scaled", "robust", ENGINE_LU), ("scaled", "robust-dantzig", ENGINE_LU),
                 ("scaled", "robust-dantzig", ENGINE_TABLEAU), ("read", "robust-dantzig", ENGINE_LU), ("scaled", "robust", ENGINE_REVISED),
                 ("read", "robust", ENGINE_REVISED), ("read", "robust", ENGINE_TABLEAU), ("scaled", "robust", ENGINE_TABLEAU),
                 ("read", "default", ENGINE_LU), ("read", "default", ENGINE_REVISED), ("read", "default", ENGINE_TABLEAU),
                 ("read", "robust-dantzig", ENGINE_TABLEAU, 12))
_ENGINE_NAMES = {ENGINE_REVISED: "revised", ENGINE_TABLEAU: "tableau", ENGINE_LU: "lu"}


def solve_verified(provider: MatrixData, pivots_per_leg: Optional[int] = None, seconds_per_leg: float = 60.0, legs=VERIFIED_LEGS):
    import time
    budget = pivots_per_leg if pivots_per_leg is not None else 30 * (int(provider.nr_rows) + int(provider.nr_columns))
    report = {"legs": [], "verified": False, "scaled": False}
    scaled = None
    said = {}
    last = RUNNING
    for entry in legs:
        data, cfg_name, kind = entry[:3]
        times = entry[3] if len(entry) > 3 else 1
        leg = {"data": data, "config": cfg_name, "engine": _ENGINE_NAMES[kind]}
        report["legs"].append(leg)
        t0 = time.perf_counter()
        if data == "scaled" and scaled is None:
            scaled = provider.scaled()
        if cfg_name == "robust":
            cfg = robust_config(engine=kind)
        elif cfg_name == "robust-dantzig":
            cfg = robust_config(engine=kind, phase_one_rule=STEEPEST_DESCENT, phase_two_rule=STEEPEST_DESCENT)
        else:
            cfg = default_config(engine=kind)
        try:
            t = Tableau(scaled[0] if data == "scaled" else provider, config=cfg)
        except RelpError as e:
            leg["outcome"] = "create_failed: " + str(e)[:120]
            continue
        try:
            oc, total = RUNNING, 0
            while total < times * budget and time.perf_counter() - t0 < times * seconds_per_leg:
                done, oc = t.run(min(20000, times * budget - total))
                total += done
                if oc not in (RUNNING, PHASE_ONE_DONE):
                    break
            leg["pivots"] = total
            leg["outcome"] = OUTCOME_NAMES.get(oc, str(oc)) if oc not in (RUNNING, PHASE_ONE_DONE) else "limit"
            last = oc
            if oc == OPTIMAL:
                ident, basic, min_b = t.check_basis()
                leg["check_basis"] = [ident, basic, min_b]
                if ident <= VERIFY_IDENTITY and basic <= VERIFY_BASIC and min_b >= VERIFY_MIN_B:
                    report["verified"] = True
                    report["scaled"] = data == "scaled"
                    if data == "scaled":
                        report["row_scale"], report["column_scale"] = scaled[1], scaled[2]
                    return OPTIMAL, t, report
            elif oc in (INFEASIBLE, UNBOUNDED) and data == "read":
                ident, basic, min_b = t.check_basis()
                leg["check_basis"] = [ident, basic, min_b]
                if ident <= VERIFY_IDENTITY and basic <= VERIFY_BASIC and np.isfinite(t.objective_function_value()):
                    said.setdefault(oc, set()).add(kind)
        except RelpError as e:
            leg["outcome"] = "error: " + str(e)[:120]
        t.close()
    for oc, engines in said.items():
        if len(engines) >= 2:
            report["verified"] = True
            return oc, None, report
    return last, None, report
```

Before: 45480 iterations/s.

## Issue tableau kernel global loads early to overlap with pivot selection reductions

Adds an early-loads mode, on by default and switchable off with RELP_TAB_EARLY_LOADS=0. In the select-column and ratio-update kernels it prefetches the first batch of pending eta/W/R0 values, d, alpha, b and basis entries before the block-wide reductions and pivot picks run. The intent is to hide global memory latency behind those serial reduction phases. In exchange it adds register pressure, a stale-shadow path with a ballot check, and more template instantiations.

```diff
diff --git a/include/relp_engine.h b/include/relp_engine.h
--- a/include/relp_engine.h
+++ b/include/relp_engine.h
@@ -113,6 +113,7 @@
 relp_status_t relp_flush(relp_engine_t *h);
 relp_status_t relp_tab_flush_stats(relp_engine_t *h, int64_t *out2);
 int32_t       relp_tab_load_batch(const relp_engine_t *h);
+int32_t       relp_tab_early_loads(const relp_engine_t *h);
 int32_t       relp_update_block(const relp_engine_t *h);
 relp_status_t relp_lu_stats(const relp_engine_t *h, int64_t *out8);
 relp_status_t relp_lu_lookahead_stats(const relp_engine_t *h, int64_t *out4);
diff --git a/rust-lp_amd/csrc/relp_abi.cpp b/rust-lp_amd/csrc/relp_abi.cpp
--- a/rust-lp_amd/csrc/relp_abi.cpp
+++ b/rust-lp_amd/csrc/relp_abi.cpp
@@ -81,6 +81,7 @@
 int64_t relp_reinversions(const relp_engine_t* h) { return h ? H(h).reinversions() : -1; }
 int32_t relp_update_block(const relp_engine_t* h) { return h ? H(h).update_block() : -1; }
 int32_t relp_tab_load_batch(const relp_engine_t* h) { return h ? H(h).tab_load_batch_size() : -1; }
+int32_t relp_tab_early_loads(const relp_engine_t* h) { return h ? H(h).tab_early_loads() : -1; }
 relp_status_t relp_lu_stats(const relp_engine_t* h, int64_t* out8) { return (h && out8) ? H(h).lu_stats(out8) : RELP_E_ARG; }
 relp_status_t relp_lu_lookahead_stats(const relp_engine_t* h, int64_t* out4) { return (h && out4) ? H(h).lu_lookahead_stats(out4) : RELP_E_ARG; }
 relp_status_t relp_lu_kernel_layout(const relp_engine_t* h, int32_t* out4) { return (h && out4) ? H(h).lu_kernel_layout(out4) : RELP_E_ARG; }
diff --git a/rust-lp_amd/csrc/relp_device_common.h b/rust-lp_amd/csrc/relp_device_common.h
--- a/rust-lp_amd/csrc/relp_device_common.h
+++ b/rust-lp_amd/csrc/relp_device_common.h
@@ -118,26 +118,32 @@
 }
 
 template <int BS>
-__device__ __forceinline__ void tab_select_entering(const TableauView& tv, const SelectPartials& sp, int count, double& k1,
-                                                    int& bj) {
+__device__ __forceinline__ void tab_select_strided(const SelectPartials& sp, int count, double& k1, int& bj) {
+    for (int t = threadIdx.x + BS; t < count; t += BS) {
+        const double key = sp.k1[t];
+        const int j = sp.j[t];
+        if (key < k1 || (key == k1 && j < bj)) { k1 = key; bj = j; }
+    }
+}
+
+template <int BS, bool kKeepOwn>
+__device__ __forceinline__ void tab_select_reduced(const TableauView& tv, const SelectPartials& sp, int count, double& k1,
+                                                   int& bj, double own) {
     constexpr int kListMax = 32, kGroups = BS / kThreads;
     __shared__ int s_list[kListMax];
     __shared__ int s_cnt;
     __shared__ int s_low[BS / 64];
-    for (int t = threadIdx.x + BS; t < count; t += BS) {
-        const double key = sp.k1[t];
-        const int j = sp.j[t];
-        if (key < k1 || (key == k1 && j < bj)) { k1 = key; bj = j; }
-    }
     if (threadIdx.x == 0) s_cnt = 0;
     block_min_key<BS>(k1, bj);
     if (!(bj != 0x7fffffff && sp.rule == 2 && sp.tol_tie > 0.0)) return;
     const double bound = k1 + sp.tol_tie * fmax(1.0, fabs(k1));
-    for (int t = threadIdx.x; t < count; t += BS) {
-        if (!(sp.k1[t] <= bound)) continue;
+    auto list_slot = [&](int t) {
         const int pos = atomicAdd(&s_cnt, 1);
         if (pos < kListMax) s_list[pos] = t;
-    }
+    };
+    if (kKeepOwn && (int)threadIdx.x < count && own <= bound) list_slot(threadIdx.x);
+    for (int t = threadIdx.x + (kKeepOwn ? BS : 0); t < count; t += BS)
+        if (sp.k1[t] <= bound) list_slot(t);
     __syncthreads();
     const int listed = s_cnt;
     const int grp = threadIdx.x / kThreads, u = threadIdx.x % kThreads;
@@ -163,6 +169,13 @@
     bj = s_low[0];
 #pragma unroll
     for (int w = 1; w < BS / 64; ++w) bj = min(bj, s_low[w]);
+}
+
+template <int BS>
+__device__ __forceinline__ void tab_select_entering(const TableauView& tv, const SelectPartials& sp, int count, double& k1,
+                                                    int& bj) {
+    tab_select_strided<BS>(sp, count, k1, bj);
+    tab_select_reduced<BS, false>(tv, sp, count, k1, bj, 0.0);
 }
 
 __device__ __forceinline__ int candidate_winner(const double* key, const double* idx, int64_t stride, int count, int rule,
@@ -394,7 +407,7 @@
     return a > tol.pivot ? bi / a : INFINITY;
 }
 
-template <int BS>
+template <int BS, bool kKeepFirst = false>
 __device__ __forceinline__ void ratio_blocks_pick(const double* alpha, const double* b, const int32_t* basis_indices, int m,
                                                   const Tolerances& tol, const double* rmin, int nblk, int* row_out, int* leave_out,
                                                   double first = INFINITY, bool have_first = false, int rpb = kThreads) {
@@ -422,11 +435,14 @@
     const double gmin = s_bcast;
     if (gmin == INFINITY) { *row_out = -1; *leave_out = 0x7fffffff; return; }
     const double bound = gmin + tol.tie * fmax(1.0, fabs(gmin));
-    for (int t = threadIdx.x; t < nblk; t += BS) {
-        if (!(rmin[t] <= bound)) continue;
+    auto list_block = [&](int t) {
         const int pos = atomicAdd(&s_cnt, 1);
         if (pos < kListMax) s_list[pos] = t;
-    }
+    };
+    const bool keep = kKeepFirst && have_first;
+    if (keep && (int)threadIdx.x < nblk && first <= bound) list_block(threadIdx.x);
+    for (int t = threadIdx.x + (keep ? BS : 0); t < nblk; t += BS)
+        if (rmin[t] <= bound) list_block(t);
     __syncthreads();
     const int listed = s_cnt;
     const bool use_list = listed <= kListMax;
diff --git a/rust-lp_amd/csrc/relp_engine.cpp b/rust-lp_amd/csrc/relp_engine.cpp
--- a/rust-lp_amd/csrc/relp_engine.cpp
+++ b/rust-lp_amd/csrc/relp_engine.cpp
@@ -88,7 +88,7 @@
 DeferredUpdate Engine::deferred() const {
     DeferredUpdate du;
     du.W = d_W_; du.ld = ld_b_; du.kmax = block_; du.S = d_S_; du.pos_of_row = d_pos_of_row_; du.wr = d_wr_; du.R = d_R_;
-    du.batch = load_batch_; du.w_split = w_split_;
+    du.batch = load_batch_; du.w_split = w_split_; du.early = early_loads_;
     return du;
 }
 
@@ -247,6 +247,8 @@
             load_batch_ = tab_load_batch(e ? std::atoi(e) : 0);
             const char* w = std::getenv("RELP_TAB_W_SPLIT");
             w_split_ = w && std::atoi(w) >= 1 ? std::min(std::atoi(w), 16) : kTabSplitDefault;
+            const char* l = std::getenv("RELP_TAB_EARLY_LOADS");
+            early_loads_ = !(l && std::atoi(l) == 0);
         }
         {
             const char* e = std::getenv("RELP_FUSED_UPDATE");
diff --git a/rust-lp_amd/csrc/relp_engine.hpp b/rust-lp_amd/csrc/relp_engine.hpp
--- a/rust-lp_amd/csrc/relp_engine.hpp
+++ b/rust-lp_amd/csrc/relp_engine.hpp
@@ -83,6 +83,7 @@
     relp_status_t get_degenerate_pivots(int64_t* out);
     relp_status_t tab_flush_stats(int64_t* out2);
     int32_t tab_load_batch_size() const { return tableau_ ? load_batch_ : 0; }
+    int32_t tab_early_loads() const { return tableau_ ? early_loads_ : 0; }
     relp_status_t get_trace(int32_t* phase, int32_t* entering, int32_t* row, int32_t* leaving, int64_t cap,
                             int64_t* count);
     relp_status_t check_basis(double* max_identity_error, double* max_basic_cost, double* min_b);
@@ -138,7 +139,7 @@
     unsigned long long *d_fmask_ = nullptr, *d_fstats_ = nullptr;
     double* d_R0c_ = nullptr;
     FlushList flush_list() const;
-    int32_t load_batch_ = 0, w_split_ = 0;
+    int32_t load_batch_ = 0, w_split_ = 0, early_loads_ = 0;
     double* d_cost_store_ = nullptr;
     int32_t* d_idcol_ = nullptr;
     bool fused_update_ = false, shadow_pending_ = false;
diff --git a/rust-lp_amd/csrc/relp_kernels.h b/rust-lp_amd/csrc/relp_kernels.h
--- a/rust-lp_amd/csrc/relp_kernels.h
+++ b/rust-lp_amd/csrc/relp_kernels.h
@@ -41,6 +41,7 @@
     double*  R;
     int32_t  batch;
     int32_t  w_split;
+    int32_t  early;
 };
 
 struct ColumnTable {
diff --git a/rust-lp_amd/csrc/relp_kernels_tableau.hip b/rust-lp_amd/csrc/relp_kernels_tableau.hip
--- a/rust-lp_amd/csrc/relp_kernels_tableau.hip
+++ b/rust-lp_amd/csrc/relp_kernels_tableau.hip
@@ -6,8 +6,7 @@
 typedef double double4_t __attribute__((ext_vector_type(4)));
 
 template <int B, class Use>
-__device__ __forceinline__ void for_pending(const double* base, int64_t stride, int64_t x, int n, Use&& use) {
-    int j0 = 0;
+__device__ __forceinline__ void for_pending_from(const double* base, int64_t stride, int64_t x, int j0, int n, Use&& use) {
     for (; j0 + B <= n; j0 += B) {
         double v[B];
 #pragma unroll
@@ -23,6 +22,26 @@
         for (int t = 0; t < B; ++t)
             if (j0 + t < n) use(j0 + t, v[t]);
     }
+}
+
+template <int B, class Use>
+__device__ __forceinline__ void for_pending(const double* base, int64_t stride, int64_t x, int n, Use&& use) {
+    for_pending_from<B>(base, stride, x, 0, n, use);
+}
+
+template <int B>
+__device__ __forceinline__ void load_pending_head(double (&head)[B], const double* base, int64_t stride, int64_t x, int n) {
+#pragma unroll
+    for (int t = 0; t < B; ++t) head[t] = base[(int64_t)min(t, n - 1) * stride + x];
+}
+
+template <int B, class Use>
+__device__ __forceinline__ void for_pending_from_head(const double (&head)[B], const double* base, int64_t stride, int64_t x,
+                                                      int n, Use&& use) {
+#pragma unroll
+    for (int t = 0; t < B; ++t)
+        if (t < n) use(t, head[t]);
+    for_pending_from<B>(base, stride, x, B, n, use);
 }
 
 template <int B>
@@ -30,6 +49,17 @@
     if (u == 0.0 || j1 <= j0) return;
     double* col = du.W + (int64_t)j0 * du.ld;
     for_pending<B>(col, du.ld, i, j1 - j0, [&](int j, double old) {
+        const double w = s_wr[j0 + j];
+        if (w != 0.0) col[(int64_t)j * du.ld + i] = fma(u, w, old);
+    });
+}
+
+template <int B>
+__device__ __forceinline__ void tab_update_w_row(const DeferredUpdate& du, int i, double u, const double* s_wr, int j0, int j1,
+                                                 const double (&head)[B]) {
+    if (u == 0.0 || j1 <= j0) return;
+    double* col = du.W + (int64_t)j0 * du.ld;
+    for_pending_from_head<B>(head, col, du.ld, i, j1 - j0, [&](int j, double old) {
         const double w = s_wr[j0 + j];
         if (w != 0.0) col[(int64_t)j * du.ld + i] = fma(u, w, old);
     });
@@ -126,24 +156,33 @@
 }
 
 template <int B>
+struct RowPrefetch { double d_old, t0_r, head[B]; };
+
+template <int B, bool kPre = false>
 __device__ __forceinline__ void tab_row_update_core(const TableauView& tv, const DeferredUpdate& du, const SelectPartials& sp,
                                                     const PivotRecord& R, int block, const double* s_wr, int p_old, int jt, int r,
-                                                    int q, int leaving, double d_q, double alpha_r) {
+                                                    int q, int leaving, double d_q, double alpha_r,
+                                                    const RowPrefetch<B>* pre = nullptr) {
     const PivotRecord* rec = &R;
     const int c = tv.c_lo + block * kThreads + threadIdx.x;
-    const double d_old = c < tv.c_hi ? tv.d[c] : 0.0;
-    __syncthreads();
+    double d_old;
+    if (kPre) d_old = pre->d_old;
+    else {
+        d_old = c < tv.c_hi ? tv.d[c] : 0.0;
+        __syncthreads();
+    }
     double key = INFINITY;
     int kj = 0x7fffffff;
     if (c < tv.c_hi) {
         double base;
         if (jt < p_old) base = tv.R0[(int64_t)jt * tv.ld_r + c];
         else {
-            base = tv.T0[(int64_t)c * tv.ld_t + r];
+            base = kPre ? pre->t0_r : tv.T0[(int64_t)c * tv.ld_t + r];
             tv.R0[(int64_t)jt * tv.ld_r + c] = base;
         }
         double row = base;
-        for_pending<B>(tv.R0, tv.ld_r, c, p_old, [&](int j, double r0) { row = fma(s_wr[j], r0, row); });
+        if (kPre) for_pending_from_head<B>(pre->head, tv.R0, tv.ld_r, c, p_old, [&](int j, double r0) { row = fma(s_wr[j], r0, row); });
+        else for_pending<B>(tv.R0, tv.ld_r, c, p_old, [&](int j, double r0) { row = fma(s_wr[j], r0, row); });
         const double theta = d_q / alpha_r;
         const int j = c - tv.col_off;
         double dn = fma(-theta, row, d_old);
@@ -214,7 +253,7 @@
     else tab_update_w_vectors_body<B>(du, m, alpha, b, basis_indices, in_basis, trace, trace_cap, R, rec, blockIdx.x - nb_row);
 }
 
-template <int B>
+template <int B, bool E>
 __global__ __launch_bounds__(kThreads) void k_tab_ratio_update_all(TableauView tv, DeferredUpdate du, SelectPartials sp, int nb_row,
                                                                    int m, const double* alpha,
                                                                    const double* __restrict__ b_in, double* __restrict__ b_out,
@@ -225,7 +264,7 @@
                                                                    double* __restrict__ shadow, int32_t* __restrict__ shadow_meta,
                                                                    PivotRecord* rec, const double* __restrict__ msgs, int count,
                                                                    int64_t msg_len, int rule, int split) {
-    const double first = (!msgs && (int)threadIdx.x < nblk) ? rmin[threadIdx.x] : INFINITY;
+    double first = (!msgs && (int)threadIdx.x < nblk) ? rmin[threadIdx.x] : INFINITY;
     PivotRecord R = *rec;
     const bool w_half = (int)blockIdx.x >= nb_row;
     const int part = w_half ? ((int)blockIdx.x - nb_row) / nblk : 0;
@@ -237,6 +276,31 @@
         if (mine) { b_out[i] = b_in[i]; basis_out[i] = basis_in[i]; }
         return;
     }
+    const int p_old = R.p_now;
+    int j_lo = 0, j_hi = 0;
+    auto share_of_part = [&]() {
+        const int share = (p_old + split - 1) / split;
+        j_lo = min(part * share, p_old); j_hi = min(j_lo + share, p_old);
+    };
+    const int c_pre = min(tv.c_lo + (int)blockIdx.x * kThreads + (int)threadIdx.x, tv.c_hi - 1);
+    const int i_pre = min(i, m - 1);
+    RowPrefetch<B> pre;
+    double a_pre, b_pre, w_head[B];
+    int basis_pre;
+    if (E) {
+        asm volatile("" : "+v"(first));
+        if (!w_half) {
+            pre.d_old = tv.d[c_pre];
+            if (p_old > 0) load_pending_head<B>(pre.head, tv.R0, tv.ld_r, c_pre, p_old);
+        } else {
+            share_of_part();
+            if (!msgs) {
+                a_pre = alpha[i_pre];
+                if (lead) { b_pre = b_in[i_pre]; basis_pre = basis_in[i_pre]; }
+            }
+            if (j_hi > j_lo) load_pending_head<B>(w_head, du.W + (int64_t)j_lo * du.ld, du.ld, i_pre, j_hi - j_lo);
+        }
+    }
     if (msgs) {
         int q_win = 0;
         double d_win = 0.0;
@@ -253,7 +317,7 @@
         rmin = alpha + m;
     }
     int r, leaving;
-    ratio_blocks_pick<kThreads>(alpha, b_in, basis_in, m, tol, rmin, nblk, &r, &leaving, first, !msgs);
+    ratio_blocks_pick<kThreads, E>(alpha, b_in, basis_in, m, tol, rmin, nblk, &r, &leaving, first, !msgs);
     if (r < 0) {
         if (mine) { b_out[i] = b_in[i]; basis_out[i] = basis_in[i]; }
         if (lead && wblock == 0 && threadIdx.x == 0) rec->outcome = DEV_NO_ROW;
@@ -262,36 +326,49 @@
     __shared__ double s_wr[kMaxEta];
     __shared__ double s_ab[2];
     __shared__ int s_jt;
-    const int p_old = R.p_now;
-    if ((int)threadIdx.x < p_old) s_wr[threadIdx.x] = du.W[(int64_t)threadIdx.x * du.ld + r];
-    if (threadIdx.x == 0) {
-        s_ab[0] = alpha[r]; s_ab[1] = b_in[r];
-        const int slot = du.pos_of_row[r];
-        s_jt = slot < 0 ? p_old : slot;
+    if (!E) {
+        if ((int)threadIdx.x < p_old) s_wr[threadIdx.x] = du.W[(int64_t)threadIdx.x * du.ld + r];
+        if (threadIdx.x == 0) {
+            s_ab[0] = alpha[r]; s_ab[1] = b_in[r];
+            const int slot = du.pos_of_row[r];
+            s_jt = slot < 0 ? p_old : slot;
+        }
+    } else {
+        double w_r, a_r, bb_r;
+        int slot;
+        if ((int)threadIdx.x < p_old) w_r = du.W[(int64_t)threadIdx.x * du.ld + r];
+        if (threadIdx.x == 0) { a_r = alpha[r]; bb_r = b_in[r]; slot = du.pos_of_row[r]; }
+        if (!w_half) pre.t0_r = tv.T0[(int64_t)c_pre * tv.ld_t + r];
+        asm volatile("" ::: "memory");
+        if ((int)threadIdx.x < p_old) s_wr[threadIdx.x] = w_r;
+        if (threadIdx.x == 0) { s_ab[0] = a_r; s_ab[1] = bb_r; s_jt = slot < 0 ? p_old : slot; }
     }
     __syncthreads();
     const double alpha_r = s_ab[0], b_r = s_ab[1];
     const int jt = s_jt, q = R.q;
     if (!w_half) {
-        tab_row_update_core<B>(tv, du, sp, R, blockIdx.x, s_wr, p_old, jt, r, q, leaving, R.d_q, alpha_r);
+        if (E) tab_row_update_core<B, true>(tv, du, sp, R, blockIdx.x, s_wr, p_old, jt, r, q, leaving, R.d_q, alpha_r, &pre);
+        else tab_row_update_core<B>(tv, du, sp, R, blockIdx.x, s_wr, p_old, jt, r, q, leaving, R.d_q, alpha_r);
         return;
     }
     const double br = b_r / alpha_r;
-    const int share = (p_old + split - 1) / split;
-    const int j_lo = min(part * share, p_old), j_hi = min(j_lo + share, p_old);
+    if (!E) share_of_part();
+    const bool early_ab = E && !msgs;
     if (!lead) {
         if (i < m && i != r) {
-            const double u = -alpha[i] / alpha_r;
-            tab_update_w_row<B>(du, i, u, s_wr, j_lo, j_hi);
+            const double u = -(early_ab ? a_pre : alpha[i]) / alpha_r;
+            if (E) tab_update_w_row<B>(du, i, u, s_wr, j_lo, j_hi, w_head);
+            else tab_update_w_row<B>(du, i, u, s_wr, j_lo, j_hi);
             if (jt >= j_lo && jt < j_hi) du.W[(int64_t)jt * du.ld + i] += u;
         }
         return;
     }
     if (i < m) {
-        const double a = alpha[i], b_i = b_in[i];
+        const double a = early_ab ? a_pre : alpha[i], b_i = early_ab ? b_pre : b_in[i];
         const double u = (i == r) ? (1.0 / alpha_r - 1.0) : (-a / alpha_r);
         if (i != r) {
-            tab_update_w_row<B>(du, i, u, s_wr, j_lo, j_hi);
+            if (E) tab_update_w_row<B>(du, i, u, s_wr, j_lo, j_hi, w_head);
+            else tab_update_w_row<B>(du, i, u, s_wr, j_lo, j_hi);
             double* tgt = du.W + (int64_t)jt * du.ld + i;
             if (jt >= p_old) *tgt = u;
             else if (jt < j_hi) *tgt += u;
@@ -305,7 +382,7 @@
             shadow_meta[1] = jt < p_old ? p_old : p_old + 1;
         }
         b_out[i] = pivot_b(a, b_i, br, i == r);
-        basis_out[i] = (i == r) ? q : basis_in[i];
+        basis_out[i] = (i == r) ? q : (early_ab ? basis_pre : basis_in[i]);
     }
     if (i == 0) {
         if (msgs) record_candidate(rec, rule, 0, q, R.d_q);
@@ -324,15 +401,25 @@
     if (threadIdx.x == 0) shadow_meta[0] = -1;
 }
 
-template <int B>
+template <int B, bool E>
 __global__ __launch_bounds__(kThreads) void k_tab_select_column(TableauView tv, DeferredUpdate du, SelectPartials sp,
                                                                 int count, double* alpha, double* msg,
                                                                 const double* b, Tolerances tol,
                                                                 double* rmin, PivotRecord* rec,
                                                                 const double* shadow, int32_t* shadow_meta) {
     const int outcome = rec->outcome, p = rec->n_eta;
-    if (shadow_meta) {
-        const int srow = shadow_meta[0], slen = shadow_meta[1];
+    __shared__ double s_sh[E ? kMaxEta : 1];
+    double sh = 0.0;
+    bool stale = false;
+    int slen = 0;
+    int srow = -1;
+    if (E && shadow_meta) {
+        srow = shadow_meta[0]; slen = shadow_meta[1];
+        sh = shadow[min((int)threadIdx.x, du.kmax)];
+    }
+    if (!E && shadow_meta) {
+        srow = shadow_meta[0];
+        slen = shadow_meta[1];
         if (srow >= 0 && srow / kThreads == (int)blockIdx.x) {
             if ((int)threadIdx.x < slen) du.W[(int64_t)threadIdx.x * du.ld + srow] = shadow[threadIdx.x];
             __syncthreads();
@@ -345,10 +432,29 @@
     if ((int)threadIdx.x < count) { k1 = sp.k1[threadIdx.x]; bj = sp.j[threadIdx.x]; }
     const int i = blockIdx.x * kThreads + threadIdx.x;
     const double b_i = (rmin && i < tv.m) ? b[i] : 0.0;
+    const double own = k1;
+    double head[B];
+    if (E) {
+        tab_select_strided<kThreads>(sp, count, k1, bj);
+        asm volatile("" : "+v"(sh), "+v"(k1), "+v"(bj));
+        if (shadow_meta) {
+            if ((int)threadIdx.x < du.kmax) s_sh[threadIdx.x] = sh;
+            if (srow >= 0 && srow / kThreads == (int)blockIdx.x) {
+                if ((int)threadIdx.x < slen) du.W[(int64_t)threadIdx.x * du.ld + srow] = sh;
+                stale = i == srow;
+                __syncthreads();
+                if (threadIdx.x == kThreads - 1) shadow_meta[0] = -1;
+            }
+            if (blockIdx.x == 0 && threadIdx.x == kThreads - 1) rec->p_now = p;
+        }
+        if (outcome != DEV_RUNNING) return;
+        if (p > 0) load_pending_head<B>(head, du.W, du.ld, min(i, tv.m - 1), p);
+    }
     if (outcome != DEV_RUNNING) return;
     __shared__ double s_vs[kMaxEta];
     __shared__ double s_min[kThreads / 64];
-    tab_select_entering<kThreads>(tv, sp, count, k1, bj);
+    if (E) tab_select_reduced<kThreads, true>(tv, sp, count, k1, bj, own);
+    else tab_select_entering<kThreads>(tv, sp, count, k1, bj);
     if (bj == 0x7fffffff) {
         if (msg) {
             if (i < tv.m) alpha[i] = 0.0;
@@ -375,7 +481,16 @@
     double ratio = INFINITY;
     if (i < tv.m) {
         double a = t0;
-        for_pending<B>(du.W, du.ld, i, p, [&](int j, double w) { a = fma(w, s_vs[j], a); });
+        if (!E) {
+            for_pending<B>(du.W, du.ld, i, p, [&](int j, double w) { a = fma(w, s_vs[j], a); });
+        } else if (__builtin_amdgcn_ballot_w64(stale) == 0) {
+            for_pending_from_head<B>(head, du.W, du.ld, i, p, [&](int j, double w) { a = fma(w, s_vs[j], a); });
+        } else {
+            for_pending_from_head<B>(head, du.W, du.ld, i, p, [&](int j, double w) {
+                if (stale && j < slen) w = s_sh[j];
+                a = fma(w, s_vs[j], a);
+            });
+        }
         alpha[i] = a;
         const double bz = b_i <= tol.zero ? 0.0 : b_i;
         if (a > tol.pivot) ratio = bz / a;
@@ -732,6 +847,14 @@
     static_assert(kTabLoadBatchDefault == 8, "the default of tab_load_batch is the switch's default case");
 }
 
+template <class Launch>
+static void with_load_batch_early(const DeferredUpdate& du, Launch&& launch) {
+    with_load_batch(du.batch, [&](auto B) {
+        if (du.early) launch(B, std::true_type{});
+        else launch(B, std::false_type{});
+    });
+}
+
 void launch_tab_build(const TableauView& tv, const double* A, int64_t ld_a, const ColumnTable& ct, hipStream_t s) {
     const int64_t total = (int64_t)tv.m * (tv.c_hi - tv.c_lo);
     if (total <= 0) return;
@@ -784,9 +907,9 @@
 void launch_tab_select_column_rmin(const TableauView& tv, const DeferredUpdate& du, SelectPartials sp, int32_t count,
                                    double* alpha, const double* b, Tolerances tol, double* rmin, PivotRecord* rec,
                                    hipStream_t s, const double* shadow, int32_t* shadow_meta) {
-    with_load_batch(du.batch, [&](auto B) {
-        hipLaunchKernelGGL((k_tab_select_column<decltype(B)::value>), dim3(cdiv(tv.m, kThreads)), dim3(kThreads), 0, s, tv, du, sp, count, alpha,
-                           (double*)nullptr, b, tol, rmin, rec, shadow, shadow_meta);
+    with_load_batch_early(du, [&](auto B, auto E) {
+        hipLaunchKernelGGL((k_tab_select_column<decltype(B)::value, decltype(E)::value>), dim3(cdiv(tv.m, kThreads)), dim3(kThreads), 0, s, tv,
+                           du, sp, count, alpha, (double*)nullptr, b, tol, rmin, rec, shadow, shadow_meta);
     });
 }
 
@@ -798,9 +921,9 @@
     const int nb_row = tv.c_hi > tv.c_lo ? tab_scan_blocks(tv.c_hi - tv.c_lo) : 0;
     const int nb_w = cdiv(m, kThreads);
     int split = tab_load_batch(du.batch) == 1 ? 1 : std::max(1, std::min({(int)du.w_split, (int)du.kmax, (kTabSplitCUs - nb_row) / nb_w}));
-    with_load_batch(du.batch, [&](auto B) {
-        hipLaunchKernelGGL((k_tab_ratio_update_all<decltype(B)::value>), dim3(nb_row + split * nb_w), dim3(kThreads), 0, s, tv, du, sp, nb_row, m,
-                           alpha, b_in, b_out, basis_in, basis_out, in_basis, trace, trace_cap, tol, rmin, nb_w, shadow,
+    with_load_batch_early(du, [&](auto B, auto E) {
+        hipLaunchKernelGGL((k_tab_ratio_update_all<decltype(B)::value, decltype(E)::value>), dim3(nb_row + split * nb_w), dim3(kThreads), 0, s,
+                           tv, du, sp, nb_row, m, alpha, b_in, b_out, basis_in, basis_out, in_basis, trace, trace_cap, tol, rmin, nb_w, shadow,
                            shadow_meta, rec, msgs, (int)count, msg_len, (int)rule, split);
     });
 }
@@ -818,9 +941,9 @@
 void launch_tab_select_column_msg(const TableauView& tv, const DeferredUpdate& du, SelectPartials sp, int32_t count,
                                   double* msg, const double* b, Tolerances tol, PivotRecord* rec, hipStream_t s,
                                   const double* shadow, int32_t* shadow_meta) {
-    with_load_batch(du.batch, [&](auto B) {
-        hipLaunchKernelGGL((k_tab_select_column<decltype(B)::value>), dim3(cdiv(tv.m, kThreads)), dim3(kThreads), 0, s, tv, du, sp, count, msg + 3,
-                           msg, b, tol, msg + 3 + tv.m, rec, shadow, shadow_meta);
+    with_load_batch_early(du, [&](auto B, auto E) {
+        hipLaunchKernelGGL((k_tab_select_column<decltype(B)::value, decltype(E)::value>), dim3(cdiv(tv.m, kThreads)), dim3(kThreads), 0, s, tv,
+                           du, sp, count, msg + 3, msg, b, tol, msg + 3 + tv.m, rec, shadow, shadow_meta);
     });
 }
 
diff --git a/rust-lp_amd/engine.py b/rust-lp_amd/engine.py
--- a/rust-lp_amd/engine.py
+++ b/rust-lp_amd/engine.py
@@ -74,6 +74,7 @@
     "relp_flush": (C.c_int, [C.c_void_p]),
     "relp_update_block": (C.c_int32, [C.c_void_p]),
     "relp_tab_load_batch": (C.c_int32, [C.c_void_p]),
+    "relp_tab_early_loads": (C.c_int32, [C.c_void_p]),
     "relp_tab_flush_stats": (C.c_int, [C.c_void_p, C.POINTER(C.c_int64)]),
     "relp_lu_stats": (C.c_int, [C.c_void_p, C.POINTER(C.c_int64)]),
     "relp_lu_lookahead_stats": (C.c_int, [C.c_void_p, C.POINTER(C.c_int64)]),
@@ -341,6 +342,9 @@
     def load_batch(self) -> int:
         return self._lib.relp_tab_load_batch(self._h)
 
+    def early_loads(self) -> int:
+        return self._lib.relp_tab_early_loads(self._h)
+
     def flush_stats(self) -> Tuple[int, int]:
         out = (C.c_int64 * 2)()
         self._ck(self._lib.relp_tab_flush_stats(self._h, out))
```

After: 45290 iterations/s. No clear change (-0.4%).
